# ldyken53/gaussian-splatting-wgpu

Hardware: AMD Instinct MI355X
Metric: frames/sec (higher is better)
Workload: dtype f32; 1 GPU; bicycle-like synthetic 6.1M gaussians @1920x1080; gaussians=6100000, width=1920, height=1080, tile_size=16, parallelism=single GPU, visible=2430918, processed=15909895, block_evaluated=6068168, sort_passes=1, depth_ordered_emission=True, tight_binning=True, blend_mode=fused, camera=64-step orbit, moved every frame

## Files before the change

gaussian-splatting-wgpu_amd/csrc/build.py:

```python
#!/usr/bin/env python3
import os
import subprocess
import sys
from concurrent.futures import ThreadPoolExecutor

HERE = os.path.dirname(os.path.abspath(__file__))
OUT = os.path.join(HERE, "..", "lib")
HIPCC = os.environ.get("HIPCC", "/opt/rocm/bin/hipcc")
ARCH = "gfx950"
FLAGS = ["--offload-arch=" + ARCH, "-O3", "-std=c++17", "-ffp-contract=off", "-fno-slp-vectorize", "-fPIC", "-fvisibility=hidden",
         "-Wall", "-Wno-unused-function", "-Wno-unused-value", "-Wno-unused-result"]
FILE_FLAGS = {}
SOURCES = ["k_preprocess.hip", "k_binning.hip", "k_gsort.hip", "k_rows.hip", "k_sort.hip", "k_blend.hip", "k_pick.hip", "k_state.hip", "k_export.hip", "k_insert.hip", "k_snapshot.hip", "k_xform.hip", "k_grade.hip", "k_coverage.hip", "k_attr.hip", "k_neigh.hip", "k_cluster.hip", "k_knn.hip", "k_pack.hip",
           "gs_context.hip", "gs_frame.hip", "gs_readback.hip", "gs_state.hip", "gs_export.hip", "gs_insert.hip", "gs_snapshot.hip", "gs_xform.hip", "gs_xform_math.hip", "gs_grade.hip", "gs_grade_math.hip", "gs_coverage.hip", "gs_attr.hip", "gs_neigh.hip", "gs_cluster.hip", "gs_knn.hip", "gs_pack.hip", "gs_pack_host.hip", "gs_ply.hip", "gs_stages.hip",
           "k_moments.hip", "gs_moments.hip", "k_pairs.hip", "gs_pairs.hip", "k_consensus.hip", "gs_consensus.hip", "k_merge.hip", "gs_merge.hip", "k_surface.hip", "gs_surface.hip"]


def _stale(target, deps):
    if not os.path.exists(target):
        return True
    t = os.path.getmtime(target)
    return any(os.path.getmtime(d) > t for d in deps)


def build(force=False, verbose=False, profiling=False):
    os.makedirs(OUT, exist_ok=True)
    objdir = os.path.join(OUT, "obj_prof" if profiling else "obj")
    os.makedirs(objdir, exist_ok=True)
    headers = [os.path.join(HERE, h) for h in ("gs_device.h", "gs_binning.h", "gs_kernels.h", "gs_tight.h", "gs_runtime.h", "gs_xform_math.h", "gs_grade_math.h", "gs_state_sum.h", "gs_neigh_dev.h", "gs_pack_math.h", "gs_exact_sum.h", "gs_exact_dev.h", "gs_pair_host.h", "gs_pack_host.h", "gs_file_writer.h", "gs_consensus_host.h", "gs_merge_math.h", "gs_grid_math.h", "gs_surface_math.h")] + [
        os.path.join(HERE, "..", "..", "include", "gsplat", "gs_abi.h")]

    def compile_one(src):
        obj = os.path.join(objdir, src.replace(".hip", ".o"))
        path = os.path.join(HERE, src)
        if force or _stale(obj, [path] + headers):
            cmd = [HIPCC] + FLAGS + FILE_FLAGS.get(src, []) + (["-DGS_PROFILING"] if profiling else []) + ["-c", path, "-o", obj]
            if verbose:
                print(" ".join(cmd))
            subprocess.check_call(cmd)
        return obj

    with ThreadPoolExecutor(max_workers=12) as ex:
        objs = list(ex.map(compile_one, SOURCES))
    so = os.path.join(OUT, "libgsplat_hip_prof.so" if profiling else "libgsplat_hip.so")
    if force or _stale(so, objs):
        subprocess.check_call([HIPCC, "--offload-arch=" + ARCH, "-shared", "-fPIC", "-o", so] + objs)
    return os.path.abspath(so)


if __name__ == "__main__":
    print(build(force="--force" in sys.argv, verbose=True, profiling="--profiling" in sys.argv))


def build_napi(force=False, verbose=False):
    inc = "/usr/include/node"
    if not os.path.exists(os.path.join(inc, "node_api.h")):
        return None
    so = build(force=force, verbose=verbose)
    src = os.path.join(HERE, "napi", "gs_napi.c")
    out = os.path.join(OUT, "gsplat_napi.node")
    if force or _stale(out, [src, so, os.path.join(HERE, "..", "..", "include", "gsplat", "gs_abi.h")]):
        cmd = ["gcc", "-O2", "-fPIC", "-shared", "-Wall", "-DNODE_GYP_MODULE_NAME=gsplat_napi", "-I" + inc, src, "-o", out,
               "-L" + OUT, "-lgsplat_hip", "-Wl,-rpath,$ORIGIN"]
        if verbose:
            print(" ".join(cmd))
        subprocess.check_call(cmd)
    return os.path.abspath(out)
```

gaussian-splatting-wgpu_amd/csrc/gs_context.hip:

```cpp
#include <atomic>
#include <cmath>
#include <cstdarg>
#include <memory>
#include <new>

#include "gs_runtime.h"

thread_local char g_err[512] = "";
int32_t fail(int32_t code, const char* fmt, ...) {
    va_list ap;
    va_start(ap, fmt);
    vsnprintf(g_err, sizeof(g_err), fmt, ap);
    va_end(ap);
    return code;
}

static uint32_t tiles_f32(uint32_t extent, uint32_t ts) {
    return (uint32_t)std::ceil((float)extent / (float)ts);
}
static uint32_t bits_for(uint64_t v) {
    uint32_t b = 0;
    while (v) { ++b; v >>= 1; }
    return b ? b : 1;
}

GS_EXPORT const char* gs_last_error(void) { return g_err; }
GS_EXPORT int32_t gs_abi_version(void) { return GS_ABI_VERSION; }

int32_t alloc_kv(gs_ctx* c, uint64_t capacity, uint64_t row_cap) {
    if (capacity >= (1ull << 30)) return fail(GS_ERR_CAPACITY, "capacity %llu exceeds 2^30 intersections", (unsigned long long)capacity);
    if (row_cap >= (1ull << 31)) return fail(GS_ERR_CAPACITY, "%llu row items exceed the 2^31 limit", (unsigned long long)row_cap);
    c->gr.valid = false;
    c->keysA.reset(); c->valsA.reset(); c->keysB.reset(); c->valsB.reset(); c->keysU.reset(); c->valsU.reset();
    c->keysG.reset(); c->chunk_table.reset(); c->arena.reset(); c->rows_sorted.reset(); c->M3.reset(); c->ctl_mem.reset();
    c->valsG.reset();
    c->keysG_valid = c->valsG_valid = c->gdataG_valid = false;
    capacity = std::max<uint64_t>(capacity, 4096);
    row_cap = (std::max<uint64_t>(row_cap, 4096) + 15) & ~(uint64_t)15;
    const size_t kb = (size_t)capacity * 4;
    HIP_TRY(hipMalloc(c->keysA.out(), kb));
    HIP_TRY(hipMalloc(c->valsA.out(), kb));
    HIP_TRY(hipMalloc(c->keysB.out(), kb));
    HIP_TRY(hipMalloc(c->valsB.out(), kb));
    c->sort_index = GsSort{{c->keysA, c->valsA}, {c->keysB, c->valsB}, c->passes, 8, 0, false, false};
    c->sort_tile = GsSort{{c->keysA, c->valsA}, {c->keysB, c->valsB}, c->tile_passes, c->tile_bits, c->tile16 ? 0u : 1u, c->tile16, true};
    HIP_TRY(hipMalloc(c->chunk_table.out(), (size_t)gs_emit_chunks(std::max(capacity, row_cap)) * 4));
    if (c->tight_ok) {
        HIP_TRY(hipMalloc(c->arena.out(), (size_t)row_cap * 12));
        HIP_TRY(hipMalloc(c->rows_sorted.out(), gs_rows_sorted_bytes(row_cap)));
        HIP_TRY(hipMalloc(c->M3.out(), (size_t)gs_rows_chunks(row_cap) * 256 * 4));
    }
    const size_t ctl_sz = (sizeof(GsControl) + 255) & ~(size_t)255;
    const size_t scan_sz = (((size_t)gs_scan_blocks(c->n ? c->n : 1) + 1) * 8 + 255) & ~(size_t)255;
    const size_t sort_sz = (size_t)std::max(c->passes, c->tile_passes) * gs_sort_tiles(capacity) * 256 * 4;
    const size_t rows_sz = c->tight_ok ? (size_t)gs_rows_sort_tiles(row_cap) * 256 * 4 : 0;
    const size_t depth_sz = ((size_t)c->T * 4 + 255) & ~(size_t)255;
    c->ctl_bytes = ctl_sz + depth_sz + rows_sz + scan_sz + sort_sz;
    c->ctl_bytes_tight = ctl_sz + depth_sz + rows_sz;
    HIP_TRY(hipMalloc(c->ctl_mem.out(), c->ctl_bytes));
    char* const base = (char*)c->ctl_mem.get();
    c->ctl = (GsControl*)base;
    c->tile_depth = (uint32_t*)(base + ctl_sz);
    c->rows_status = (uint32_t*)(base + ctl_sz + depth_sz);
    c->scan_status = (unsigned long long*)(base + ctl_sz + depth_sz + rows_sz);
    c->sort_status = (uint32_t*)(base + ctl_sz + depth_sz + rows_sz + scan_sz);
    c->capacity = capacity;
    c->row_cap = row_cap;
    c->frame.capacity = (uint32_t)capacity;
    c->frame.row_cap = (uint32_t)row_cap;
    return GS_OK;
}

GS_EXPORT int32_t gs_create(const gs_config* cfg, gs_ctx** out) {
    if (!cfg || !out) return fail(GS_ERR_INVALID_ARGUMENT, "gs_create: null argument");
    if (cfg->struct_size != sizeof(gs_config)) return fail(GS_ERR_INVALID_ARGUMENT, "gs_create: struct_size %u != %zu", cfg->struct_size, sizeof(gs_config));
    if (cfg->width == 0 || cfg->height == 0) return fail(GS_ERR_INVALID_ARGUMENT, "gs_create: empty canvas");
    if (cfg->tile_size != 8 && cfg->tile_size != 16 && cfg->tile_size != 32)
        return fail(GS_ERR_INVALID_ARGUMENT, "gs_create: tile_size must be 8, 16 or 32 (got %u)", cfg->tile_size);
    int ndev = 0;
    if (hipGetDeviceCount(&ndev) != hipSuccess || ndev == 0) return fail(GS_ERR_NO_DEVICE, "gs_create: no HIP device");
    if (cfg->device < 0 || cfg->device >= ndev) return fail(GS_ERR_INVALID_ARGUMENT, "gs_create: device %d of %d", cfg->device, ndev);
    HIP_TRY(hipSetDevice(cfg->device));

    std::unique_ptr<gs_ctx> c(new (std::nothrow) gs_ctx());
    if (!c) return fail(GS_ERR_OUT_OF_MEMORY, "gs_create: host allocation failed");
    c->cfg = *cfg;
    GsFrame& f = c->frame;
    f.width = cfg->width; f.height = cfg->height; f.tile_size = cfg->tile_size;
    f.ntx = tiles_f32(cfg->width, cfg->tile_size);
    f.nty = tiles_f32(cfg->height, cfg->tile_size);
    if (f.ntx >= 32768 || f.nty >= 65536) return fail(GS_ERR_INVALID_ARGUMENT, "gs_create: canvas too large");
    f.col0 = cfg->col_begin;
    f.col1 = cfg->col_end;
    if (f.col0 == 0 && f.col1 == 0) f.col1 = f.ntx;
    if (f.col1 > f.ntx || f.col0 >= f.col1) return fail(GS_ERR_INVALID_ARGUMENT, "gs_create: bad tile-column slab [%u,%u) of %u", f.col0, f.col1, f.ntx);
    f.full = (f.col0 == 0 && f.col1 == f.ntx) ? 1u : 0u;
    f.px0 = f.col0 * f.tile_size;
    f.slab_w = std::min(f.width, f.col1 * f.tile_size) - f.px0;
    c->T = f.ntx * f.nty;
    const uint64_t max_key = ((uint64_t)f.nty * f.ntx + f.ntx) * 1000ull + 999ull;
    if (max_key > 0xFFFFFFFFull) return fail(GS_ERR_INVALID_ARGUMENT, "gs_create: tile ids overflow the 32-bit key (write_tile_ids.wgsl:29)");
    c->key_bits = bits_for(max_key);
    c->passes = (c->key_bits + 7) / 8;
    const uint32_t tbits = bits_for((uint64_t)f.nty * f.ntx + f.ntx);
    c->tile_passes = (tbits + 7) / 8;
    c->tile_bits = (tbits + c->tile_passes - 1) / c->tile_passes;
    c->tile16 = ((uint64_t)f.nty * f.ntx + f.ntx) < 0xFFFFull;
    if ((uint64_t)(f.ntx + 1) * (f.nty + 1) > GS_COUNT_MASK) return fail(GS_ERR_INVALID_ARGUMENT, "gs_create: canvas has too many tiles");
    c->tight_ok = f.ntx <= 255u && f.nty <= 255u;

    hipDeviceProp_t prop;
    HIP_TRY(hipGetDeviceProperties(&prop, cfg->device));
    c->opt.grid_persist = (uint32_t)prop.multiProcessorCount * 4;
    if (cfg->stream) c->stream = (hipStream_t)cfg->stream;
    else { HIP_TRY(hipStreamCreateWithFlags(c->own_stream.out(), hipStreamNonBlocking)); c->stream = c->own_stream; }

    HIP_TRY(hipMalloc(c->ranges.out(), (size_t)c->T * 4));
    HIP_TRY(hipMemset(c->ranges, 0, (size_t)c->T * 4));
    const size_t px = (size_t)f.slab_w * f.height;
    HIP_TRY(hipMalloc(c->rgba8.out(), px * 4));
    HIP_TRY(hipMemset(c->rgba8, 0, px * 4));
    if (cfg->flags & GS_FLAG_F32_TAP) HIP_TRY(hipMalloc(c->rgbf.out(), px * 12));
    if (cfg->flags & GS_FLAG_AUX_OUTPUTS) {
        HIP_TRY(hipMalloc(c->alpha.out(), px * 4));
        HIP_TRY(hipMalloc(c->depth.out(), px * 4));
        HIP_TRY(hipMemset(c->alpha, 0, px * 4));
        HIP_TRY(hipMemset(c->depth, 0, px * 4));
    }
    HIP_TRY(hipHostMalloc(c->h_ctl.out(), sizeof(GsControl), hipHostMallocDefault));
    memset(c->h_ctl, 0, sizeof(GsControl));
    HIP_TRY(hipMalloc(c->d_pxb.out(), 65 * 4));
    HIP_TRY(hipMalloc(c->tileoff.out(), 256 * 256 * 4));
    HIP_TRY(hipMalloc(c->rowtot.out(), 256 * 4));
    HIP_TRY(hipMalloc(c->sticky.out(), 4 * 4));
    HIP_TRY(hipMemset(c->sticky, 0, 4 * 4));
    HIP_TRY(hipHostMalloc(c->h_rep.out(), sizeof(GsReport), hipHostMallocDefault));
    memset(c->h_rep, 0, sizeof(GsReport));
    if (cfg->flags & GS_FLAG_TIMING) {
        for (auto& row : c->ev)
            for (auto& e : row) HIP_TRY(hipEventCreate(e.out()));
        c->have_events = true;
    }
    c->fif = (c->own_stream && f.full) ? 3u : 1u;
    *out = c.release();
    return GS_OK;
}

gs_ctx::~gs_ctx() { drop_graph(this); }

GS_EXPORT int32_t gs_destroy(gs_ctx* c) {
    if (!c) return GS_OK;
    hipSetDevice(c->cfg.device);
    drop_shadows(c);
    if (c->stream) hipStreamSynchronize(c->stream);
    delete c;
    return GS_OK;
}

static int32_t alloc_per_gaussian(gs_ctx* c, uint64_t n, uint64_t min_capacity = 0, uint64_t min_rows = 0) {
    c->gr.valid = false;
    c->scene_own.reset();
    c->scene_mem = nullptr;
    c->n = (uint32_t)n;
    c->frame.n = (uint32_t)n;
    c->have_frame = false;
    c->cov.reset();
    c->ng = gs_ctx::Neigh{};
    c->cl = gs_ctx::Cluster{};
    c->kn = gs_ctx::Knn{};
    c->sf = gs_ctx::Surface{};
    c->counts.reset(); c->offsets.reset(); c->grec.reset(); c->rowptr.reset(); c->gsort_scratch.reset(); c->gdata.reset(); c->gdataG.reset();
    c->unit_off.reset(); c->unit_n.reset();
    const size_t np = ((size_t)n + 63) & ~(size_t)63;
    const size_t ne = (size_t)gs_gsort_tiles((uint32_t)(n ? n : 1)) * 2048, nu = ne / 1024 + 2;
    HIP_TRY(hipMalloc(c->counts.out(), ne * 4));
    HIP_TRY(hipMalloc(c->offsets.out(), std::max<size_t>(np * 4, 256)));
    HIP_TRY(hipMalloc(c->grec.out(), std::max<size_t>(np * 16, 256)));
    HIP_TRY(hipMalloc(c->rowptr.out(), ne * 4));
    HIP_TRY(hipMalloc(c->unit_off.out(), ne * 2));
    HIP_TRY(hipMalloc(c->unit_n.out(), nu * 4));
    HIP_TRY(hipMemsetAsync(c->unit_n, 0, nu * 4, c->stream));
    HIP_TRY(hipMalloc(c->gsort_scratch.out(), gs_gsort_scratch_bytes((uint32_t)n)));
    HIP_TRY(hipMalloc(c->gdata.out(), ((size_t)n + GS_RECORD_SLACK) * 64));
    HIP_TRY(hipMemsetAsync(c->gdata, 0, ((size_t)n + GS_RECORD_SLACK) * 64, c->stream));
    uint64_t cap = c->cfg.max_intersections ? c->cfg.max_intersections : std::max<uint64_t>(4 * n, 1u << 22);
    cap = std::max<uint64_t>(cap, min_capacity);
    cap = std::min<uint64_t>(cap, (1ull << 30) - 1);
    const uint64_t rows = std::max<uint64_t>(std::max<uint64_t>(2 * n, 1u << 20), min_rows);
    return alloc_kv(c, cap, rows);
}

GsSceneLayout scene_layout(void* base, uint64_t n, bool state) {
    GsSceneLayout L;
    const size_t np = ((size_t)n + 63) & ~(size_t)63;
    const size_t sh_end = np * 4 * 4 + np * 32 + (size_t)n * 192, state_at = (sh_end + 255) & ~(size_t)255;
    L.np = np;
    L.state_at = state_at;
    L.bytes = state ? state_at + np : sh_end;
    char* p = (char*)base;
    GsScene& s = L.scene;
    s.px = (float*)p; p += np * 4; s.py = (float*)p; p += np * 4; s.pz = (float*)p; p += np * 4;
    s.smax = (float*)p; p += np * 4;
    s.geo = (float4*)p; p += np * 32;
    s.sh = (float4*)p;
    s.state = state ? (const uint8_t*)base + state_at : nullptr;
    return L;
}
static void scene_views(gs_ctx* c, uint64_t n) {
    const GsSceneLayout L = scene_layout(c->scene_own.get(), n, has_state(c));
    c->scene_mem = c->scene_own;
    c->scene_bytes = L.bytes;
    c->scene = L.scene;
}

uint64_t scene_new_serial() {
    static std::atomic<uint64_t> next{1};
    return next.fetch_add(1, std::memory_order_relaxed);
}
int32_t scene_alloc(gs_ctx* c, uint64_t n, uint64_t min_capacity, uint64_t min_rows) {
    c->scene_serial = scene_new_serial();
    int32_t rc = alloc_per_gaussian(c, n, min_capacity, min_rows);
    if (rc != GS_OK) return rc;
    const GsSceneLayout L = scene_layout(nullptr, n, has_state(c));
    HIP_TRY(hipMalloc(c->scene_own.out(), std::max<size_t>(L.bytes, 256)));
    scene_views(c, n);
    if (has_state(c))
        HIP_TRY(hipMemsetAsync((char*)c->scene_mem + L.state_at, 0, std::max<size_t>(L.np, 4), c->stream));
    return GS_OK;
}

int32_t scene_install(gs_ctx* c, DevBuf<>&& mem, uint64_t n, uint64_t min_capacity, uint64_t min_rows) {
    const int32_t rc = alloc_per_gaussian(c, n, min_capacity, min_rows);
    if (rc != GS_OK) {
        c->scene = GsScene{};
        c->n = c->frame.n = 0;
        return rc;
    }
    c->scene_own = std::move(mem);
    scene_views(c, n);
    return GS_OK;
}

static int32_t upload_common(gs_ctx* c, const void* d_aos, uint64_t n) {
    int32_t rc = scene_alloc(c, n);
    if (rc != GS_OK) return rc;
    if (n) gs_launch_repack(d_aos, (uint32_t)n, 0, c->scene, c->stream);
    HIP_TRY(hipGetLastError());
    HIP_TRY(hipStreamSynchronize(c->stream));
    return GS_OK;
}

void drop_shadows(gs_ctx* c) {
    for (gs_ctx* s : c->shadows) gs_destroy(s);
    c->shadows.clear();
    c->last = c;
    c->rr = 0;
    c->cap_hint = 0;
    c->row_hint = 0;
}
GS_EXPORT int32_t gs_share_splats(gs_ctx* c, gs_ctx* owner) {
    if (!c || !owner || c == owner) return fail(GS_ERR_INVALID_ARGUMENT, "gs_share_splats: needs two distinct contexts");
    if (c->cfg.device != owner->cfg.device) return fail(GS_ERR_INVALID_ARGUMENT, "gs_share_splats: contexts are on different devices");
    if (!c->is_shadow) drop_shadows(c);
    if (!owner->scene_mem) return fail(GS_ERR_NO_SCENE, "gs_share_splats: the owner holds no splats");
    if (has_state(c) && !has_state(owner))
        return fail(GS_ERR_INVALID_ARGUMENT, "gs_share_splats: this context has GS_FLAG_SPLAT_STATE, the owner keeps no state plane");
    HIP_TRY(hipSetDevice(c->cfg.device));
    if (c->pending) { int32_t rc = wait_one(c); if (rc != GS_OK) return rc; }
    int32_t rc = alloc_per_gaussian(c, owner->n, c->cfg.max_intersections ? 0 : owner->capacity, owner->row_cap);
    if (rc != GS_OK) return rc;
    c->scene_mem = owner->scene_mem;
    c->scene_bytes = owner->scene_bytes;
    c->scene = owner->scene;
    c->scene_serial = scene_new_serial();
    HIP_TRY(hipStreamSynchronize(c->stream));
    return GS_OK;
}

GS_EXPORT int32_t gs_upload_splats_device(gs_ctx* c, const void* d_aos, uint64_t n) {
    if (!c || (!d_aos && n)) return fail(GS_ERR_INVALID_ARGUMENT, "gs_upload_splats_device: null argument");
    if (n >= (1ull << 31)) return fail(GS_ERR_INVALID_ARGUMENT, "gs_upload_splats: too many gaussians");
    HIP_TRY(hipSetDevice(c->cfg.device));
    drop_shadows(c);
    return upload_common(c, d_aos, n);
}

GS_EXPORT int32_t gs_upload_splats(gs_ctx* c, const void* aos, uint64_t n) {
    if (!c || (!aos && n)) return fail(GS_ERR_INVALID_ARGUMENT, "gs_upload_splats: null argument");
    if (n >= (1ull << 31)) return fail(GS_ERR_INVALID_ARGUMENT, "gs_upload_splats: too many gaussians");
    HIP_TRY(hipSetDevice(c->cfg.device));
    drop_shadows(c);
    DevBuf<> d;
    const size_t bytes = (size_t)n * GS_SPLAT_RECORD_BYTES;
    HIP_TRY(hipMalloc(d.out(), std::max<size_t>(bytes, 256)));
    if (bytes) {
        hipError_t e = hipMemcpy(d, aos, bytes, hipMemcpyHostToDevice);
        if (e != hipSuccess) return fail(GS_ERR_HIP, "upload memcpy: %s", hipGetErrorString(e));
    }
    return upload_common(c, d, n);
}

GS_EXPORT int32_t gs_host_alloc(uint64_t bytes, void** out) {
    if (!out) return fail(GS_ERR_INVALID_ARGUMENT, "gs_host_alloc: null argument");
    *out = nullptr;
    HIP_TRY(hipHostMalloc(out, std::max<size_t>((size_t)bytes, 256), hipHostMallocDefault));
    return GS_OK;
}
GS_EXPORT void gs_host_free(void* p) { if (p) hipHostFree(p); }

GS_EXPORT int32_t gs_slab_width(gs_ctx* c, uint32_t* px_begin, uint32_t* px_width) {
    if (!c) return fail(GS_ERR_INVALID_ARGUMENT, "gs_slab_width: null ctx");
    if (px_begin) *px_begin = c->frame.px0;
    if (px_width) *px_width = c->frame.slab_w;
    return GS_OK;
}

static int32_t set_option_one(gs_ctx* c, int32_t key, int64_t value) {
    c->gr.valid = false;
    GsOptions& o = c->opt;
    switch (key) {
    case GS_OPT_FRAME_GRAPH: o.frame_graph = (value != 0); return GS_OK;
    case GS_OPT_BLEND_ABLATION: o.blend_ablation = (uint32_t)value & 0x3FFFFu; return GS_OK;
    case GS_OPT_PERSISTENT_GRID: if (value <= 0) break; o.grid_persist = (uint32_t)value; return GS_OK;
    case GS_OPT_RESET_TIMING: c->timed_from = c->frames; c->max_I_seen = 0; c->truncated_frames = 0; return GS_OK;
    case GS_OPT_EMIT_ORDER: if (value < 0 || value > 2) break; o.emit_order = (int)value; return GS_OK;
    case GS_OPT_UNFUSED: return GS_OK;
    case GS_OPT_DEBUG_VIEW: if (value < 0 || value > 4) break; o.debug_view = (uint32_t)value; return GS_OK;
    case GS_OPT_TILE_CULL: o.tile_cull = (value != 0); return GS_OK;
    case GS_OPT_PROJ_CHUNKS: if (value != 0 && value != 2 && value != 4 && value != 8) break; o.tight_nb = (uint32_t)value; return GS_OK;
    case GS_OPT_SELECT_TINT:
        if (!has_state(c)) return fail(GS_ERR_INVALID_ARGUMENT, "gs_set_option: GS_OPT_SELECT_TINT needs GS_FLAG_SPLAT_STATE");
        if (value < 0 || value > 0xFFFFFFFFll) break;
        o.select_tint = (uint32_t)value;
        return GS_OK;
    default: break;
    }
    return fail(GS_ERR_INVALID_ARGUMENT, "gs_set_option: bad key/value %d/%lld", key, (long long)value);
}
GS_EXPORT int32_t gs_set_option(gs_ctx* c, int32_t key, int64_t value) {
    if (!c) return fail(GS_ERR_INVALID_ARGUMENT, "gs_set_option: null ctx");
    if (key == GS_OPT_FRAMES_IN_FLIGHT) {
        if (value < 1 || value > 4) return fail(GS_ERR_INVALID_ARGUMENT, "gs_set_option: frames in flight must be 1..4");
        if (!c->own_stream || !c->frame.full) value = 1;
        int32_t rc = gs_wait(c);
        if (rc != GS_OK && rc != GS_ERR_TRUNCATED) return rc;
        while (c->shadows.size() + 1 > (size_t)value) {
            if (c->last == c->shadows.back()) { c->last = c; }
            gs_destroy(c->shadows.back());
            c->shadows.pop_back();
        }
        c->fif = (uint32_t)value;
        c->rr = 0;
        return GS_OK;
    }
    int32_t rc = set_option_one(c, key, value);
    for (gs_ctx* s : c->shadows) if (rc == GS_OK) rc = set_option_one(s, key, value);
    return rc;
}
```

gaussian-splatting-wgpu_amd/csrc/gs_device.h:

```cpp
#pragma once
#include <hip/hip_runtime.h>
#include <stdint.h>

#define GS_WAVE 64

struct GsFrame {
    uint32_t n;
    uint32_t width, height, tile_size;
    uint32_t ntx, nty;
    uint32_t col0, col1;
    uint32_t px0, slab_w;
    uint32_t capacity;
    uint32_t full;
    uint32_t row_cap;
};

#define GS_COUNT_BITS 22
#define GS_COUNT_MASK 0x3FFFFFu

struct GsControl {
    uint32_t scan_ticket[2];
    uint32_t sort_ticket[4];
    uint32_t rows_ticket;
    uint32_t num_slots;
    uint32_t num_items;
    uint32_t fault;
    uint32_t overflow;
    uint32_t num_intersections;
    uint32_t num_visible;
    uint32_t pad0;
    uint32_t row_cursor[16];
    uint32_t rec_cursor[16];
    unsigned long long num_processed[64];
    unsigned long long num_evaluated[64];
    uint32_t hist[4][256];
    uint32_t rowhist[8][256];
};
__device__ __forceinline__ uint32_t gs_rowhist(const GsControl* ctl, uint32_t r) {
    uint32_t s = 0;
#pragma unroll
    for (int k = 0; k < 8; ++k) s += ctl->rowhist[k][r];
    return s;
}

struct GsReport {
    uint32_t fault, overflow, num_intersections, num_visible, num_slots, num_items, pad0, pad1;
    uint32_t row_cursor[16];
    uint32_t sticky[4];
};
__device__ __forceinline__ void gs_frame_report(const GsControl* ctl, uint32_t I, uint32_t num_items, uint32_t capacity, uint32_t* sticky,
                                                GsReport* rep) {
    uint32_t need = 0;
    for (int k = 0; k < 16; ++k) need = ctl->row_cursor[k] > need ? ctl->row_cursor[k] : need;
    need = need > 0x07FFFFFFu ? 0x7FFFFFFFu : need * 16u;
    const uint32_t over = (I > capacity || ctl->overflow) ? 1u : 0u;
    uint32_t s0 = 0, s1 = 0, s2 = 0, s3 = 0;
    if (sticky) {
        s0 = atomicAdd(&sticky[0], over) + over;
        s1 = atomicOr(&sticky[1], ctl->fault ? 1u : 0u) | (ctl->fault ? 1u : 0u);
        s2 = atomicMax(&sticky[2], I); s2 = s2 > I ? s2 : I;
        s3 = atomicMax(&sticky[3], need); s3 = s3 > need ? s3 : need;
    }
    if (rep) {
        rep->fault = ctl->fault; rep->overflow = over; rep->num_intersections = I; rep->num_visible = ctl->num_visible;
        rep->num_slots = ctl->num_slots; rep->num_items = num_items;
        for (int k = 0; k < 16; ++k) rep->row_cursor[k] = ctl->row_cursor[k];
        rep->sticky[0] = s0; rep->sticky[1] = s1; rep->sticky[2] = s2; rep->sticky[3] = s3;
    }
}

struct GsTightOut {
    uint32_t* arena; uint32_t* rowptr; GsControl* ctl;
    unsigned short* unit_off; uint32_t* unit_n;
    uint32_t rec_shard_cap;
};
#define GS_RECORD_SLACK (16u * 512u * 8u)

struct GsScene {
    const float* px; const float* py; const float* pz;
    const float* smax;
    const float4* geo;
    const float4* sh;
    const uint8_t* state;
};

#define GS_ST_HIDDEN 1u
#define GS_ST_SELECTED 2u
struct GsTint { float t[3]; float k; };
__device__ __forceinline__ uint32_t gs_state_apply(uint32_t s, uint32_t op, uint32_t bits) {
    return op == 1u ? (s | bits) : op == 2u ? (s & ~bits) : op == 3u ? (s ^ bits) : bits;
}
struct GsStateQuad { uint32_t w, valid; };
__device__ __forceinline__ GsStateQuad gs_state_quad(const uint8_t* __restrict__ state, uint32_t n, uint32_t q) {
    const uint64_t first = (uint64_t)q * 4u;
    uint32_t w = 0u, valid = 0u;
    if (first + 4u <= n) {
        valid = 4u;
        if (state) w = reinterpret_cast<const uint32_t*>(state)[q];
    } else if (first < n) {
        valid = (uint32_t)(n - first);
        if (state)
            for (uint32_t k = 0; k < valid; ++k) w |= (uint32_t)state[first + k] << (8u * k);
    }
    return GsStateQuad{w, valid};
}

struct GsPlyTable {
    uint32_t stride, nsrc, all_float;
    uint16_t soff[11 + 48];
    uint8_t stype[11 + 48], slot[11 + 48];
};

struct GsUniforms {
    float view[16];
    float proj[16];
    float cam[3];
    float tan_fovx, tan_fovy, focal_x, focal_y, scale_modifier;
};

__device__ __forceinline__ float wg_max(float a, float b) { return (a < b) ? b : a; }
__device__ __forceinline__ float wg_min(float a, float b) { return (b < a) ? b : a; }
__device__ __forceinline__ int wg_maxi(int a, int b) { return (a < b) ? b : a; }
__device__ __forceinline__ int wg_mini(int a, int b) { return (b < a) ? b : a; }

__device__ __forceinline__ int f2i_sat(float x) {
    if (x != x) return 0;
    if (x >= 2147483648.0f) return 2147483647;
    if (x <= -2147483648.0f) return (-2147483647 - 1);
    return (int)x;
}
__device__ __forceinline__ uint32_t f2u_sat(float x) {
    if (x != x) return 0u;
    if (x >= 4294967296.0f) return 0xFFFFFFFFu;
    if (x <= 0.0f) return 0u;
    return (uint32_t)x;
}

__device__ __forceinline__ float gs_exp(float x) {
    if (x != x) return x;
    if (x > 88.72283935546875f) return __builtin_inff();
    if (x < -103.97208404541015625f) return 0.0f;
    const float nf = __builtin_rintf(x * 1.44269502162933349609375f);
    float r = __builtin_fmaf(-nf, 0.693145751953125f, x);
    r = __builtin_fmaf(-nf, 1.42860677465796470642e-06f, r);
    float p = 1.9875691500e-4f;
    p = __builtin_fmaf(p, r, 1.3981999507e-3f);
    p = __builtin_fmaf(p, r, 8.3334519073e-3f);
    p = __builtin_fmaf(p, r, 4.1665795894e-2f);
    p = __builtin_fmaf(p, r, 1.6666665459e-1f);
    p = __builtin_fmaf(p, r, 5.0000001201e-1f);
    const float z = r * r;
    float y = __builtin_fmaf(p, z, r);
    y = y + 1.0f;
    const int n = (int)nf;
    const int a = n >> 1;
    const int b = n - a;
    const float sa = __uint_as_float((uint32_t)(a + 127) << 23);
    const float sb = __uint_as_float((uint32_t)(b + 127) << 23);
    return (y * sa) * sb;
}

__device__ __forceinline__ float gs_blend_power(float cx, float cy, float cz, float dx, float dy) {
    const float t1 = cx * dx * dx, t2 = cz * dy * dy, t3 = cy * dx * dy;
    return -0.5f * (t1 + t2) - t3;
}
__device__ __forceinline__ float gs_blend_alpha(float op, float power) { return wg_min(0.99f, op * gs_exp(power)); }
struct GsPixel { float T, cr, cg, cb, cd; };
template <bool AUX>
__device__ __forceinline__ GsPixel gs_blend_exact(GsPixel p, float4 p1, float4 p2, float dx, float dy) {
    const float power = gs_blend_power(p1.x, p1.y, p1.z, dx, dy);
    const float alpha = gs_blend_alpha(p2.w, power);
    const float test = p.T * (1.0f - alpha);
    const float cond = (power <= 0.0f && alpha >= (float)(1.0 / 255.0) && test >= 0.0001f) ? 1.0f : 0.0f;
    p.cr += cond * p2.x * alpha * p.T;
    p.cg += cond * p2.y * alpha * p.T;
    p.cb += cond * p2.z * alpha * p.T;
    if constexpr (AUX) p.cd += cond * p1.w * alpha * p.T;
    p.T = cond * test + (1.0f - cond) * p.T;
    return p;
}
template <bool EXACT>
__device__ __forceinline__ bool gs_pixel_final(float T) {
    const float c255 = (float)(1.0 / 255.0);
    return (EXACT ? T * (1.0f - c255) : __builtin_fmaf(-T, c255, T)) < 0.0001f;
}

__device__ __forceinline__ float block_qmin(float cx, float cy, float cz, float dxlo, float dxhi, float dylo, float dyhi,
                                            float& mag) {
    const float X = __builtin_fminf(__builtin_fmaxf(0.0f, dxlo), dxhi);
    const float Y = __builtin_fminf(__builtin_fmaxf(0.0f, dylo), dyhi);
    float q = 3.0e38f;
    mag = 0.0f;
    if (X == 0.0f && Y == 0.0f) return 0.0f;
    if (X != 0.0f) {
        const float dy = __builtin_fminf(__builtin_fmaxf(-cy * X * __builtin_amdgcn_rcpf(cz), dylo), dyhi);
        const float a = 0.5f * cx * X * X, b = 0.5f * cz * dy * dy, c = cy * X * dy;
        q = a + b + c;
        mag = __builtin_fabsf(a) + __builtin_fabsf(b) + __builtin_fabsf(c);
    }
    if (Y != 0.0f) {
        const float dx = __builtin_fminf(__builtin_fmaxf(-cy * Y * __builtin_amdgcn_rcpf(cx), dxlo), dxhi);
        const float a = 0.5f * cx * dx * dx, b = 0.5f * cz * Y * Y, c = cy * dx * Y;
        const float q2 = a + b + c;
        if (q2 < q) { q = q2; mag = __builtin_fabsf(a) + __builtin_fabsf(b) + __builtin_fabsf(c); }
    }
    return q;
}

__device__ __forceinline__ bool blend_tmax_cull(float cx, float cy, float cz, float op, float dxlo, float dxhi, float dylo, float dyhi, float Tmax) {
    const float ax0 = (0.5f * cx) * dxlo * dxlo, ax1 = (0.5f * cx) * dxhi * dxhi, by0 = (0.5f * cz) * dylo * dylo, by1 = (0.5f * cz) * dyhi * dyhi;
    const float c00 = cy * dxlo * dylo, c01 = cy * dxlo * dyhi, c10 = cy * dxhi * dylo, c11 = cy * dxhi * dyhi;
    const float qmax = __builtin_fmaxf(__builtin_fmaxf(ax0 + by0 + c00, ax0 + by1 + c01), __builtin_fmaxf(ax1 + by0 + c10, ax1 + by1 + c11));
    const float qmag = __builtin_fmaxf(ax0, ax1) + __builtin_fmaxf(by0, by1) +
                       __builtin_fmaxf(__builtin_fmaxf(__builtin_fabsf(c00), __builtin_fabsf(c01)), __builtin_fmaxf(__builtin_fabsf(c10), __builtin_fabsf(c11)));
    const float alo = 0.99f * __builtin_fminf(0.99f, op * __builtin_amdgcn_exp2f(-1.44269502162933349609375f * (qmax + 1.0e-5f * qmag)));
    return Tmax * (1.0f - alo) < 0.0000999f;
}

struct GsLiveBox { float c0, c1, r0, r1; };
template <bool EMPTY_OK>
__device__ __forceinline__ GsLiveBox gs_live_box(unsigned long long lv) {
    uint32_t lcm = (uint32_t)lv | (uint32_t)(lv >> 32);
    lcm |= lcm >> 16; lcm |= lcm >> 8; lcm &= 0xFFu;
    const unsigned long long lo = EMPTY_OK ? lv | (1ull << 63) : lv, hi = EMPTY_OK ? lv | 1ull : lv;
    return GsLiveBox{(float)__builtin_ctz(lcm | 0x100u), (float)(31 - __builtin_clz(lcm | 1u)), (float)(__builtin_ctzll(lo) >> 3),
                     (float)((63 - __builtin_clzll(hi)) >> 3)};
}

__device__ __forceinline__ uint2 gs_tile_range(const uint32_t* __restrict__ ranges, uint32_t tile, uint32_t capacity) {
    const uint32_t start = tile > 0 ? ranges[tile - 1] : 0u;
    uint32_t end = ranges[tile];
    if (end > capacity) end = capacity;
    return make_uint2(start, end);
}

struct GsListRec {
    float ux, uy, cx, cy, cz, z, op;
    uint32_t id;
    bool live;
};
__device__ __forceinline__ GsListRec gs_list_fetch(const uint4* __restrict__ gdata, const uint32_t* __restrict__ values, uint32_t i, uint32_t end,
                                                   uint32_t id_mask, uint32_t want, uint32_t nrec, uint32_t n) {
    GsListRec r;
    r.ux = r.uy = r.cx = r.cy = r.cz = r.z = r.op = 0.0f;
    r.id = 0u;
    r.live = false;
    if (i < end) {
        const uint32_t v = values[i];
        const uint32_t g = v & id_mask;
        if (g < nrec && (want == 0u || (v & want) != 0u)) {
            const uint4 p0 = gdata[(uint64_t)g * 4 + 0];
            const uint4 p1 = gdata[(uint64_t)g * 4 + 1];
            r.op = __uint_as_float(((const uint32_t*)gdata)[(uint64_t)g * 16 + 11]);
            r.ux = __uint_as_float(p0.x); r.uy = __uint_as_float(p0.y);
            r.cx = __uint_as_float(p1.x); r.cy = __uint_as_float(p1.y); r.cz = __uint_as_float(p1.z); r.z = __uint_as_float(p1.w);
            r.id = p0.z;
            r.live = p0.z < n;
        }
    }
    return r;
}
__device__ __forceinline__ uint32_t gs_bcast(uint32_t v, int l) { return (uint32_t)__builtin_amdgcn_readlane((int)v, l); }
__device__ __forceinline__ float gs_bcast(float v, int l) { return __uint_as_float((uint32_t)__builtin_amdgcn_readlane((int)__float_as_uint(v), l)); }

__device__ __forceinline__ void slab_cols(uint32_t rx0, uint32_t rx1, const GsFrame& f, uint32_t& xa, uint32_t& wmain,
                                          uint32_t& alias) {
    const uint32_t hi = rx1 < f.ntx ? rx1 : f.ntx;
    xa = rx0 > f.col0 ? rx0 : f.col0;
    const uint32_t xb = hi < f.col1 ? hi : f.col1;
    wmain = xb > xa ? xb - xa : 0u;
    alias = (rx1 == f.ntx + 1u && f.col0 == 0u) ? 1u : 0u;
}

__device__ __forceinline__ uint32_t lane_id() { return __builtin_amdgcn_mbcnt_hi(~0u, __builtin_amdgcn_mbcnt_lo(~0u, 0u)); }

#define GS_DPP(v, ctrl, rm) (uint32_t)__builtin_amdgcn_update_dpp(0, (int)(v), (ctrl), (rm), 0xf, false)
__device__ __forceinline__ uint32_t wave_incl_scan(uint32_t v, uint32_t) {
    v += GS_DPP(v, 0x111, 0xf);
    v += GS_DPP(v, 0x112, 0xf);
    v += GS_DPP(v, 0x114, 0xf);
    v += GS_DPP(v, 0x118, 0xf);
    v += GS_DPP(v, 0x142, 0xa);
    v += GS_DPP(v, 0x143, 0xc);
    return v;
}
__device__ __forceinline__ unsigned long long wave_incl_scan64(unsigned long long v, uint32_t lane) {
#pragma unroll
    for (int d = 1; d < 64; d <<= 1) {
        const uint32_t lo = __shfl_up((uint32_t)v, d, 64), hi = __shfl_up((uint32_t)(v >> 32), d, 64);
        if ((int)lane >= d) v += ((unsigned long long)hi << 32) | lo;
    }
    return v;
}
__device__ __forceinline__ uint32_t wave_incl_max(uint32_t v) {
    uint32_t t;
    t = GS_DPP(v, 0x111, 0xf); v = (t > v) ? t : v;
    t = GS_DPP(v, 0x112, 0xf); v = (t > v) ? t : v;
    t = GS_DPP(v, 0x114, 0xf); v = (t > v) ? t : v;
    t = GS_DPP(v, 0x118, 0xf); v = (t > v) ? t : v;
    t = GS_DPP(v, 0x142, 0xa); v = (t > v) ? t : v;
    t = GS_DPP(v, 0x143, 0xc); v = (t > v) ? t : v;
    return v;
}
__device__ __forceinline__ uint32_t wave_sum(uint32_t v) {
    return (uint32_t)__builtin_amdgcn_readlane((int)wave_incl_scan(v, 0u), 63);
}

__device__ __forceinline__ void st_agent(uint32_t* p, uint32_t v) {
    __hip_atomic_store(p, v, __ATOMIC_RELAXED, __HIP_MEMORY_SCOPE_AGENT);
}
__device__ __forceinline__ uint32_t ld_agent(const uint32_t* p) {
    return __hip_atomic_load(p, __ATOMIC_RELAXED, __HIP_MEMORY_SCOPE_AGENT);
}
// ... 9 lines not shown
```

gaussian-splatting-wgpu_amd/csrc/gs_export.hip:

```cpp
#include "gs_file_writer.h"
#include "gs_runtime.h"

static int32_t edit_begin(gs_ctx* c, const char* who, uint32_t mask, uint32_t value) { return resident_begin(c, who, Plane::filtered, mask, value); }

int32_t edit_select(gs_ctx* c, uint32_t mask, uint32_t value, bool want_ids, uint64_t* total) {
    const uint32_t nb = gs_select_blocks(c->n);
    int32_t rc = c->ex.counts.reserve((uint64_t)nb + 1);
    if (rc != GS_OK) return rc;
    gs_launch_select_count(c->scene.state, c->n, mask, value, c->ex.counts, c->stream);
    HIP_TRY(hipGetLastError());
    uint32_t t = 0;
    HIP_TRY(hipMemcpyAsync(&t, c->ex.counts.get() + nb, 4, hipMemcpyDeviceToHost, c->stream));
    HIP_TRY(hipStreamSynchronize(c->stream));
    *total = t;
    if (!want_ids || !t) return GS_OK;
    rc = c->ex.ids.reserve(t);
    if (rc != GS_OK) return rc;
    gs_launch_select_scatter(c->scene.state, c->n, mask, value, c->ex.counts, c->ex.ids, t, c->stream);
    HIP_TRY(hipGetLastError());
    return GS_OK;
}

GS_EXPORT int32_t gs_state_list(gs_ctx* c, uint32_t mask, uint32_t value, uint32_t* ids, uint64_t cap, uint64_t* n) {
    int32_t rc = edit_begin(c, "gs_state_list", mask, value);
    if (rc != GS_OK) return rc;
    if (!n) return fail(GS_ERR_INVALID_ARGUMENT, "gs_state_list: null n");
    uint64_t total = 0;
    rc = edit_select(c, mask, value, ids != nullptr, &total);
    if (rc != GS_OK) return rc;
    *n = total;
    if (!ids) return GS_OK;
    if (cap < total) return fail(GS_ERR_INVALID_ARGUMENT, "gs_state_list: %llu ids needed, the buffer holds %llu", (unsigned long long)total, (unsigned long long)cap);
    if (total) HIP_TRY(hipMemcpyAsync(ids, c->ex.ids, (size_t)total * 4, hipMemcpyDeviceToHost, c->stream));
    HIP_TRY(hipStreamSynchronize(c->stream));
    return GS_OK;
}

static int32_t export_common(gs_ctx* c, const char* who, uint32_t mask, uint32_t value, void* out, uint64_t cap, uint64_t* n, uint32_t* ids_out,
                             bool device) {
    int32_t rc = edit_begin(c, who, mask, value);
    if (rc != GS_OK) return rc;
    if (!n) return fail(GS_ERR_INVALID_ARGUMENT, "%s: null n", who);
    const bool all = !(mask | value);
    uint64_t total = c->n;
    if (!all) {
        rc = edit_select(c, mask, value, out != nullptr, &total);
        if (rc != GS_OK) return rc;
    }
    *n = total;
    if (!out) return GS_OK;
    if (cap < total) return fail(GS_ERR_INVALID_ARGUMENT, "%s: %llu records needed, the buffer holds %llu", who, (unsigned long long)total, (unsigned long long)cap);
    const uint32_t* sel = all ? nullptr : c->ex.ids.get();
    if (device) {
        gs_launch_unpack(c->scene, c->n, sel, 0, (uint32_t)total, out, ids_out, c->stream);
        HIP_TRY(hipGetLastError());
        HIP_TRY(hipStreamSynchronize(c->stream));
        return GS_OK;
    }
    DevBuf<> bounce;
    HIP_TRY(hipMalloc(bounce.out(), std::max<size_t>((size_t)std::min(total, kBounceRecords) * GS_SPLAT_RECORD_BYTES, 256)));
    for (uint64_t first = 0; first < total; first += kBounceRecords) {
        const uint64_t m = std::min(kBounceRecords, total - first);
        gs_launch_unpack(c->scene, c->n, sel, (uint32_t)first, (uint32_t)m, bounce, nullptr, c->stream);
        HIP_TRY(hipGetLastError());
        HIP_TRY(hipMemcpyAsync((char*)out + first * GS_SPLAT_RECORD_BYTES, bounce, (size_t)m * GS_SPLAT_RECORD_BYTES, hipMemcpyDeviceToHost, c->stream));
        HIP_TRY(hipStreamSynchronize(c->stream));
    }
    if (ids_out) {
        if (all) for (uint64_t i = 0; i < total; ++i) ids_out[i] = (uint32_t)i;
        else if (total) HIP_TRY(hipMemcpy(ids_out, c->ex.ids, (size_t)total * 4, hipMemcpyDeviceToHost));
    }
    return GS_OK;
}

GS_EXPORT int32_t gs_export_splats(gs_ctx* c, uint32_t mask, uint32_t value, void* aos320, uint64_t cap_records, uint64_t* n, uint32_t* ids) {
    return export_common(c, "gs_export_splats", mask, value, aos320, cap_records, n, ids, false);
}
GS_EXPORT int32_t gs_export_splats_device(gs_ctx* c, uint32_t mask, uint32_t value, void* d_aos320, uint64_t cap_records, uint64_t* n,
                                          uint32_t* d_ids) {
    return export_common(c, "gs_export_splats_device", mask, value, d_aos320, cap_records, n, d_ids, true);
}

GS_EXPORT int32_t gs_compact(gs_ctx* c, uint32_t mask, uint32_t value, uint64_t* kept, uint32_t* ids) {
    int32_t rc = edit_begin(c, "gs_compact", mask, value);
    if (rc != GS_OK) return rc;
    if (c->scene_mem != c->scene_own.get())
        return fail(GS_ERR_INVALID_ARGUMENT, "gs_compact: this context borrows its splats (gs_share_splats): compact the owner");
    uint64_t total = 0;
    rc = edit_select(c, mask, value, true, &total);
    if (rc != GS_OK) return rc;
    if (ids && total) HIP_TRY(hipMemcpyAsync(ids, c->ex.ids, (size_t)total * 4, hipMemcpyDeviceToHost, c->stream));
    HIP_TRY(hipStreamSynchronize(c->stream));
    drop_shadows(c);
    DevBuf<> old_mem = std::move(c->scene_own);
    const GsScene old = c->scene;
    const uint32_t n_old = c->n;
    rc = scene_alloc(c, total, c->capacity, c->row_cap);
    if (rc != GS_OK) {
        c->scene_own.reset();
        c->scene_mem = nullptr;
        c->scene = GsScene{};
        c->n = c->frame.n = 0;
        return rc;
    }
    gs_launch_compact_planes(old, n_old, c->ex.ids, (uint32_t)total, c->scene, c->stream);
    HIP_TRY(hipGetLastError());
    HIP_TRY(hipStreamSynchronize(c->stream));
    if (kept) *kept = total;
    return GS_OK;
}

static void ply_rows(const uint32_t* rec, uint64_t m, int K, uint32_t* out) {
    for (uint64_t i = 0; i < m; ++i, rec += 80) {
        *out++ = rec[0]; *out++ = rec[1]; *out++ = rec[2];
        *out++ = 0u; *out++ = 0u; *out++ = 0u;
        *out++ = rec[16]; *out++ = rec[17]; *out++ = rec[18];
        for (int ch = 0; ch < 3; ++ch)
            for (int k = 0; k < K; ++k) *out++ = rec[16 + 4 * (k + 1) + ch];
        *out++ = rec[12];
        *out++ = rec[4]; *out++ = rec[5]; *out++ = rec[6];
        *out++ = rec[8]; *out++ = rec[9]; *out++ = rec[10]; *out++ = rec[11];
    }
}
static std::string ply_header(uint64_t n, int K) {
    std::string h = "ply\nformat binary_little_endian 1.0\nelement vertex " + std::to_string(n) + "\n";
    auto prop = [&](const std::string& name) { h += "property float " + name + "\n"; };
    for (const char* nm : {"x", "y", "z", "nx", "ny", "nz", "f_dc_0", "f_dc_1", "f_dc_2"}) prop(nm);
    for (int k = 0; k < 3 * K; ++k) prop("f_rest_" + std::to_string(k));
    for (const char* nm : {"opacity", "scale_0", "scale_1", "scale_2", "rot_0", "rot_1", "rot_2", "rot_3"}) prop(nm);
    return h + "end_header\n";
}
static constexpr uint64_t kPlyChunk = kStreamTrip;

GS_EXPORT int32_t gs_ply_save(const char* path, const void* records, uint64_t n, int32_t sh_degree) {
    if (!path) return fail(GS_ERR_INVALID_ARGUMENT, "gs_ply_save: null path");
    if (!records && n) return fail(GS_ERR_INVALID_ARGUMENT, "gs_ply_save: null records (%s)", path);
    if (sh_degree < 0 || sh_degree > 3) return fail(GS_ERR_INVALID_ARGUMENT, "gs_ply_save: sh_degree %d is not 0..3 (%s)", sh_degree, path);
    const int K = (sh_degree + 1) * (sh_degree + 1) - 1;
    const size_t row = 17 + 3 * (size_t)K;
    FileWriter w("gs_ply_save", path);
    int32_t rc = w.open(ply_header(n, K));
    if (rc != GS_OK) return rc;
    std::vector<uint32_t> rows((size_t)std::min<uint64_t>(std::max<uint64_t>(n, 1), kPlyChunk) * row);
    for (uint64_t first = 0; first < n; first += kPlyChunk) {
        const uint64_t m = std::min(kPlyChunk, n - first);
        ply_rows((const uint32_t*)records + first * 80, m, K, rows.data());
        rc = w.write(rows.data(), (size_t)m * row * 4);
        if (rc != GS_OK) return rc;
    }
    return w.finish();
}

GS_EXPORT int32_t gs_export_ply(gs_ctx* c, const char* path, uint32_t mask, uint32_t value, int32_t sh_degree, uint64_t* n_out) {
    int32_t rc = edit_begin(c, "gs_export_ply", mask, value);
    if (rc != GS_OK) return rc;
    if (!path) return fail(GS_ERR_INVALID_ARGUMENT, "gs_export_ply: null path");
    if (sh_degree < 0 || sh_degree > 3) return fail(GS_ERR_INVALID_ARGUMENT, "gs_export_ply: sh_degree %d is not 0..3 (%s)", sh_degree, path);
    const bool all = !(mask | value);
    uint64_t total = c->n;
    if (!all) {
        rc = edit_select(c, mask, value, true, &total);
        if (rc != GS_OK) return rc;
    }
    const uint32_t* sel = all ? nullptr : c->ex.ids.get();
    const int K = (sh_degree + 1) * (sh_degree + 1) - 1;
    const size_t row = 17 + 3 * (size_t)K;
    const size_t chunk_bytes = (size_t)kPlyChunk * GS_SPLAT_RECORD_BYTES;
    FileWriter w("gs_export_ply", path);
    rc = w.open(ply_header(total, K));
    if (rc != GS_OK) return rc;
    DevBuf<> d_stage;
    TripRing ring;
    HIP_TRY(hipMalloc(d_stage.out(), chunk_bytes));
    rc = ring.init(chunk_bytes, false);
    if (rc != GS_OK) return rc;
    std::vector<uint32_t> rows((size_t)kPlyChunk * row);
    auto records = [&](uint64_t it) { return std::min(kPlyChunk, total - it * kPlyChunk); };
    rc = ring.drain((total + kPlyChunk - 1) / kPlyChunk, c->stream,
                    [&](uint64_t it, unsigned char* h) {
                        gs_launch_unpack(c->scene, c->n, sel, (uint32_t)(it * kPlyChunk), (uint32_t)records(it), d_stage, nullptr, c->stream);
                        HIP_TRY(hipGetLastError());
                        HIP_TRY(hipMemcpyAsync(h, d_stage, (size_t)records(it) * GS_SPLAT_RECORD_BYTES, hipMemcpyDeviceToHost, c->stream));
                        return (int32_t)GS_OK;
                    },
                    [&](uint64_t it, unsigned char* h) {
                        ply_rows((const uint32_t*)h, records(it), K, rows.data());
                        return w.write(rows.data(), (size_t)records(it) * row * 4);
                    });
    if (rc != GS_OK) return rc;
    HIP_TRY(hipStreamSynchronize(c->stream));
    rc = w.finish();
    if (rc != GS_OK) return rc;
    if (n_out) *n_out = total;
    return GS_OK;
}
```

gaussian-splatting-wgpu_amd/csrc/gs_frame.hip:

```cpp
#include <dlfcn.h>

#include "gs_runtime.h"
#include "gs_tight.h"

namespace {
struct Roctx {
    int (*push)(const char*) = nullptr;
    int (*pop)() = nullptr;
    Roctx() {
        void* h = dlopen("librocprofiler-sdk-roctx.so.1", RTLD_LAZY | RTLD_LOCAL);
        if (!h) h = dlopen("libroctx64.so.4", RTLD_LAZY | RTLD_LOCAL);
        if (h) {
            push = (int (*)(const char*))dlsym(h, "roctxRangePushA");
            pop = (int (*)())dlsym(h, "roctxRangePop");
            if (!push || !pop) push = nullptr, pop = nullptr;
        }
    }
};
Roctx& roctx() { static Roctx r; return r; }
const char* const kStageRange[] = {"gsplat:process_gaussians", "gsplat:exclusive_scan", "gsplat:write_tile_ids", "gsplat:radix_sort",
                                   "gsplat:compute_ranges", "gsplat:compute_tiles"};
}

static inline void mark(gs_ctx* c, int i) {
    if (!c->have_events) return;
    hipEventRecord(c->ev[c->frames % GS_EV_RING][i], c->stream);
    Roctx& r = roctx();
    if (r.push) {
        if (i > 0) r.pop();
        if (i < GS_STAGE_COUNT) r.push(kStageRange[i]);
    }
}

static void mark_cb(void* p, int i) { mark((gs_ctx*)p, i); }

GsLists frame_lists(const gs_ctx* c) {
    return GsLists{c->gdata, c->notes.valsS, c->ranges, c->frame, c->notes.last_tight ? GS_ID_MASK : 0xFFFFFFFFu,
                   c->notes.last_tight ? c->n + GS_RECORD_SLACK : c->n};
}

static void prepare_projection(gs_ctx* c, const GsUniforms& u, bool tight) {
    gs_preprocess_prepare(c->pre, c->scene, u, c->frame, c->gdata, c->counts, tight, c->arena, c->rowptr, c->unit_off, c->unit_n, c->ctl, c->opt.tight_nb,
                          has_state(c), tint_of(c->opt.select_tint));
}


static FrameNotes bin_tight(gs_ctx* c) {
    hipStream_t st = c->stream;
    gs_launch_gsort(c->counts, c->rowptr, c->unit_off, c->unit_n, c->n, c->gsort_scratch, c->grec, c->chunk_table,
                    (uint32_t)gs_emit_chunks(std::max(c->capacity, c->row_cap)), &c->ctl->num_visible, &c->ctl->num_slots, c->opt.grid_persist, st);
    mark(c, 2);
    gs_launch_rows(c->arena, c->grec, c->chunk_table, c->rows_sorted, c->ctl, c->rows_status, (uint32_t)c->row_cap, c->M3, c->tileoff, c->rowtot, c->frame,
                   c->valsA, c->ranges, c->opt.grid_persist / 4u, c->sticky, c->h_rep, st, mark_cb, c);
    mark(c, 4);
    return FrameNotes{nullptr, c->valsA,  1u,  1u,  false,  false,  true};
}

static FrameNotes sort_to_ranges(gs_ctx* c, const GsSort& plan, bool by_index) {
    hipStream_t st = c->stream;
    mark(c, 3);
    const GsSortPair sorted = gs_launch_sort(plan, c->ctl, c->sort_status, (uint32_t)c->capacity, c->opt.grid_persist, st);
    mark(c, 4);
    const uint32_t grid = c->opt.grid_persist * 2;
    if (plan.keys16) gs_launch_ranges16((const uint16_t*)sorted.keys, c->ctl, (uint32_t)c->capacity, c->T, c->ranges, grid, c->sticky, c->h_rep, st);
    else gs_launch_ranges(sorted.keys, c->ctl, (uint32_t)c->capacity, c->T, c->ranges, grid, c->sticky, c->h_rep, st);
    return FrameNotes{sorted.keys, sorted.vals, plan.passes,  1u, by_index, plan.keys16,  false};
}

static int32_t bin_by_index(gs_ctx* c, bool debug, FrameNotes& nt) {
    hipStream_t st = c->stream;
    gs_launch_scan(c->counts, c->n, c->offsets, c->scan_status, &c->ctl->scan_ticket[0], c->ctl, st);
    mark(c, 2);
    gs_launch_emit(c->gdata, c->counts, c->offsets, c->frame, c->keysA, c->valsA, c->ctl, st);
    if (debug) {
        const size_t kb = (size_t)c->capacity * 4;
        if (!c->keysU) {
            HIP_TRY(hipMalloc(c->keysU.out(), kb));
            HIP_TRY(hipMalloc(c->valsU.out(), kb));
        }
        HIP_TRY(hipMemcpyAsync(c->keysU, c->keysA, kb, hipMemcpyDeviceToDevice, st));
        HIP_TRY(hipMemcpyAsync(c->valsU, c->valsA, kb, hipMemcpyDeviceToDevice, st));
    }
    nt = sort_to_ranges(c, c->sort_index, true);
    return GS_OK;
}

static FrameNotes bin_by_depth(gs_ctx* c) {
    gs_launch_gsort(c->counts, nullptr, nullptr, nullptr, c->n, c->gsort_scratch, c->grec, c->chunk_table, (uint32_t)gs_emit_chunks(std::max(c->capacity, c->row_cap)),
                    &c->ctl->num_visible, &c->ctl->num_intersections, c->opt.grid_persist, c->stream);
    mark(c, 2);
    gs_launch_emit_balanced(c->gdata, c->grec, c->chunk_table, c->frame, c->keysA, c->valsA, c->ctl, c->opt.grid_persist * 2, c->tile_bits, c->tile_passes,
                            c->tile16, c->stream);
    return sort_to_ranges(c, c->sort_tile, false);
}

static int32_t record_frame(gs_ctx* c, const GsUniforms& u, bool debug, void* ext_rgba8, bool tight, bool index_order) {
    hipStream_t st = c->stream;
    const GsOptions& o = c->opt;
    gs_launch_zero(c->ctl_mem, tight ? c->ctl_bytes_tight : c->ctl_bytes, st);
    c->h_ctl_valid = false;
    if (debug) HIP_TRY(hipMemsetAsync(c->gdata, 0, std::max<size_t>((size_t)c->n * 64, 256), st));
    mark(c, 0);
    prepare_projection(c, u, tight);
    gs_launch_preprocess(c->pre, st);
    mark(c, 1);
    FrameNotes& nt = c->notes;
    if (tight) nt = bin_tight(c);
    else if (!debug && !index_order) nt = bin_by_depth(c);
    else if (const int32_t rc = bin_by_index(c, debug, nt); rc != GS_OK) return rc;
    mark(c, 5);
    uint32_t* target = ext_rgba8 ? (uint32_t*)ext_rgba8 : c->rgba8.get();
    const bool prof = (o.blend_ablation & 0x10000u) != 0;
    if (prof && !c->blend_prof) HIP_TRY(hipMalloc(c->blend_prof.out(), (size_t)(1u << 20) * 16));
    const bool aux = (c->cfg.flags & GS_FLAG_AUX_OUTPUTS) != 0;
    const int walkers = gs_launch_blend(frame_lists(c), target, c->rgbf, aux, c->alpha, c->depth, c->ctl, c->tile_depth, (c->cfg.flags & GS_FLAG_EXACT_BLEND) != 0,
                                        o.blend_ablation & 0xFFFFu, st, prof ? c->blend_prof.get() : nullptr, &c->blend_prof_blocks);
    if (walkers == -2) return fail(GS_ERR_INVALID_ARGUMENT, "blend: GS_FLAG_AUX_OUTPUTS without its alpha / depth planes");
    if (walkers < 0) return fail(GS_ERR_INVALID_ARGUMENT, "unsupported tile size %u", c->frame.tile_size);
    nt.blend_walkers = (uint32_t)walkers;
    mark(c, 6);
    if (o.debug_view) gs_launch_debug_view(c->ranges, c->frame, o.debug_view, target, st);
    return GS_OK;
}

void drop_graph(gs_ctx* c) {
    if (c->gr.exec) hipGraphExecDestroy(c->gr.exec);
    if (c->gr.graph) hipGraphDestroy(c->gr.graph);
    c->gr.exec = nullptr; c->gr.graph = nullptr; c->gr.pre_node = nullptr;
    c->gr.valid = false;
}

static int32_t enqueue_frame(gs_ctx* c, const GsUniforms& u, bool debug, void* ext_rgba8) {
    hipStream_t st = c->stream;
    bool index_order = (c->opt.emit_order == 1);
    if (c->opt.emit_order == 2) {
        const uint64_t saved = c->passes > c->tile_passes ? c->passes - c->tile_passes : 0;
        index_order = !(c->have_frame && saved * (uint64_t)c->h_rep->num_intersections >= 1000000ull);
    }
    const bool tight = !debug && c->opt.tile_cull && c->tight_ok && (uint64_t)c->n + GS_RECORD_SLACK <= (1ull << GS_ID_BITS);
    const bool graphable = c->opt.frame_graph && !debug && !c->have_events && !(c->opt.blend_ablation & 0x10000u) && c->n;
    if (graphable) {
        const GraphKey key{index_order, tight, ext_rgba8, c->alpha, c->depth};
        if (!c->gr.exec || !c->gr.valid || !(c->gr.key == key)) {
            if (c->gr.exec) HIP_TRY(hipStreamSynchronize(st));
            drop_graph(c);
            HIP_TRY(hipStreamBeginCapture(st, hipStreamCaptureModeRelaxed));
            const int32_t rc = record_frame(c, u, debug, ext_rgba8, tight, index_order);
            const hipError_t e = hipStreamEndCapture(st, &c->gr.graph);
            if (rc != GS_OK) { drop_graph(c); return rc; }
            if (e != hipSuccess || !c->gr.graph) return fail(GS_ERR_HIP, "frame graph capture: %s", hipGetErrorString(e));
            hipGraph_t g = c->gr.graph;
            HIP_TRY(hipGraphInstantiate(&c->gr.exec, g, nullptr, nullptr, 0));
            size_t nn = 0;
            HIP_TRY(hipGraphGetNodes(g, nullptr, &nn));
            std::vector<hipGraphNode_t> nodes(nn);
            HIP_TRY(hipGraphGetNodes(g, nodes.data(), &nn));
            uint32_t found = 0;
            for (hipGraphNode_t nd : nodes) {
                hipGraphNodeType ty;
                if (hipGraphNodeGetType(nd, &ty) != hipSuccess || ty != hipGraphNodeTypeKernel) continue;
                hipKernelNodeParams kp;
                if (hipGraphKernelNodeGetParams(nd, &kp) == hipSuccess && kp.func == c->pre.func) { c->gr.pre_node = nd; ++found; }
            }
            if (found != 1) {
                c->opt.frame_graph = false;
                c->gr.pre_node = nullptr;
            }
            c->gr.key = key;
            c->gr.notes = c->notes;
            c->gr.valid = true;
        } else {
            c->notes = c->gr.notes;
            prepare_projection(c, u, tight);
            hipKernelNodeParams kp{};
            kp.func = const_cast<void*>(c->pre.func);
            kp.gridDim = dim3(c->pre.blocks); kp.blockDim = dim3(256); kp.sharedMemBytes = 0;
            kp.kernelParams = c->pre.args; kp.extra = nullptr;
            HIP_TRY(hipGraphExecKernelNodeSetParams(c->gr.exec, c->gr.pre_node, &kp));
        }
        HIP_TRY(hipGraphLaunch(c->gr.exec, st));
        c->gr.frames++;
    } else {
        const int32_t rc = record_frame(c, u, debug, ext_rgba8, tight, index_order);
        if (rc != GS_OK) return rc;
    }
    c->keysG_valid = c->valsG_valid = c->gdataG_valid = false;
    c->h_ctl_valid = false;
    HIP_TRY(hipGetLastError());
    c->pending = true;
    c->have_frame = true;
    c->last_debug = debug;
    c->last_ext = ext_rgba8;
    c->last_u = u;
    c->frames++;
    return GS_OK;
}

static int32_t render_common(gs_ctx* c, const void* uniforms, bool debug, void* ext) {
    if (!c || !uniforms) return fail(GS_ERR_INVALID_ARGUMENT, "gs_render: null argument");
    if (!c->scene_mem) return fail(GS_ERR_NO_SCENE, "gs_render: no splats uploaded");
    HIP_TRY(hipSetDevice(c->cfg.device));
    GsUniforms u;
    static_assert(sizeof(GsUniforms) == GS_UNIFORM_BYTES, "uniform block must be 160 bytes");
    memcpy(&u, uniforms, sizeof(u));
    return enqueue_frame(c, u, debug, ext);
}

int32_t wait_one(gs_ctx* c) {
    if (!c) return fail(GS_ERR_INVALID_ARGUMENT, "gs_wait: null ctx");
    HIP_TRY(hipSetDevice(c->cfg.device));
    uint32_t dropped = 0;
    for (int attempt = 0; attempt < 8; ++attempt) {
        HIP_TRY(hipStreamSynchronize(c->stream));
        c->pending = false;
        if (!c->have_frame) return GS_OK;
        const uint32_t over_frames = c->h_rep->sticky[0], fault_any = c->h_rep->sticky[1];
        const uint64_t max_I = c->h_rep->sticky[2], max_rows = c->h_rep->sticky[3];
        if (over_frames || fault_any || max_I || max_rows) HIP_TRY(hipMemset(c->sticky, 0, 4 * 4));
        c->h_rep->sticky[0] = c->h_rep->sticky[1] = c->h_rep->sticky[2] = c->h_rep->sticky[3] = 0;
        if (max_I > c->max_I_seen) c->max_I_seen = max_I;
        if (fault_any || c->h_rep->fault) return fail(GS_ERR_DEVICE_FAULT, "a look-back spin exceeded its bound (fault word set)");
        const uint64_t I = c->h_rep->num_intersections;
        uint64_t rows_last = 0;
        if (c->notes.last_tight)
            for (int k = 0; k < 16; ++k) rows_last = std::max<uint64_t>(rows_last, (uint64_t)c->h_rep->row_cursor[k] * 16);
        const bool last_over = I > c->capacity || c->h_rep->overflow;
        if (attempt == 0 && over_frames > (last_over ? 1u : 0u)) dropped = over_frames - (last_over ? 1u : 0u);
        const uint64_t need = std::max<uint64_t>(I, max_I), need_rows = std::max<uint64_t>(rows_last, max_rows);
        if (!last_over && need <= c->capacity && need_rows <= c->row_cap) break;
        if (need >= (1ull << 30)) return fail(GS_ERR_CAPACITY, "%llu intersections exceed the 2^30 limit", (unsigned long long)need);
        uint64_t want = c->capacity, want_rows = c->row_cap;
        if (need > c->capacity) want = std::min<uint64_t>(std::max<uint64_t>(need + need / 4, c->capacity * 2), (1ull << 30) - 1);
        if (need_rows > c->row_cap) want_rows = std::max<uint64_t>(need_rows + need_rows / 4, c->row_cap * 2);
        if (want == c->capacity && want_rows == c->row_cap) {
            if (last_over) return fail(GS_ERR_CAPACITY, "the frame reports an overflow that growing cannot fix (capacity %llu, rows %llu)",
                                       (unsigned long long)c->capacity, (unsigned long long)c->row_cap);
            break;
        }
        int32_t rc = alloc_kv(c, want, want_rows);
        if (rc != GS_OK) return rc;
        if (!last_over) break;
        if (attempt == 7) return fail(GS_ERR_CAPACITY, "capacity did not converge");
        c->frames--;
        rc = enqueue_frame(c, c->last_u, c->last_debug, c->last_ext);
        if (rc != GS_OK) return rc;
    }
    if (dropped) {
        c->truncated_frames += dropped;
        return fail(GS_ERR_TRUNCATED, "%u frame(s) enqueued before the last one overflowed the (key,value) capacity and were rendered from "
                    "truncated lists; the capacity has been grown to %llu -- wait after every frame, or pass gs_config.max_intersections",
                    dropped, (unsigned long long)c->capacity);
    }
    return GS_OK;
}

GS_EXPORT int32_t gs_wait(gs_ctx* c) {
    if (!c) return fail(GS_ERR_INVALID_ARGUMENT, "gs_wait: null ctx");
    int32_t first = wait_one(c);
    char msg[sizeof(g_err)];
    if (first != GS_OK) memcpy(msg, g_err, sizeof(msg));
    for (gs_ctx* s : c->shadows) {
        const int32_t rc = wait_one(s);
        if (rc != GS_OK && first == GS_OK) { first = rc; memcpy(msg, g_err, sizeof(msg)); }
    }
    c->cap_hint = std::max(c->cap_hint, over_ring(c, [](const gs_ctx* m) { return m->capacity; }, true));
    c->row_hint = std::max(c->row_hint, over_ring(c, [](const gs_ctx* m) { return m->row_cap; }, true));
    if (first != GS_OK) memcpy(g_err, msg, sizeof(msg));
    return first;
}

static int32_t add_shadow(gs_ctx* c) {
    gs_config cfg = c->cfg;
    cfg.stream = nullptr;
    cfg.max_intersections = 0;
    gs_ctx* s = nullptr;
    int32_t rc = gs_create(&cfg, &s);
    if (rc != GS_OK) return rc;
    s->fif = 1;
    s->is_shadow = true;
    rc = gs_share_splats(s, c);
    if (rc != GS_OK) { gs_destroy(s); return rc; }
    s->opt = c->opt;
    c->shadows.push_back(s);
    return GS_OK;
}

GS_EXPORT int32_t gs_render(gs_ctx* c, const void* uniforms) {
    if (!c || !uniforms) return fail(GS_ERR_INVALID_ARGUMENT, "gs_render: null argument");
    gs_ctx* t = c;
    if (c->fif > 1 && c->scene_mem) {
        if (c->pending && c->shadows.size() + 1 < c->fif) {
            int32_t rc = add_shadow(c);
            if (rc != GS_OK) return rc;
            c->rr = (uint32_t)c->shadows.size();
        }
        if (!c->shadows.empty()) {
            const uint32_t slot = c->rr++ % (uint32_t)(c->shadows.size() + 1);
            t = slot ? c->shadows[slot - 1] : c;
        }
        if (t->capacity < c->cap_hint || t->row_cap < c->row_hint) {
            HIP_TRY(hipSetDevice(t->cfg.device));
            if (t->pending) { int32_t rc = wait_one(t); if (rc != GS_OK && rc != GS_ERR_TRUNCATED) return rc; }
            int32_t rc = alloc_kv(t, std::max(t->capacity, c->cap_hint), std::max(t->row_cap, c->row_hint));
            if (rc != GS_OK) return rc;
            t->have_frame = false;
        }
    }
    const int32_t rc = render_common(t, uniforms, false, nullptr);
    if (rc == GS_OK) c->last = t;
    return rc;
}
GS_EXPORT int32_t gs_render_debug(gs_ctx* c, const void* uniforms) {
    const int32_t rc = render_common(c, uniforms, true, nullptr);
    if (rc == GS_OK && c) c->last = c;
    return rc;
}
GS_EXPORT int32_t gs_render_to(gs_ctx* c, const void* uniforms, void* d_rgba8) {
    if (!d_rgba8) return fail(GS_ERR_INVALID_ARGUMENT, "gs_render_to: null output");
    const int32_t rc = render_common(c, uniforms, false, d_rgba8);
    if (rc == GS_OK && c) c->last = c;
    return rc;
}

GS_EXPORT int32_t gs_render_host(gs_ctx* c, const void* uniforms, void* host_dst, uint64_t size, uint64_t* ticket) {
    if (!c || !uniforms || !host_dst || !ticket) return fail(GS_ERR_INVALID_ARGUMENT, "gs_render_host: null argument");
    const uint64_t bytes = (uint64_t)c->frame.slab_w * c->frame.height * 4;
    if (size < bytes) return fail(GS_ERR_INVALID_ARGUMENT, "gs_render_host: need %llu bytes, got %llu", (unsigned long long)bytes, (unsigned long long)size);
    int32_t rc = gs_render(c, uniforms);
    if (rc != GS_OK) return rc;
    gs_ctx* t = last_of(c);
    if (!t->ev_done) HIP_TRY(hipEventCreateWithFlags(t->ev_done.out(), hipEventDisableTiming));
    HIP_TRY(hipMemcpyAsync(host_dst, t->rgba8, bytes, hipMemcpyDeviceToHost, t->stream));
    std::lock_guard<std::mutex> lk(c->ticket_mu);
    HIP_TRY(hipEventRecord(t->ev_done, t->stream));
    const uint64_t k = c->next_ticket++;
    c->tickets[k & 63u].ticket = k;
    c->tickets[k & 63u].member = t;
    *ticket = k;
    return GS_OK;
}

GS_EXPORT int32_t gs_wait_ticket(gs_ctx* c, uint64_t ticket) {
    if (!c) return fail(GS_ERR_INVALID_ARGUMENT, "gs_wait_ticket: null ctx");
    gs_ctx* t = nullptr;
    {
        std::lock_guard<std::mutex> lk(c->ticket_mu);
        if (ticket == 0 || ticket >= c->next_ticket) return fail(GS_ERR_INVALID_ARGUMENT, "gs_wait_ticket: unknown ticket %llu", (unsigned long long)ticket);
        if (c->next_ticket - ticket > 64 || c->tickets[ticket & 63u].ticket != ticket) return GS_OK;
        t = c->tickets[ticket & 63u].member;
    }
    HIP_TRY(hipSetDevice(c->cfg.device));
    HIP_TRY(hipEventSynchronize(t->ev_done));
    return GS_OK;
}
```

gaussian-splatting-wgpu_amd/csrc/gs_grade.hip:

```cpp
#include "gs_grade_math.h"
#include "gs_runtime.h"

GS_EXPORT int32_t gs_grade_compose(const float gain[3], const float offset[3], float saturation, float black, float white, float opacity_gain,
                                   gs_grade* out) {
    char msg[256] = "";
    const int32_t rc = gs_grade_compose_host(gain, offset, saturation, black, white, opacity_gain, out, msg, sizeof(msg));
    return rc == GS_OK ? GS_OK : fail(rc, "%s", msg);
}

GS_EXPORT int32_t gs_grade_splats(gs_ctx* c, uint32_t mask, uint32_t value, const gs_grade* g, uint64_t* matched) {
    const char* who = "gs_grade_splats";
    if (!c) return fail(GS_ERR_INVALID_ARGUMENT, "%s: null ctx", who);
    char msg[256] = "";
    if (gs_grade_validate_host(g, msg, sizeof(msg)) != GS_OK) return fail(GS_ERR_INVALID_ARGUMENT, "%s", msg);
    if (c->scene_mem && c->scene_mem != c->scene_own.get())
        return fail(GS_ERR_INVALID_ARGUMENT, "%s: this context borrows its splats (gs_share_splats): grade the owner", who);
    int32_t rc = resident_begin(c, who, Plane::filtered, mask, value);
    if (rc != GS_OK) return rc;
    const bool all = !(mask | value);
    uint64_t total = c->n;
    if (!all) {
        rc = edit_select(c, mask, value, g->flags != 0u, &total);
        if (rc != GS_OK) return rc;
    }
    gs_launch_grade(c->scene, c->n, all ? nullptr : c->ex.ids.get(), (uint32_t)total, *g, c->stream);
    HIP_TRY(hipGetLastError());
    HIP_TRY(hipStreamSynchronize(c->stream));
    if (matched) *matched = total;
    return GS_OK;
}
```

gaussian-splatting-wgpu_amd/csrc/gs_insert.hip:

```cpp
#include "gs_runtime.h"

static int32_t new_state_check(const char* who, uint32_t new_state) {
    if (new_state > 0xFFu) return fail(GS_ERR_INVALID_ARGUMENT, "%s: new_state 0x%x does not fit the state byte", who, new_state);
    return GS_OK;
}
static int32_t insert_check(gs_ctx* c, const char* who, uint32_t new_state, uint32_t mask = 0, uint32_t value = 0) {
    const int32_t rc = resident_check(c, who, Plane::filtered, mask, value);
    if (rc != GS_OK) return rc;
    if (new_state && !has_state(c)) return fail(GS_ERR_INVALID_ARGUMENT, "%s: the context was created without GS_FLAG_SPLAT_STATE (new_state must be 0)", who);
    if (c->scene_mem != c->scene_own.get())
        return fail(GS_ERR_INVALID_ARGUMENT, "%s: this context borrows its splats (gs_share_splats): insert into the owner", who);
    return GS_OK;
}
static int32_t insert_fits(const gs_ctx* c, const char* who, uint64_t m) {
    if (m >= (1ull << 31) || (uint64_t)c->n + m >= (1ull << 31))
        return fail(GS_ERR_INVALID_ARGUMENT, "%s: %u resident + %llu new splats reach the limit of 2^31", who, c->n, (unsigned long long)m);
    return GS_OK;
}

template <class Fill>
static int32_t insert_grow(gs_ctx* c, uint64_t m, uint32_t new_state, Fill fill) {
    const uint32_t n_old = c->n;
    const uint64_t n_new = (uint64_t)n_old + m;
    const bool state = has_state(c);
    DevBuf<> mem;
    HIP_TRY(hipMalloc(mem.out(), std::max<size_t>(scene_layout(nullptr, n_new, state).bytes, 256)));
    const GsScene dst = scene_layout(mem.get(), n_new, state).scene;
    gs_launch_grow(c->scene, n_old, dst, (uint32_t)n_new, new_state, c->opt.grid_persist * 2u, c->stream);
    HIP_TRY(hipGetLastError());
    int32_t rc = fill(dst);
    if (rc != GS_OK) return rc;
    HIP_TRY(hipGetLastError());
    HIP_TRY(hipStreamSynchronize(c->stream));
    drop_shadows(c);
    rc = scene_install(c, std::move(mem), n_new, c->capacity, c->row_cap);
    if (rc != GS_OK) return rc;
    HIP_TRY(hipStreamSynchronize(c->stream));
    return GS_OK;
}

static int32_t append_common(gs_ctx* c, const char* who, const void* aos, uint64_t m, uint32_t new_state, uint64_t* first, bool device) {
    int32_t rc = new_state_check(who, new_state);
    if (rc != GS_OK) return rc;
    if (!aos && m) return fail(GS_ERR_INVALID_ARGUMENT, "%s: null records", who);
    rc = insert_check(c, who, new_state);
    if (rc != GS_OK) return rc;
    rc = insert_fits(c, who, m);
    if (rc != GS_OK) return rc;
    rc = resident_drain(c);
    if (rc != GS_OK) return rc;
    const uint32_t n_old = c->n;
    if (m) {
        DevBuf<> bounce;
        const void* d_aos = aos;
        if (!device) {
            HIP_TRY(hipMalloc(bounce.out(), (size_t)m * GS_SPLAT_RECORD_BYTES));
            hipError_t e = hipMemcpy(bounce, aos, (size_t)m * GS_SPLAT_RECORD_BYTES, hipMemcpyHostToDevice);
            if (e != hipSuccess) return fail(GS_ERR_HIP, "%s: memcpy: %s", who, hipGetErrorString(e));
            d_aos = bounce;
        }
        rc = insert_grow(c, m, new_state, [&](const GsScene& dst) {
            gs_launch_repack(d_aos, (uint32_t)m, n_old, dst, c->stream);
            return (int32_t)GS_OK;
        });
        if (rc != GS_OK) return rc;
    }
    if (first) *first = n_old;
    return GS_OK;
}

GS_EXPORT int32_t gs_append_splats(gs_ctx* c, const void* aos320, uint64_t m, uint32_t new_state, uint64_t* first) {
    return append_common(c, "gs_append_splats", aos320, m, new_state, first, false);
}
GS_EXPORT int32_t gs_append_splats_device(gs_ctx* c, const void* d_aos320, uint64_t m, uint32_t new_state, uint64_t* first) {
    return append_common(c, "gs_append_splats_device", d_aos320, m, new_state, first, true);
}

template <class Source>
static int32_t append_source(const char* who, gs_ctx* c, const char* path, uint32_t new_state, uint64_t* first, uint64_t* m_out) {
    int32_t rc = new_state_check(who, new_state);
    if (rc != GS_OK) return rc;
    if (!path) return fail(GS_ERR_INVALID_ARGUMENT, "%s: null path", who);
    rc = insert_check(c, who, new_state);
    if (rc != GS_OK) return rc;
    Source src;
    rc = src.open(who, path);
    if (rc != GS_OK) return rc;
    const uint64_t m = src.count();
    rc = insert_fits(c, who, m);
    if (rc != GS_OK) return rc;
    rc = resident_drain(c);
    if (rc != GS_OK) return rc;
    const uint32_t n_old = c->n;
    if (m) {
        rc = insert_grow(c, m, new_state, [&](const GsScene& dst) { return src.stream(who, c, dst, n_old); });
        if (rc != GS_OK) return rc;
    }
    if (first) *first = n_old;
    if (m_out) *m_out = m;
    return GS_OK;
}
GS_EXPORT int32_t gs_append_ply(gs_ctx* c, const char* path, uint32_t new_state, uint64_t* first, uint64_t* m_out) {
    return append_source<PlySource>("gs_append_ply", c, path, new_state, first, m_out);
}
GS_EXPORT int32_t gs_append_packed(gs_ctx* c, const char* path, uint32_t new_state, uint64_t* first, uint64_t* m_out) {
    return append_source<PackSource>("gs_append_packed", c, path, new_state, first, m_out);
}

GS_EXPORT int32_t gs_duplicate_splats(gs_ctx* c, uint32_t mask, uint32_t value, uint32_t new_state, uint64_t* first, uint64_t* m_out,
                                      uint32_t* ids) {
    static const char who[] = "gs_duplicate_splats";
    int32_t rc = new_state_check(who, new_state);
    if (rc != GS_OK) return rc;
    rc = insert_check(c, who, new_state, mask, value);
    if (rc != GS_OK) return rc;
    rc = resident_drain(c);
    if (rc != GS_OK) return rc;
    const uint32_t n_old = c->n;
    uint64_t m = 0;
    rc = edit_select(c, mask, value, true, &m);
    if (rc != GS_OK) return rc;
    rc = insert_fits(c, who, m);
    if (rc != GS_OK) return rc;
    if (m) {
        rc = insert_grow(c, m, new_state, [&](const GsScene& dst) {
            gs_launch_compact_planes(c->scene, n_old, c->ex.ids, (uint32_t)m, dst, c->stream, n_old, false);
            return (int32_t)GS_OK;
        });
        if (rc != GS_OK) return rc;
        if (ids) HIP_TRY(hipMemcpy(ids, c->ex.ids, (size_t)m * 4, hipMemcpyDeviceToHost));
    }
    if (first) *first = n_old;
    if (m_out) *m_out = m;
    return GS_OK;
}
```

gaussian-splatting-wgpu_amd/csrc/gs_kernels.h:

```cpp
#pragma once
#include "gs_device.h"
#include "gs_consensus_host.h"
#include "gs_grid_math.h"

void gs_launch_repack(const void* d_aos, uint32_t n, uint32_t first, const GsScene& s, hipStream_t st);
void gs_launch_ply_chunk(const void* d_raw, uint32_t m, uint32_t first, const GsPlyTable& t, const GsScene& s, hipStream_t st);
struct GsPreprocessLaunch {
    const void* func;
    uint32_t blocks;
    GsScene s; GsUniforms u; GsFrame f;
    void* gdata; uint32_t* counts; GsTightOut to; GsTint tint;
    float w2;
    void* args[8];
};
float gs_view_norm2(const GsUniforms& u);
void gs_preprocess_prepare(GsPreprocessLaunch& L, const GsScene& s, const GsUniforms& u, const GsFrame& f, void* gdata, uint32_t* counts,
                           bool tight, uint32_t* arena, uint32_t* rowptr, unsigned short* unit_off, uint32_t* unit_n, GsControl* ctl,
                           uint32_t tight_nb = 0, bool state = false, GsTint tint = GsTint{});
void gs_launch_preprocess(GsPreprocessLaunch& L, hipStream_t st);
void gs_launch_zero(void* p, uint64_t bytes, hipStream_t st);
uint32_t gs_scan_blocks(uint32_t n);
void gs_launch_scan(const uint32_t* counts, uint32_t n, uint32_t* offsets, unsigned long long* status, uint32_t* ticket, GsControl* ctl,
                    hipStream_t st);
uint64_t gs_emit_chunks(uint64_t capacity);
void gs_launch_emit_balanced(const void* gdata, const void* grec, const uint32_t* chunk_table, const GsFrame& f, uint32_t* keys, uint32_t* values,
                             GsControl* ctl, uint32_t grid, uint32_t hist_bits, uint32_t hist_passes, bool keys16, hipStream_t st);
void gs_launch_emit(const void* gdata, const uint32_t* counts, const uint32_t* offsets, const GsFrame& f, uint32_t* keys, uint32_t* values,
                    GsControl* ctl, hipStream_t st);
void gs_launch_ranges16(const uint16_t* tiles, const GsControl* ctl, uint32_t capacity, uint32_t T, uint32_t* ranges, uint32_t grid,
                        uint32_t* sticky, GsReport* rep, hipStream_t st);
void gs_launch_rebuild_keys(const uint16_t* tiles, const uint32_t* vals, const uint32_t* counts, uint32_t count, uint32_t n, uint32_t* keys,
                            hipStream_t st);
void gs_launch_ranges(const uint32_t* keys, const GsControl* ctl, uint32_t capacity, uint32_t T, uint32_t* ranges, uint32_t grid,
                      uint32_t* sticky, GsReport* rep, hipStream_t st);
uint32_t gs_sort_tiles(uint64_t capacity);
struct GsSortPair { uint32_t *keys, *vals; };
struct GsSort {
    GsSortPair in, alt;
    uint32_t passes, bits, by_tile;
    bool keys16, have_hist;
};
GsSortPair gs_launch_sort(const GsSort& s, GsControl* ctl, uint32_t* status, uint32_t capacity, uint32_t grid, hipStream_t st);
struct GsLists {
    const void* gdata;
    const uint32_t* values;
    const uint32_t* ranges;
    GsFrame f;
    uint32_t id_mask;
    uint32_t nrec;
};
int gs_launch_blend(const GsLists& L, uint32_t* rgba8, float* rgbf, bool aux, float* alpha, float* depth, GsControl* ctl, uint32_t* tile_depth,
                    bool exact, uint32_t ablation, hipStream_t st, uint32_t* prof = nullptr, uint32_t* prof_blocks = nullptr);
void gs_launch_debug_view(const uint32_t* ranges, const GsFrame& f, uint32_t view, uint32_t* rgba8, hipStream_t st);
void gs_launch_assemble(const void* slabs, void* image, uint32_t width, uint32_t height, const uint32_t* d_px_bounds, uint32_t n_slabs,
                        uint64_t slab_stride_px, hipStream_t st);
uint32_t gs_gsort_tiles(uint32_t n);
uint64_t gs_gsort_scratch_bytes(uint32_t n);
void gs_launch_gsort(const uint32_t* words, const uint32_t* aux_in, const unsigned short* unit_off, const uint32_t* unit_n, uint32_t n, void* scratch,
                     void* grec, uint32_t* chunk_table, uint32_t chunk_cap, uint32_t* tot_visible, uint32_t* tot_quantity, uint32_t grid, hipStream_t st);
uint32_t gs_rows_sort_tiles(uint64_t row_cap);
uint32_t gs_rows_chunks(uint64_t row_cap);
size_t gs_rows_sorted_bytes(uint64_t row_cap);
void gs_launch_rows(const uint32_t* arena, const void* grec, const uint32_t* chunk_table, uint32_t* rows_sorted, GsControl* ctl, uint32_t* sort_status, uint32_t row_cap,
                    uint32_t* M3, uint32_t* tileoff, uint32_t* rowtot, const GsFrame& f, uint32_t* values, uint32_t* ranges, uint32_t cus,
                    uint32_t* sticky, GsReport* rep, hipStream_t st, void (*mark)(void*, int), void* mark_arg);
void gs_launch_rows_rebuild_keys(const uint32_t* ranges, uint32_t T, const uint32_t* vals, const void* gdata, uint32_t nrec, uint32_t count, uint32_t n,
                                 uint32_t* keys, hipStream_t st);
void gs_launch_rows_rebuild_taps(const uint32_t* vals, const void* gdata, uint32_t nrec, uint32_t count, uint32_t n, uint32_t* ids_out, void* gdata_out,
                                 hipStream_t st);
struct GsRegionDev {
    float a[3], b[3];
    float x0, y0, x1, y1;
    float W, H;
    uint32_t wi, hi;
    float proj[16];
    float viewz[4];
    const uint8_t* mask;
};
#define GS_STATE_SLOTS 32
#define GS_STATE_SLOT_STRIDE 32
void gs_launch_state_region(uint32_t kind, uint8_t* state, const GsScene& s, uint32_t n, const GsRegionDev& r, uint32_t op, uint32_t bits,
                            uint32_t where_mask, uint32_t where_value, unsigned long long* matched, hipStream_t st);
void gs_launch_state_ids(uint8_t* state, const uint32_t* ids, uint64_t n, uint32_t op, uint32_t bits, hipStream_t st);
void gs_launch_state_count(const uint8_t* state, uint32_t n, uint32_t mask, uint32_t value, unsigned long long* count, hipStream_t st);
void gs_launch_state_coverage(uint8_t* state, const void* planes, uint32_t n, uint32_t min_hits, float min_weight, uint32_t covered, uint32_t op,
                              uint32_t bits, uint32_t where_mask, uint32_t where_value, unsigned long long* matched, hipStream_t st);
void gs_launch_attr_state(uint32_t kind, uint8_t* state, const GsScene& s, const void* cov, uint32_t n, const GsAttrDev& a, float lo, float hi,
                          uint32_t inside, uint32_t op, uint32_t bits, uint32_t where_mask, uint32_t where_value, unsigned long long* matched,
                          hipStream_t st);
struct GsAttrSlot { unsigned long long matched, nan; uint32_t kmin, kmax; };
void gs_launch_attr_summary(uint32_t kind, const uint8_t* state, const GsScene& s, const void* cov, uint32_t n, const GsAttrDev& a, uint32_t mask,
                            uint32_t value, unsigned long long* slots, hipStream_t st);
void gs_launch_attr_histogram(uint32_t kind, const uint8_t* state, const GsScene& s, const void* cov, uint32_t n, const GsAttrDev& a, uint32_t mask,
                              uint32_t value, float lo, float hi, float scale, uint32_t bins, unsigned long long* counts, uint32_t grid, hipStream_t st);
void gs_launch_attr_values(uint32_t kind, const GsScene& s, const void* cov, uint32_t n, const GsAttrDev& a, const uint32_t* ids, uint32_t first,
                           uint32_t m, float* out, hipStream_t st);
#define GS_CONSENSUS_PAD 8u
void gs_launch_consensus(uint32_t kind, const uint8_t* state, const float* px, const float* py, const float* pz, uint32_t n, const float* params,
                         uint32_t hp, float lo, float hi, uint32_t mask, uint32_t value, unsigned long long* counts, unsigned long long* slots,
                         uint32_t grid, hipStream_t st);
#define GS_MOMENTS_SLOTS 8
#define GS_MOMENTS_SLOT_WORDS 192
void gs_launch_moments(uint32_t planes, const uint8_t* state, const float* p0, const float* p1, const float* p2, uint32_t n, uint32_t mask,
                       uint32_t value, unsigned long long* slots, uint32_t grid, hipStream_t st);
#define GS_PAIRS_SLOTS 8
#define GS_PAIRS_SLOT_WORDS 448
void gs_launch_pairs(const uint8_t* state, const float* px, const float* py, const float* pz, const uint32_t* partner, uint32_t n, uint32_t mask,
                     uint32_t value, float max_d2, unsigned long long* slots, uint32_t grid, hipStream_t st);
void gs_launch_neigh_bounds(const uint8_t* state, const GsScene& s, uint32_t n, uint32_t smask, uint32_t svalue, uint32_t qmask, uint32_t qvalue,
                            const uint32_t* gate, uint32_t* out, hipStream_t st);
void gs_launch_neigh_keys(const uint8_t* state, const GsScene& s, uint32_t n, uint32_t mask, uint32_t value, const uint32_t* gate, const GsNeighGrid& g,
                          uint32_t* keys, uint32_t* vals, hipStream_t st);
void gs_launch_neigh_records(const uint32_t* keys, const uint32_t* vals, uint32_t n, const GsNeighGrid& g, const GsScene& s, void* rec, uint32_t* skeys,
                             void* table, hipStream_t st);
void gs_launch_neigh_cands(const void* qrec, uint32_t nq, const void* srec, const uint32_t* skeys, const void* table, uint32_t nrec, const GsNeighGrid& g,
                           unsigned long long* sums, hipStream_t st);
void gs_launch_neigh_query(const void* qrec, uint32_t nq, uint32_t first_block, uint32_t blocks, const void* srec, const uint32_t* skeys, const void* table,
                           uint32_t nrec, const GsNeighGrid& g, float r2, uint32_t limit, uint32_t n, uint32_t* plane, hipStream_t st);
void gs_launch_state_neigh(uint8_t* state, const uint32_t* plane, uint32_t n, uint32_t min_count, uint32_t max_count, uint32_t inside, uint32_t op,
                           uint32_t bits, uint32_t where_mask, uint32_t where_value, unsigned long long* matched, hipStream_t st);
void gs_launch_cluster_init(const uint8_t* state, const GsScene& s, uint32_t n, uint32_t mask, uint32_t value, uint32_t* parent, uint32_t* count,
                            hipStream_t st);
void gs_launch_cluster_edges(const void* rec, uint32_t nrec, uint32_t first_block, uint32_t blocks, const uint32_t* skeys, const void* table,
                             const GsNeighGrid& g, float r2, uint32_t n, uint32_t* parent, uint32_t* changed, hipStream_t st);
void gs_launch_cluster_flatten(const void* rec, uint32_t nrec, uint32_t n, uint32_t* parent, hipStream_t st);
void gs_launch_cluster_sizes(const void* rec, uint32_t nrec, uint32_t n, const uint32_t* parent, uint32_t* count, bool fold, hipStream_t st);
void gs_launch_cluster_commit(const uint32_t* parent, const uint32_t* count, uint32_t n, uint32_t* labels, uint32_t* sizes, unsigned long long* slots,
                              hipStream_t st);
void gs_launch_cluster_seeds(const uint8_t* state, const uint32_t* labels, uint32_t n, uint32_t mask, uint32_t value, uint32_t* flag, hipStream_t st);
void gs_launch_state_cluster_linked(uint8_t* state, const uint32_t* labels, uint32_t n, const uint32_t* flag, uint32_t op, uint32_t bits, uint32_t where_mask,
                                    uint32_t where_value, unsigned long long* matched, hipStream_t st);
void gs_launch_knn_init(const uint8_t* state, uint32_t n, uint32_t mask, uint32_t value, uint32_t* dist2, uint32_t* nearest, hipStream_t st);
void gs_launch_knn_query(const void* qrec, uint32_t nq, uint32_t first_block, uint32_t blocks, const void* srec, const uint32_t* skeys, const void* table,
                         uint32_t nrec, const GsNeighGrid& g, float r2, uint32_t k, uint32_t n, uint32_t* dist2, uint32_t* nearest, uint32_t* unresolved,
                         hipStream_t st);
void gs_launch_state_knn(uint8_t* state, const uint32_t* dist2, uint32_t n, float lo, float hi, uint32_t inside, uint32_t op, uint32_t bits,
                         uint32_t where_mask, uint32_t where_value, unsigned long long* matched, hipStream_t st);
void gs_launch_surface_init(uint32_t n, void* nrm, void* eig, hipStream_t st);
void gs_launch_surface_query(const void* qrec, uint32_t nq, uint32_t first_block, uint32_t blocks, const void* srec, const uint32_t* skeys, const void* table,
                             uint32_t nrec, const GsNeighGrid& g, float r2, float scale, uint32_t n, int64_t* out, bool by_id, uint64_t word_stride,
                             uint32_t* unresolved, hipStream_t st);
void gs_launch_surface_finish(const void* qrec, uint32_t first, uint32_t count, uint32_t n, const int64_t* in, bool by_id, uint64_t word_stride,
                              double unscale, bool orient, const float toward[3], void* nrm, void* eig, hipStream_t st);
void gs_launch_surface_unpack(const void* rec, uint32_t n, float* xyz, uint32_t* w, hipStream_t st);
void gs_launch_state_surface(uint8_t* state, const void* plane, uint32_t n, uint32_t kind, float lo, float hi, uint32_t inside, const float axis[3], uint32_t op,
                             uint32_t bits, uint32_t where_mask, uint32_t where_value, unsigned long long* matched, hipStream_t st);
uint32_t gs_select_blocks(uint32_t n);
void gs_launch_select_count(const uint8_t* state, uint32_t n, uint32_t mask, uint32_t value, uint32_t* counts, hipStream_t st);
void gs_launch_select_scatter(const uint8_t* state, uint32_t n, uint32_t mask, uint32_t value, const uint32_t* offsets, uint32_t* ids, uint32_t cap,
                              hipStream_t st);
void gs_launch_unpack(const GsScene& s, uint32_t n, const uint32_t* ids, uint32_t first, uint32_t m, void* d_aos, uint32_t* out_ids, hipStream_t st);
void gs_launch_compact_planes(const GsScene& o, uint32_t n_old, const uint32_t* ids, uint32_t m, const GsScene& d, hipStream_t st, uint32_t first = 0,
                              bool with_state = true);
void gs_launch_grow(const GsScene& o, uint32_t n_old, const GsScene& d, uint32_t n_new, uint32_t new_state, uint32_t grid, hipStream_t st);
struct GsSnapshotDev {
    const uint32_t* ids;
    float *x, *y, *z;
    float4 *geo, *sh;
    uint32_t* state;
};
void gs_launch_snapshot(uint32_t mode, const GsScene& sc, uint32_t n, const GsSnapshotDev& s, uint32_t m, uint32_t parts, hipStream_t st);
void gs_launch_write(const void* d_aos, const uint8_t* d_states, uint32_t m, const uint32_t* ids, const GsScene& s, uint32_t n, uint32_t parts,
                     hipStream_t st);
void gs_launch_ids_ascending(const uint32_t* ids, uint64_t m, uint32_t n, unsigned long long* first_bad, hipStream_t st);
struct gs_xform;
void gs_launch_xform(const GsScene& s, uint32_t n, const uint32_t* ids, uint32_t m, const gs_xform& x, hipStream_t st);
struct gs_grade;
void gs_launch_grade(const GsScene& s, uint32_t n, const uint32_t* ids, uint32_t m, const gs_grade& x, hipStream_t st);
struct GsPackBox { float lo[3], hi[3]; };
void gs_launch_pack_keys(const GsScene& s, uint32_t n, const uint32_t* ids, uint32_t m, const GsPackBox& box, uint32_t* keys, uint32_t* vals,
                         hipStream_t st);
// ... 25 lines not shown
```

gaussian-splatting-wgpu_amd/csrc/gs_readback.hip:

```cpp
#include <cstddef>

#include "gs_runtime.h"
#include "gs_tight.h"

static int32_t tight_tap(gs_ctx* c, bool want_gdata) {
    if (want_gdata ? c->gdataG_valid : c->valsG_valid) return GS_OK;
    if (c->pending) { int32_t rc = wait_one(c); if (rc != GS_OK) return rc; }
    const uint64_t I = std::min<uint64_t>(c->h_rep->num_intersections, c->capacity);
    const GsLists L = frame_lists(c);
    const size_t gbytes = std::max<size_t>((size_t)c->n * 64, 256);
    if (want_gdata) {
        if (!c->gdataG) HIP_TRY(hipMalloc(c->gdataG.out(), gbytes));
        HIP_TRY(hipMemsetAsync(c->gdataG, 0, gbytes, c->stream));
    } else if (!c->valsG) HIP_TRY(hipMalloc(c->valsG.out(), (size_t)c->capacity * 4));
    gs_launch_rows_rebuild_taps(L.values, L.gdata, L.nrec, (uint32_t)I, c->n, want_gdata ? nullptr : c->valsG.get(),
                                want_gdata ? c->gdataG.get() : nullptr, c->stream);
    HIP_TRY(hipGetLastError());
    HIP_TRY(hipStreamSynchronize(c->stream));
    (want_gdata ? c->gdataG_valid : c->valsG_valid) = true;
    return GS_OK;
}

static int32_t tap(gs_ctx* c, int32_t which, void** ptr, uint64_t* bytes) {
    const FrameNotes& nt = c->notes;
    const uint64_t I = std::min<uint64_t>(c->h_rep->num_intersections, c->capacity);
    const uint64_t px = (uint64_t)c->frame.slab_w * c->frame.height;
    switch (which) {
    case GS_BUF_TILE_COUNTS: *ptr = c->counts; *bytes = (uint64_t)c->n * 4; return GS_OK;
    case GS_BUF_TILE_OFFSETS:
        if (!c->last_debug) return fail(GS_ERR_NO_FRAME, "the offsets tap needs gs_render_debug (index-order scan)");
        *ptr = c->offsets; *bytes = (uint64_t)c->n * 4; return GS_OK;
    case GS_BUF_GAUSSIAN_DATA:
        *bytes = (uint64_t)c->n * 64;
        if (!nt.last_tight) { *ptr = c->gdata; return GS_OK; }
        if (const int32_t rc = tight_tap(c, true); rc != GS_OK) return rc;
        *ptr = c->gdataG;
        return GS_OK;
    case GS_BUF_KEYS_UNSORTED:
    case GS_BUF_VALUES_UNSORTED:
        if (!c->last_debug || !c->keysU) return fail(GS_ERR_NO_FRAME, "unsorted taps need gs_render_debug");
        *ptr = which == GS_BUF_KEYS_UNSORTED ? c->keysU.get() : c->valsU.get(); *bytes = I * 4; return GS_OK;
    case GS_BUF_KEYS:
        *bytes = I * 4;
        if (!nt.last_keys16 && !nt.last_tight) { *ptr = nt.keysS; return GS_OK; }
        if (!c->keysG_valid) {
            if (c->pending) { int32_t rc = wait_one(c); if (rc != GS_OK) return rc; }
            if (!c->keysG) HIP_TRY(hipMalloc(c->keysG.out(), (size_t)c->capacity * 4));
            if (nt.last_tight) gs_launch_rows_rebuild_keys(c->ranges, c->T, nt.valsS, c->gdata, c->n + GS_RECORD_SLACK, (uint32_t)I, c->n, c->keysG, c->stream);
            else gs_launch_rebuild_keys((const uint16_t*)nt.keysS, nt.valsS, c->counts, (uint32_t)I, c->n, c->keysG, c->stream);
            HIP_TRY(hipStreamSynchronize(c->stream));
            c->keysG_valid = true;
        }
        *ptr = c->keysG;
        return GS_OK;
    case GS_BUF_VALUES:
    case GS_BUF_BLOCK_MASKS:
        *bytes = I * 4;
        if (!nt.last_tight) { *ptr = nt.valsS; return GS_OK; }
        if (const int32_t rc = tight_tap(c, false); rc != GS_OK) return rc;
        *ptr = c->valsG;
        return GS_OK;
    case GS_BUF_RANGES: *ptr = c->ranges; *bytes = (uint64_t)c->T * 4; return GS_OK;
    case GS_BUF_RGBA8: *ptr = c->last_ext ? c->last_ext : (void*)c->rgba8.get(); *bytes = px * 4; return GS_OK;
    case 12:
        *ptr = c->scene_mem; *bytes = c->scene_bytes; return GS_OK;
    case 11:
        if (!c->blend_prof) return fail(GS_ERR_INVALID_ARGUMENT, "no blend profile (GS_OPT_BLEND_ABLATION bit 16)");
        *ptr = c->blend_prof; *bytes = (uint64_t)c->blend_prof_blocks * 16; return GS_OK;
    case GS_BUF_RGB_F32:
        if (!c->rgbf) return fail(GS_ERR_INVALID_ARGUMENT, "GS_BUF_RGB_F32 needs GS_FLAG_F32_TAP");
        *ptr = c->rgbf; *bytes = px * 12; return GS_OK;
    case GS_BUF_ALPHA_F32:
    case GS_BUF_DEPTH_F32:
        if (!c->alpha || !c->depth)
            return fail(GS_ERR_INVALID_ARGUMENT, "%s needs GS_FLAG_AUX_OUTPUTS", which == GS_BUF_ALPHA_F32 ? "GS_BUF_ALPHA_F32" : "GS_BUF_DEPTH_F32");
        *ptr = which == GS_BUF_ALPHA_F32 ? c->alpha.get() : c->depth.get(); *bytes = px * 4; return GS_OK;
    default: return fail(GS_ERR_INVALID_ARGUMENT, "unknown buffer id %d", which);
    }
}

static int32_t state_tap(gs_ctx* c, void** ptr, uint64_t* bytes) {
    if (!has_state(c)) return fail(GS_ERR_INVALID_ARGUMENT, "GS_BUF_SPLAT_STATE needs GS_FLAG_SPLAT_STATE");
    if (!c->scene_mem || !c->scene.state) return fail(GS_ERR_NO_SCENE, "GS_BUF_SPLAT_STATE: no splats uploaded");
    *ptr = const_cast<uint8_t*>(c->scene.state);
    *bytes = c->n;
    return GS_OK;
}

int32_t last_frame(gs_ctx* root, const char* who, gs_ctx** out) {
    gs_ctx* c = last_of(root);
    if (who && !c->have_frame) return fail(GS_ERR_NO_FRAME, "%s: no frame rendered", who);
    if (c->pending) { int32_t rc = wait_one(c); if (rc != GS_OK) return rc; }
    HIP_TRY(hipSetDevice(c->cfg.device));
    *out = c;
    return GS_OK;
}

static int32_t size_protocol(uint64_t bytes, const void* dst, uint64_t size, uint64_t* written, bool* copy) {
    if (written) *written = bytes;
    *copy = dst != nullptr;
    if (dst && size < bytes) return fail(GS_ERR_INVALID_ARGUMENT, "gs_read_buffer: need %llu bytes, got %llu", (unsigned long long)bytes, (unsigned long long)size);
    return GS_OK;
}

GS_EXPORT int32_t gs_read_buffer(gs_ctx* c, int32_t which, void* dst, uint64_t size, uint64_t* written) {
    if (!c) return fail(GS_ERR_INVALID_ARGUMENT, "gs_read_buffer: null ctx");
    void* p = nullptr;
    uint64_t bytes = 0;
    bool copy = false;
    if (which == GS_BUF_SPLAT_STATE) {
        int32_t rc = state_tap(c, &p, &bytes);
        if (rc == GS_OK) rc = size_protocol(bytes, dst, size, written, &copy);
        if (rc != GS_OK || !copy) return rc;
        HIP_TRY(hipSetDevice(c->cfg.device));
        if (bytes) HIP_TRY(hipMemcpy(dst, p, bytes, hipMemcpyDeviceToHost));
        return GS_OK;
    }
    { int32_t rc = last_frame(c, "gs_read_buffer", &c); if (rc != GS_OK) return rc; }
    const GsLists L = frame_lists(c);
    const bool tight = c->notes.last_tight;
    const uint64_t I = std::min<uint64_t>(c->h_rep->num_intersections, c->capacity);
    const bool all_masks = which == GS_BUF_BLOCK_MASKS && !tight, list_counts = which == GS_BUF_TILE_COUNTS && tight;
    if (all_masks) bytes = I * 4;
    else if (list_counts) bytes = (uint64_t)c->n * 4;
    else { int32_t rc = tap(c, which, &p, &bytes); if (rc != GS_OK) return rc; }
    { int32_t rc = size_protocol(bytes, dst, size, written, &copy); if (rc != GS_OK || !copy) return rc; }
    uint32_t* w = (uint32_t*)dst;
    if (all_masks) {
        const uint32_t nb = (c->frame.tile_size / 8) * (c->frame.tile_size / 8);
        const uint32_t all = nb >= 32 ? 0xFFFFFFFFu : (1u << nb) - 1u;
        for (uint64_t i = 0; i < bytes / 4; ++i) w[i] = all;
        return GS_OK;
    }
    if (list_counts) {
        std::vector<uint32_t> v(I);
        uint64_t vbytes = 0;
        { int32_t rc = tap(c, GS_BUF_VALUES, &p, &vbytes); if (rc != GS_OK) return rc; }
        if (I) HIP_TRY(hipMemcpy(v.data(), p, I * 4, hipMemcpyDeviceToHost));
        memset(w, 0, bytes);
        for (uint64_t i = 0; i < I; ++i) { const uint32_t g = v[i] & L.id_mask; if (g < c->n) w[g]++; }
        return GS_OK;
    }
    if (bytes) HIP_TRY(hipMemcpy(dst, p, bytes, hipMemcpyDeviceToHost));
    if (which == GS_BUF_TILE_COUNTS)
        for (uint64_t i = 0; i < bytes / 4; ++i) w[i] &= GS_COUNT_MASK;
    if (which == GS_BUF_GAUSSIAN_DATA && !tight)
        for (uint64_t i = 0; i < bytes / 64; ++i) w[i * 16 + 2] = 0u;
    if (which == GS_BUF_VALUES && L.id_mask != 0xFFFFFFFFu)
        for (uint64_t i = 0; i < bytes / 4; ++i) w[i] &= L.id_mask;
    if (which == GS_BUF_BLOCK_MASKS) {
        const uint32_t ts = c->frame.tile_size;
        for (uint64_t i = 0; i < bytes / 4; ++i) {
            const uint32_t m = w[i] >> GS_ID_BITS;
            uint32_t out = m & (ts == 8 ? 1u : 0xFu);
            if (ts == 32) {
                out = 0;
                for (uint32_t by = 0; by < 4; ++by)
                    for (uint32_t bx = 0; bx < 4; ++bx)
                        if ((m >> ((by / 2) * 2 + bx / 2)) & 1u) out |= 1u << (by * 4 + bx);
            }
            w[i] = out;
        }
    }
    return GS_OK;
}

GS_EXPORT int32_t gs_read_rgba8(gs_ctx* c, void* dst, uint64_t size) {
    if (!dst) return fail(GS_ERR_INVALID_ARGUMENT, "gs_read_rgba8: null destination");
    return gs_read_buffer(c, GS_BUF_RGBA8, dst, size, nullptr);
}

GS_EXPORT int32_t gs_device_ptr(gs_ctx* c, int32_t which, void** d_ptr) {
    if (!c || !d_ptr) return fail(GS_ERR_INVALID_ARGUMENT, "gs_device_ptr: null argument");
    uint64_t bytes = 0;
    if (which == GS_BUF_SPLAT_STATE) return state_tap(c, d_ptr, &bytes);
    c = last_of(c);
    if (which == GS_BUF_RGBA8) { *d_ptr = c->rgba8; return GS_OK; }
    if (!c->have_frame) return fail(GS_ERR_NO_FRAME, "gs_device_ptr: no frame rendered");
    return tap(c, which, d_ptr, &bytes);
}

static void stage_times(const gs_ctx* c, gs_stats* out) {
    if (!c->have_events || c->frames == 0) return;
    const uint64_t last = c->frames - 1;
    uint64_t first = c->timed_from;
    if (last + 1 > GS_EV_RING && first < last + 1 - GS_EV_RING) first = last + 1 - GS_EV_RING;
    if (first > last) first = last;
    double sum[GS_STAGE_COUNT + 1] = {0};
    uint32_t cnt = 0;
    for (uint64_t fr = first; fr <= last; ++fr) {
        const Event* e = c->ev[fr % GS_EV_RING];
        float ms = 0, tot = 0;
        bool ok = true;
        float st[GS_STAGE_COUNT];
        for (int i = 0; i < GS_STAGE_COUNT && ok; ++i) {
            ok = hipEventElapsedTime(&ms, e[i], e[i + 1]) == hipSuccess;
            st[i] = ms * 1000.0f;
        }
        ok = ok && hipEventElapsedTime(&tot, e[0], e[GS_STAGE_COUNT]) == hipSuccess;
        if (!ok) continue;
        for (int i = 0; i < GS_STAGE_COUNT; ++i) sum[i] += st[i];
        sum[GS_STAGE_COUNT] += tot * 1000.0f;
        ++cnt;
        if (fr == last) {
            for (int i = 0; i < GS_STAGE_COUNT; ++i) out->stage_us[i] = st[i];
            out->frame_us = tot * 1000.0f;
        }
    }
    out->frames_timed = cnt;
    if (cnt) {
        for (int i = 0; i < GS_STAGE_COUNT; ++i) out->stage_us_mean[i] = (float)(sum[i] / cnt);
        out->frame_us_mean = (float)(sum[GS_STAGE_COUNT] / cnt);
    }
}

GS_EXPORT int32_t gs_get_stats(gs_ctx* root, gs_stats* out) {
    if (!root || !out) return fail(GS_ERR_INVALID_ARGUMENT, "gs_get_stats: null argument");
    gs_ctx* c = nullptr;
    { int32_t rc = last_frame(root, nullptr, &c); if (rc != GS_OK) return rc; }
    const FrameNotes& nt = c->notes;
    memset(out, 0, sizeof(*out));
    out->num_gaussians = c->n;
    out->num_tiles = c->T;
    out->sort_passes = nt.last_passes ? nt.last_passes : c->passes;
    out->frames = over_ring(root, [](const gs_ctx* m) { return m->frames; });
    out->depth_ordered = (c->have_frame && !nt.last_by_index) ? 1u : 0u;
    if (c->have_frame) {
        if (!c->h_ctl_valid) {
            HIP_TRY(hipMemcpy(c->h_ctl, c->ctl, offsetof(GsControl, hist), hipMemcpyDeviceToHost));
            c->h_ctl_valid = true;
        }
        out->num_visible = c->h_rep->num_visible;
        out->num_intersections = c->h_rep->num_intersections;
        out->capacity = c->capacity;
        out->max_intersections_seen = std::max<uint64_t>(c->max_I_seen, c->h_rep->num_intersections);
        out->truncated_frames = over_ring(root, [](const gs_ctx* m) { return m->truncated_frames; });
        out->frames_in_flight = (uint32_t)root->shadows.size() + 1u;
        out->graph_frames = over_ring(root, [](const gs_ctx* m) { return m->gr.frames; });
        out->tight_binning = nt.last_tight ? 1u : 0u;
        out->row_capacity = c->row_cap;
        if (nt.last_tight) {
            out->num_row_items = c->h_rep->num_items;
            out->num_row_slots = c->h_rep->num_slots;
        }
        for (int k = 0; k < 64; ++k) out->num_processed += c->h_ctl->num_processed[k];
        if (nt.blend_walkers >= 4) {
            std::vector<uint32_t> depth(c->T);
            if (hipMemcpy(depth.data(), c->tile_depth, (size_t)c->T * 4, hipMemcpyDeviceToHost) == hipSuccess)
                for (uint32_t v : depth) out->num_processed += v;
        }
        for (int k = 0; k < 64; ++k) out->num_evaluated += c->h_ctl->num_evaluated[k];
        stage_times(c, out);
    }
    return GS_OK;
}

GS_EXPORT int32_t gs_pick(gs_ctx* root, const gs_pick_query* queries, uint32_t n, gs_pick_result* results, uint32_t max_contrib,
                          gs_pick_contrib* contrib) {
    static_assert(sizeof(gs_pick_query) == 8 && sizeof(gs_pick_result) == 48 && sizeof(gs_pick_contrib) == 8, "gs_pick record layouts");
    if (!root || !queries || !results) return fail(GS_ERR_INVALID_ARGUMENT, "gs_pick: null argument");
    if (n == 0 || n > GS_PICK_MAX_QUERIES) return fail(GS_ERR_INVALID_ARGUMENT, "gs_pick: n must be 1..%u (got %u)", GS_PICK_MAX_QUERIES, n);
    if (max_contrib > GS_PICK_MAX_CONTRIB) return fail(GS_ERR_INVALID_ARGUMENT, "gs_pick: max_contrib must be at most %u (got %u)", GS_PICK_MAX_CONTRIB, max_contrib);
    if ((contrib != nullptr) != (max_contrib != 0))
        return fail(GS_ERR_INVALID_ARGUMENT, "gs_pick: contrib and max_contrib must be given together (contrib %s, max_contrib %u)",
                    contrib ? "set" : "null", max_contrib);
    for (uint32_t i = 0; i < n; ++i)
        if (queries[i].x >= root->frame.width || queries[i].y >= root->frame.height)
            return fail(GS_ERR_INVALID_ARGUMENT, "gs_pick: query %u: pixel (%u, %u) is outside the %u x %u canvas", i, queries[i].x, queries[i].y,
                        root->frame.width, root->frame.height);
    gs_ctx* c = nullptr;
    int32_t rc = last_frame(root, "gs_pick", &c);
    if (rc != GS_OK) return rc;
    auto& pk = root->pick;
    if (!pk.q) HIP_TRY(hipMalloc(pk.q.out(), (size_t)GS_PICK_MAX_QUERIES * sizeof(gs_pick_query)));
    if (!pk.r) HIP_TRY(hipMalloc(pk.r.out(), (size_t)GS_PICK_MAX_QUERIES * sizeof(gs_pick_result)));
    const uint64_t cbytes = (uint64_t)n * max_contrib * sizeof(gs_pick_contrib);
    rc = pk.c.reserve(cbytes);
    if (rc != GS_OK) return rc;
    HIP_TRY(hipMemcpyAsync(pk.q, queries, (size_t)n * sizeof(gs_pick_query), hipMemcpyHostToDevice, c->stream));
    gs_launch_pick(frame_lists(c), pk.q, n, pk.r, max_contrib, max_contrib ? pk.c.get() : nullptr, c->stream);
// ... 26 lines not shown
```

gaussian-splatting-wgpu_amd/csrc/gs_runtime.h:

```cpp
#pragma once
#include <hip/hip_runtime.h>

#include <algorithm>
#include <cstdint>
#include <cstdio>
#include <cstring>
#include <mutex>
#include <vector>

#include "../../include/gsplat/gs_abi.h"
#include "gs_kernels.h"
#include "gs_pack_host.h"

#define GS_EXPORT extern "C" __attribute__((visibility("default")))

extern thread_local char g_err[512];
int32_t fail(int32_t code, const char* fmt, ...) __attribute__((format(printf, 2, 3)));
#define HIP_TRY(expr)                                                                                       \
    do {                                                                                                    \
        hipError_t e_ = (expr);                                                                             \
        if (e_ != hipSuccess)                                                                               \
            return fail(e_ == hipErrorOutOfMemory ? GS_ERR_OUT_OF_MEMORY : GS_ERR_HIP, "%s: %s", #expr,      \
                        hipGetErrorString(e_));                                                             \
    } while (0)

template <class P, auto Destroy>
struct Owned {
    P p = nullptr;
    Owned() = default;
    explicit Owned(P q) : p(q) {}
    Owned(const Owned&) = delete;
    Owned& operator=(const Owned&) = delete;
    Owned(Owned&& o) noexcept : p(o.p) { o.p = nullptr; }
    Owned& operator=(Owned&& o) noexcept { if (this != &o) { reset(); p = o.p; o.p = nullptr; } return *this; }
    ~Owned() { reset(); }
    void reset() { if (p) { (void)Destroy(p); p = nullptr; } }
    P* out() { reset(); return &p; }
    P get() const { return p; }
    operator P() const { return p; }
    P operator->() const { return p; }
};
template <class T = void> using DevBuf = Owned<T*, hipFree>;
template <class T = void> using PinnedBuf = Owned<T*, hipHostFree>;
template <class T>
struct Scratch : DevBuf<T> {
    uint64_t cap = 0;
    int32_t reserve(uint64_t count) {
        if (count <= cap) return GS_OK;
        cap = 0;
        HIP_TRY(hipMalloc(this->out(), (size_t)count * sizeof(T)));
        cap = count;
        return GS_OK;
    }
};
using Event = Owned<hipEvent_t, hipEventDestroy>;
using Stream = Owned<hipStream_t, hipStreamDestroy>;
using File = Owned<FILE*, fclose>;

struct FrameNotes {
    uint32_t *keysS = nullptr, *valsS = nullptr;
    uint32_t last_passes = 0;
    uint32_t blend_walkers = 1;
    bool last_by_index = true;
    bool last_keys16 = false;
    bool last_tight = false;
};

struct GraphKey {
    bool index = false, tight = false;
    void* ext = nullptr;
    float *alpha = nullptr, *depth = nullptr;
    bool operator==(const GraphKey& o) const { return index == o.index && tight == o.tight && ext == o.ext && alpha == o.alpha && depth == o.depth; }
};

struct GsOptions {
    int emit_order = 2;
    uint32_t debug_view = 0;
    bool tile_cull = true;
    uint32_t tight_nb = 0;
    uint32_t blend_ablation = 0;
    uint32_t select_tint = 0x80FFFF00u;
    uint32_t grid_persist = 0;
    bool frame_graph = false;
};

#define GS_EV_RING 256
struct gs_ctx {
    ~gs_ctx();
    gs_config cfg{};
    Stream own_stream;
    hipStream_t stream = nullptr;
    GsFrame frame{};
    uint32_t T = 0, passes = 0, key_bits = 0;
    uint32_t tile_passes = 0, tile_bits = 0;
    bool tile16 = false;
    bool tight_ok = false;
    GsOptions opt;
    DevBuf<uint32_t> blend_prof;
    uint32_t blend_prof_blocks = 0;
    uint32_t fif = 1;
    std::vector<gs_ctx*> shadows;
    bool is_shadow = false;
    gs_ctx* last = nullptr;
    uint32_t rr = 0;
    uint64_t cap_hint = 0, row_hint = 0;
    Event ev_done;
    uint64_t next_ticket = 1;
    struct { uint64_t ticket; gs_ctx* member; } tickets[64] = {};
    std::mutex ticket_mu;
    DevBuf<> scene_own;
    void* scene_mem = nullptr;
    size_t scene_bytes = 0;
    GsScene scene{};
    uint32_t n = 0;
    uint64_t scene_serial = 0;
    DevBuf<uint32_t> counts, offsets, rowptr;
    DevBuf<unsigned short> unit_off;
    DevBuf<uint32_t> unit_n;
    DevBuf<> gdata;
    DevBuf<> grec;
    DevBuf<> gsort_scratch;
    uint64_t capacity = 0;
    DevBuf<uint32_t> keysA, valsA, keysB, valsB;
    GsSort sort_index{}, sort_tile{};
    DevBuf<uint32_t> keysU, valsU;
    DevBuf<uint32_t> keysG;
    bool keysG_valid = false;
    DevBuf<uint32_t> valsG;
    DevBuf<> gdataG;
    bool valsG_valid = false, gdataG_valid = false;
    DevBuf<uint32_t> chunk_table;
    uint64_t row_cap = 0;
    DevBuf<uint32_t> arena, rows_sorted, M3;
    DevBuf<uint32_t> tileoff, rowtot;
    DevBuf<> ctl_mem;
    size_t ctl_bytes = 0;
    size_t ctl_bytes_tight = 0;
    GsControl* ctl = nullptr;
    uint32_t* tile_depth = nullptr;
    uint32_t* rows_status = nullptr;
    unsigned long long* scan_status = nullptr;
    uint32_t* sort_status = nullptr;
    PinnedBuf<GsControl> h_ctl;
    bool h_ctl_valid = false;
    PinnedBuf<GsReport> h_rep;
    DevBuf<uint32_t> sticky;
    uint64_t max_I_seen = 0;
    uint64_t truncated_frames = 0;
    DevBuf<uint32_t> ranges, rgba8;
    DevBuf<float> rgbf;
    DevBuf<float> alpha, depth;
    DevBuf<uint32_t> d_pxb;
    uint32_t pxb_host[65] = {};
    uint32_t pxb_n = 0;
    struct { DevBuf<> q, r; Scratch<uint8_t> c; } pick;
    struct { DevBuf<unsigned long long> counter; Scratch<uint32_t> ids; Scratch<uint8_t> mask; } st;
    struct { Scratch<uint32_t> counts, ids; } ex;
    struct { DevBuf<unsigned long long> slots; Scratch<unsigned long long> hist; Scratch<float> vals; } at;
    struct { DevBuf<unsigned long long> counts; DevBuf<float> params; Scratch<uint32_t> ids; } cs;
    struct { DevBuf<unsigned long long> slots; Scratch<float> vals[3]; } mo;
    struct { DevBuf<unsigned long long> slots; Scratch<uint32_t> partner; } pr;
    DevBuf<> cov;
    struct Neigh {
        DevBuf<uint32_t> plane;
        Scratch<uint32_t> keysA, valsA, keysB, valsB, skeys, bounds;
        Scratch<uint8_t> ctl, src, qry, table;
        Scratch<unsigned long long> sums;
        uint32_t n32 = 0;
    } ng;
    struct Cluster { DevBuf<uint32_t> label, size; } cl;
    struct Knn { DevBuf<uint32_t> dist2, nearest; uint32_t k = 0; } kn;
    struct Surface {
        DevBuf<> nrm, eig;
        DevBuf<int64_t> sums;
        bool have_sums = false;
        Scratch<int64_t> slice;
        Scratch<uint32_t> out;
    } sf;
    struct { Scratch<uint8_t> flags, member, rec; Scratch<uint32_t> counts, heads, mruns, ids, group_of, stats; Scratch<double> sums; } mg;
    Event ev[GS_EV_RING][GS_STAGE_COUNT + 1];
    bool have_events = false;
    uint64_t timed_from = 0;
    struct {
        bool valid = false;
        hipGraph_t graph = nullptr;
        hipGraphExec_t exec = nullptr;
        hipGraphNode_t pre_node = nullptr;
        GraphKey key;
        FrameNotes notes;
        uint64_t frames = 0;
    } gr;
    GsPreprocessLaunch pre{};
    FrameNotes notes;
    bool have_frame = false, pending = false, last_debug = false;
    void* last_ext = nullptr;
    GsUniforms last_u{};
    uint64_t frames = 0;
};

int32_t alloc_kv(gs_ctx* c, uint64_t capacity, uint64_t row_cap);
int32_t scene_alloc(gs_ctx* c, uint64_t n, uint64_t min_capacity = 0, uint64_t min_rows = 0);
struct GsSceneLayout {
    GsScene scene{};
    size_t np = 0, state_at = 0, bytes = 0;
};
GsSceneLayout scene_layout(void* base, uint64_t n, bool state);
int32_t scene_install(gs_ctx* c, DevBuf<>&& mem, uint64_t n, uint64_t min_capacity, uint64_t min_rows);
uint64_t scene_new_serial();
void drop_shadows(gs_ctx* c);
void drop_graph(gs_ctx* c);
int32_t wait_one(gs_ctx* c);
GsLists frame_lists(const gs_ctx* c);
template <class Get>
uint64_t over_ring(const gs_ctx* root, Get get, bool maximum = false) {
    uint64_t v = get(root);
    for (const gs_ctx* s : root->shadows) v = maximum ? std::max<uint64_t>(v, get(s)) : v + get(s);
    return v;
}
enum class Plane {
    none,
    filtered,
    always
};
int32_t resident_check(gs_ctx* c, const char* who, Plane need, uint32_t mask = 0, uint32_t value = 0);
int32_t resident_drain(gs_ctx* c, bool counter = false);
inline int32_t resident_begin(gs_ctx* c, const char* who, Plane need, uint32_t mask = 0, uint32_t value = 0) {
    const int32_t rc = resident_check(c, who, need, mask, value);
    return rc != GS_OK ? rc : resident_drain(c);
}
int32_t stage_mask(gs_ctx* root, const uint8_t* mask, hipStream_t st, const uint8_t** dev);
int32_t last_frame(gs_ctx* root, const char* who, gs_ctx** c);
int32_t cover_planes(gs_ctx* root, hipStream_t st);
int32_t neigh_plane(gs_ctx* c, hipStream_t st);
size_t plane_bytes(const gs_ctx* c);
struct NeighBuilt {
    GsNeighGrid g{};
    const uint8_t* state = nullptr;
    uint64_t sources = 0, queried = 0;
    uint32_t nsrc = 0, nqry = 0;
    bool grid = false;
    float cell_edge = 0.0f;
    const void* qrec = nullptr;
    std::vector<unsigned long long> sums;
    uint64_t candidates = 0;
};
int32_t neigh_check_radius(const char* who, float radius, float* r2);
int32_t neigh_build(gs_ctx* c, const char* who, float radius, uint32_t smask, uint32_t svalue, uint32_t qmask, uint32_t qvalue, NeighBuilt* b,
                    const uint32_t* gate = nullptr);
int32_t neigh_budget(const char* who, uint64_t candidates, uint64_t max_candidates, float radius);
template <class Launch>
void neigh_slices(const std::vector<unsigned long long>& sums, Launch launch) {
    const uint32_t nblocks = (uint32_t)sums.size();
    for (uint32_t b0 = 0; b0 < nblocks;) {
        uint64_t sum = sums[b0];
        uint32_t b1 = b0 + 1u;
        while (b1 < nblocks && sum + sums[b1] <= GS_NEIGH_SLICE_CANDIDATES) sum += sums[b1++];
        launch(b0, b1 - b0);
        b0 = b1;
    }
}
int32_t neigh_bounds(gs_ctx* c, const uint8_t* state, uint32_t smask, uint32_t svalue, uint32_t qmask, uint32_t qvalue, uint32_t hb[16],
                     const uint32_t* gate = nullptr);
static constexpr size_t kCtlBytes = (sizeof(GsControl) + 255) & ~(size_t)255;
inline size_t private_sort_bytes(uint64_t n, uint32_t passes) { return kCtlBytes + (size_t)passes * gs_sort_tiles(n) * 256 * 4; }
inline GsSort private_sort_plan(uint32_t* keysA, uint32_t* valsA, uint32_t* keysB, uint32_t* valsB, uint32_t passes) {
    return GsSort{{keysA, valsA}, {keysB, valsB}, passes, 8, 0, false, false};
}
inline int32_t private_sort_reserve(gs_ctx* c, uint32_t n, uint32_t passes) {
    gs_ctx::Neigh& s = c->ng;
    int32_t rc;
    if ((rc = s.keysA.reserve(n)) != GS_OK || (rc = s.valsA.reserve(n)) != GS_OK || (rc = s.keysB.reserve(n)) != GS_OK ||
        (rc = s.valsB.reserve(n)) != GS_OK)
        return rc;
    return s.ctl.reserve(private_sort_bytes(n, passes));
}
template <class Keys>
int32_t private_sort(gs_ctx* c, uint32_t n, uint32_t passes, Keys keys, GsSortPair* sorted) {
    gs_ctx::Neigh& s = c->ng;
    const int32_t rc = private_sort_reserve(c, n, passes);
    if (rc != GS_OK) return rc;
    HIP_TRY(hipMemsetAsync(s.ctl, 0, private_sort_bytes(n, passes), c->stream));
    GsControl* ctl = (GsControl*)s.ctl.get();
    s.n32 = n;
    HIP_TRY(hipMemcpyAsync(&ctl->num_intersections, &s.n32, 4, hipMemcpyHostToDevice, c->stream));
    keys();
    *sorted = gs_launch_sort(private_sort_plan(s.keysA, s.valsA, s.keysB, s.valsB, passes), ctl, (uint32_t*)(s.ctl.get() + kCtlBytes), n,
                             std::max(c->opt.grid_persist, 1u), c->stream);
    return GS_OK;
}
inline int32_t private_sort_fault(gs_ctx* c, uint32_t* fault) {
    HIP_TRY(hipMemcpyAsync(fault, &((const GsControl*)c->ng.ctl.get())->fault, 4, hipMemcpyDeviceToHost, c->stream));
    return GS_OK;
}
int32_t cluster_planes(gs_ctx* c, hipStream_t st);
int32_t knn_planes(gs_ctx* c, hipStream_t st);
int32_t surface_planes(gs_ctx* c, hipStream_t st);
int32_t edit_select(gs_ctx* c, uint32_t mask, uint32_t value, bool want_ids, uint64_t* total);
static constexpr uint64_t kBounceRecords = 1ull << 20;
struct PlyLayout {
    uint64_t data_off = 0, vertex_count = 0;
    uint32_t stride = 0;
    int degree = 0, nsrc = 0;
    uint32_t soff[11 + 48], stype[11 + 48], slot[11 + 48];
    bool all_float = true;
};
static constexpr uint64_t kStreamTrip = 65536;
struct PlySource {
    File fp;
    PlyLayout L;
    int32_t open(const char* who, const char* path);
    uint64_t count() const { return L.vertex_count; }
    int32_t stream(const char* who, gs_ctx* c, const GsScene& dst, uint64_t first);
};
struct PackSource {
    File fp;
    GsPackLayout L;
    int32_t open(const char* who, const char* path);
    uint64_t count() const { return L.n; }
    int32_t stream(const char* who, gs_ctx* c, const GsScene& dst, uint64_t first);
};
template <class Source>
int32_t upload_source(const char* who, gs_ctx* c, const char* path, uint64_t* n_out) {
    if (!c || !path) return fail(GS_ERR_INVALID_ARGUMENT, "%s: null argument", who);
    Source src;
    int32_t rc = src.open(who, path);
    if (rc != GS_OK) return rc;
    hipError_t he = hipSetDevice(c->cfg.device);
    if (he != hipSuccess) return fail(GS_ERR_HIP, "hipSetDevice: %s", hipGetErrorString(he));
    drop_shadows(c);
    rc = scene_alloc(c, src.count());
    if (rc != GS_OK) return rc;
    rc = src.stream(who, c, c->scene, 0);
    if (rc != GS_OK) return rc;
    if (n_out) *n_out = src.count();
    return GS_OK;
}
struct TripRing {
    PinnedBuf<unsigned char> h[2];
    DevBuf<unsigned char> d[2];
    Event done[2];
    int32_t init(size_t bytes, bool device) {
        for (int k = 0; k < 2; ++k) {
            HIP_TRY(hipHostMalloc(h[k].out(), bytes, hipHostMallocDefault));
            if (device) HIP_TRY(hipMalloc(d[k].out(), bytes));
            HIP_TRY(hipEventCreateWithFlags(done[k].out(), hipEventDisableTiming));
        }
        return GS_OK;
    }
    template <class Trip>
    int32_t feed(uint64_t trips, hipStream_t st, Trip trip) {
        for (uint64_t it = 0; it < trips; ++it) {
            const int k = (int)(it & 1u);
            if (it >= 2) HIP_TRY(hipEventSynchronize(done[k]));
            const int32_t rc = trip(it, h[k].get(), d[k].get());
            if (rc != GS_OK) return rc;
            HIP_TRY(hipEventRecord(done[k], st));
        }
        return GS_OK;
    }
    template <class Enqueue, class Consume>
    int32_t drain(uint64_t trips, hipStream_t st, Enqueue enqueue, Consume consume) {
        for (uint64_t it = 0; it <= trips && trips; ++it) {
            int32_t rc;
            if (it < trips) {
                if ((rc = enqueue(it, h[it & 1u].get())) != GS_OK) return rc;
                HIP_TRY(hipEventRecord(done[it & 1u], st));
            }
            if (it >= 1) {
                HIP_TRY(hipEventSynchronize(done[(it - 1) & 1u]));
                if ((rc = consume(it - 1, h[(it - 1) & 1u].get())) != GS_OK) return rc;
            }
        }
        return GS_OK;
    }
};
int32_t attr_check(const char* who, const gs_attr* a, GsAttrDev* dev);
inline bool attr_needs_cover(const gs_attr* a) { return a->kind >= GS_ATTR_COVER_HITS; }
inline gs_ctx* last_of(gs_ctx* c) { return (c && c->last) ? c->last : c; }
inline bool has_state(const gs_ctx* c) { return (c->cfg.flags & GS_FLAG_SPLAT_STATE) != 0; }
inline GsTint tint_of(uint32_t argb) {
    return GsTint{{(float)((argb >> 16) & 255u) / 255.0f, (float)((argb >> 8) & 255u) / 255.0f, (float)(argb & 255u) / 255.0f},
                  (float)(argb >> 24) / 255.0f};
}
```

gaussian-splatting-wgpu_amd/csrc/gs_snapshot.hip:

```cpp
#include <memory>
#include <new>

#include "gs_runtime.h"

static constexpr uint32_t kAllParts = GS_PART_RECORD | GS_PART_STATE;

static int32_t snap_check(gs_ctx* c, const char* who, const char* verb, uint32_t parts, bool filtered = false, uint32_t mask = 0, uint32_t value = 0) {
    if (!c) return fail(GS_ERR_INVALID_ARGUMENT, "%s: null ctx", who);
    if (c->scene_mem && c->scene_mem != c->scene_own.get())
        return fail(GS_ERR_INVALID_ARGUMENT, "%s: this context borrows its splats (gs_share_splats): %s the owner", who, verb);
    const int32_t rc = resident_check(c, who, filtered ? Plane::filtered : Plane::none, mask, value);
    if (rc != GS_OK) return rc;
    if ((parts & GS_PART_STATE) && !has_state(c))
        return fail(GS_ERR_INVALID_ARGUMENT, "%s: the context was created without GS_FLAG_SPLAT_STATE (GS_PART_STATE needs the plane)", who);
    return GS_OK;
}
static int32_t parts_check(const char* who, uint32_t parts) {
    if (parts & ~kAllParts) return fail(GS_ERR_INVALID_ARGUMENT, "%s: unknown part bits 0x%x", who, parts & ~kAllParts);
    return GS_OK;
}

static int32_t id_check(const char* who, uint64_t p, bool have_prev, uint32_t prev, uint32_t id, uint32_t n) {
    if (id >= n) return fail(GS_ERR_INVALID_ARGUMENT, "%s: ids[%llu] = %u is not a splat (N = %u)", who, (unsigned long long)p, id, n);
    if (have_prev && prev >= id)
        return fail(GS_ERR_INVALID_ARGUMENT, "%s: ids[%llu] = %u does not exceed ids[%llu] = %u: the ids must be strictly ascending", who,
                    (unsigned long long)p, id, (unsigned long long)(p - 1), prev);
    return GS_OK;
}
static int32_t ids_check_host(const char* who, const uint32_t* ids, uint64_t m, uint32_t n) {
    for (uint64_t p = 0; p < m; ++p) {
        const int32_t rc = id_check(who, p, p > 0, p > 0 ? ids[p - 1] : 0u, ids[p], n);
        if (rc != GS_OK) return rc;
    }
    return GS_OK;
}
static int32_t ids_check_device(gs_ctx* c, const char* who, const uint32_t* d_ids, uint64_t m) {
    unsigned long long bad = ~0ull;
    HIP_TRY(hipMemsetAsync(c->st.counter, 0xFF, sizeof(bad), c->stream));
    gs_launch_ids_ascending(d_ids, m, c->n, c->st.counter, c->stream);
    HIP_TRY(hipGetLastError());
    HIP_TRY(hipMemcpyAsync(&bad, c->st.counter, sizeof(bad), hipMemcpyDeviceToHost, c->stream));
    HIP_TRY(hipStreamSynchronize(c->stream));
    if (bad == ~0ull) return GS_OK;
    uint32_t pair[2] = {0u, 0u};
    const uint64_t from = bad ? bad - 1 : 0;
    HIP_TRY(hipMemcpy(pair + (bad ? 0 : 1), d_ids + from, bad ? 8 : 4, hipMemcpyDeviceToHost));
    const int32_t rc = id_check(who, bad, bad > 0, pair[0], pair[1], c->n);
    return rc != GS_OK ? rc : fail(GS_ERR_INVALID_ARGUMENT, "%s: ids[%llu] is out of order", who, bad);
}

static int32_t write_common(gs_ctx* c, const char* who, const uint32_t* ids, uint64_t m, const void* aos, const uint8_t* states, uint32_t parts,
                            uint64_t* written, bool device) {
    int32_t rc = parts_check(who, parts);
    if (rc != GS_OK) return rc;
    if ((parts & GS_PART_RECORD) && !aos && m) return fail(GS_ERR_INVALID_ARGUMENT, "%s: null records", who);
    if ((parts & GS_PART_STATE) && !states && m) return fail(GS_ERR_INVALID_ARGUMENT, "%s: null states (GS_PART_STATE reads one byte per record)", who);
    rc = snap_check(c, who, "write to", parts);
    if (rc != GS_OK) return rc;
    if (m > c->n)
        return fail(GS_ERR_INVALID_ARGUMENT, "%s: m = %llu records, the scene holds %u splats%s", who, (unsigned long long)m, c->n,
                    ids ? " (the ids must be strictly ascending)" : " (ids == NULL writes splats 0 .. m)");
    if (ids && !device) {
        rc = ids_check_host(who, ids, m, c->n);
        if (rc != GS_OK) return rc;
    }
    rc = resident_drain(c, device && ids != nullptr && m != 0);
    if (rc != GS_OK) return rc;
    if (written) *written = 0;
    if (!m || !parts) return GS_OK;
    const bool rec = (parts & GS_PART_RECORD) != 0, st = (parts & GS_PART_STATE) != 0;
    if (device) {
        if (ids) {
            rc = ids_check_device(c, who, ids, m);
            if (rc != GS_OK) return rc;
        }
        gs_launch_write(aos, states, (uint32_t)m, ids, c->scene, c->n, parts, c->stream);
        HIP_TRY(hipGetLastError());
        HIP_TRY(hipStreamSynchronize(c->stream));
        if (written) *written = m;
        return GS_OK;
    }
    const uint64_t trip = std::min(m, kBounceRecords);
    const size_t rec_bytes = rec ? (size_t)trip * GS_SPLAT_RECORD_BYTES : 0, ids_bytes = ids ? (size_t)trip * 4 : 0;
    DevBuf<> bounce;
    HIP_TRY(hipMalloc(bounce.out(), std::max<size_t>(rec_bytes + ids_bytes + (st ? (size_t)trip : 0), 256)));
    char* const d_rec = (char*)bounce.get();
    uint32_t* const d_ids = (uint32_t*)(d_rec + rec_bytes);
    uint8_t* const d_st = (uint8_t*)(d_rec + rec_bytes + ids_bytes);
    for (uint64_t first = 0; first < m; first += kBounceRecords) {
        const uint64_t k = std::min(kBounceRecords, m - first);
        if (rec) HIP_TRY(hipMemcpyAsync(d_rec, (const char*)aos + first * GS_SPLAT_RECORD_BYTES, (size_t)k * GS_SPLAT_RECORD_BYTES, hipMemcpyHostToDevice, c->stream));
        if (ids) HIP_TRY(hipMemcpyAsync(d_ids, ids + first, (size_t)k * 4, hipMemcpyHostToDevice, c->stream));
        if (st) HIP_TRY(hipMemcpyAsync(d_st, states + first, (size_t)k, hipMemcpyHostToDevice, c->stream));
        GsScene s = c->scene;
        uint32_t n = c->n;
        if (!ids) {
            s.px += first; s.py += first; s.pz += first; s.smax += first; s.geo += 2 * first; s.sh += 12 * first;
            if (s.state) s.state += first;
            n -= (uint32_t)first;
        }
        gs_launch_write(d_rec, d_st, (uint32_t)k, ids ? d_ids : nullptr, s, n, parts, c->stream);
        HIP_TRY(hipGetLastError());
        HIP_TRY(hipStreamSynchronize(c->stream));
    }
    if (written) *written = m;
    return GS_OK;
}

GS_EXPORT int32_t gs_write_splats(gs_ctx* c, const uint32_t* ids, uint64_t m, const void* aos320, const uint8_t* states, uint32_t parts, uint64_t* written) {
    return write_common(c, "gs_write_splats", ids, m, aos320, states, parts, written, false);
}
GS_EXPORT int32_t gs_write_splats_device(gs_ctx* c, const uint32_t* d_ids, uint64_t m, const void* d_aos320, const uint8_t* d_states, uint32_t parts,
                                         uint64_t* written) {
    return write_common(c, "gs_write_splats_device", d_ids, m, d_aos320, d_states, parts, written, true);
}

struct gs_snapshot {
    int device = 0;
    uint64_t serial = 0;
    uint64_t count = 0, n_at_take = 0;
    uint32_t parts = 0;
    bool dense = false;
    size_t bytes = 0;
    DevBuf<> mem;
    GsSnapshotDev dev{};
};
static size_t snapshot_layout(char* base, uint64_t m, uint32_t parts, bool dense, GsSnapshotDev* d) {
    const size_t m4 = ((size_t)m + 3) & ~(size_t)3;
    size_t off = 0;
    *d = GsSnapshotDev{};
    if (!dense) { d->ids = (const uint32_t*)(base + off); off += m4 * 4; }
    if (parts & GS_PART_POSITION) {
        d->x = (float*)(base + off); off += m4 * 4;
        d->y = (float*)(base + off); off += m4 * 4;
        d->z = (float*)(base + off); off += m4 * 4;
    }
    if (parts & GS_PART_GEOMETRY) { d->geo = (float4*)(base + off); off += (size_t)m * 32; }
    if (parts & GS_PART_SH) { d->sh = (float4*)(base + off); off += (size_t)m * 192; }
    if (parts & GS_PART_STATE) { d->state = (uint32_t*)(base + off); off += m4; }
    return off;
}

GS_EXPORT int32_t gs_snapshot_take(gs_ctx* c, uint32_t mask, uint32_t value, uint32_t parts, gs_snapshot** out) {
    static const char who[] = "gs_snapshot_take";
    if (!out) return fail(GS_ERR_INVALID_ARGUMENT, "%s: null out", who);
    int32_t rc = parts_check(who, parts);
    if (rc != GS_OK) return rc;
    rc = snap_check(c, who, "snapshot", parts, true, mask, value);
    if (rc != GS_OK) return rc;
    rc = resident_drain(c);
    if (rc != GS_OK) return rc;
    const bool all = !(mask | value);
    uint64_t total = c->n;
    if (!all) {
        rc = edit_select(c, mask, value, true, &total);
        if (rc != GS_OK) return rc;
    }
    std::unique_ptr<gs_snapshot> s(new (std::nothrow) gs_snapshot);
    if (!s) return fail(GS_ERR_OUT_OF_MEMORY, "%s: out of host memory", who);
    s->device = c->cfg.device;
    s->serial = c->scene_serial;
    s->count = total;
    s->n_at_take = c->n;
    s->parts = parts;
    s->dense = all;
    GsSnapshotDev d;
    s->bytes = total ? snapshot_layout(nullptr, total, parts, all, &d) : 0;
    if (s->bytes) {
        HIP_TRY(hipMalloc(s->mem.out(), s->bytes));
        snapshot_layout((char*)s->mem.get(), total, parts, all, &s->dev);
        if (!all) HIP_TRY(hipMemcpyAsync(const_cast<uint32_t*>(s->dev.ids), c->ex.ids, (size_t)total * 4, hipMemcpyDeviceToDevice, c->stream));
        gs_launch_snapshot(0u, c->scene, c->n, s->dev, (uint32_t)total, parts, c->stream);
        HIP_TRY(hipGetLastError());
        HIP_TRY(hipStreamSynchronize(c->stream));
    }
    *out = s.release();
    return GS_OK;
}

static int32_t apply_common(gs_ctx* c, const gs_snapshot* s, uint32_t parts, uint64_t* moved, uint32_t mode, const char* who) {
    if (!s) return fail(GS_ERR_INVALID_ARGUMENT, "%s: null snapshot", who);
    int32_t rc = parts_check(who, parts);
    if (rc != GS_OK) return rc;
    if (!parts) parts = s->parts;
    if (parts & ~s->parts) return fail(GS_ERR_INVALID_ARGUMENT, "%s: part bits 0x%x were not taken (the snapshot holds 0x%x)", who, parts & ~s->parts, s->parts);
    rc = snap_check(c, who, mode == 1u ? "restore" : "swap with", parts);
    if (rc != GS_OK) return rc;
    if (c->scene_serial != s->serial)
        return fail(GS_ERR_INVALID_ARGUMENT,
                    "%s: the snapshot was taken from scene serial %llu, the context holds serial %llu: the scene was replaced or renumbered "
                    "(another context, an upload or a compaction since)",
                    who, (unsigned long long)s->serial, (unsigned long long)c->scene_serial);
    rc = resident_drain(c);
    if (rc != GS_OK) return rc;
    const bool work = s->count && parts;
    if (work) {
        gs_launch_snapshot(mode, c->scene, c->n, s->dev, (uint32_t)s->count, parts, c->stream);
        HIP_TRY(hipGetLastError());
        HIP_TRY(hipStreamSynchronize(c->stream));
    }
    if (moved) *moved = work ? s->count : 0;
    return GS_OK;
}
GS_EXPORT int32_t gs_snapshot_restore(gs_ctx* c, const gs_snapshot* s, uint32_t parts, uint64_t* restored) {
    return apply_common(c, s, parts, restored, 1u, "gs_snapshot_restore");
}
GS_EXPORT int32_t gs_snapshot_swap(gs_ctx* c, gs_snapshot* s, uint32_t parts, uint64_t* swapped) {
    return apply_common(c, s, parts, swapped, 2u, "gs_snapshot_swap");
}

GS_EXPORT int32_t gs_snapshot_get_info(const gs_snapshot* s, gs_snapshot_info* out) {
    if (!s) return fail(GS_ERR_INVALID_ARGUMENT, "gs_snapshot_get_info: null snapshot");
    if (!out) return fail(GS_ERR_INVALID_ARGUMENT, "gs_snapshot_get_info: null out");
    out->count = s->count;
    out->n_at_take = s->n_at_take;
    out->device_bytes = s->bytes;
    out->parts = s->parts;
    out->dense = s->dense ? 1u : 0u;
    return GS_OK;
}

GS_EXPORT int32_t gs_snapshot_free(gs_snapshot* s) {
    if (!s) return GS_OK;
    if (s->mem) (void)hipSetDevice(s->device);
    delete s;
    return GS_OK;
}
```

gaussian-splatting-wgpu_amd/csrc/gs_xform.hip:

```cpp
#include <cmath>

#include "gs_runtime.h"
#include "gs_xform_math.h"

GS_EXPORT int32_t gs_xform_compose(const float rot_rxyz[4], const float translate[3], float scale, const float pivot[3], gs_xform* out) {
    char msg[256] = "";
    const int32_t rc = gs_xform_compose_host(rot_rxyz, translate, scale, pivot, out, msg, sizeof(msg));
    return rc == GS_OK ? GS_OK : fail(rc, "%s", msg);
}

static bool all_finite(const float* v, int n) {
    for (int k = 0; k < n; ++k)
        if (!std::isfinite(v[k])) return false;
    return true;
}

GS_EXPORT int32_t gs_transform_splats(gs_ctx* c, uint32_t mask, uint32_t value, const gs_xform* x, uint64_t* matched) {
    const char* who = "gs_transform_splats";
    if (!c) return fail(GS_ERR_INVALID_ARGUMENT, "%s: null ctx", who);
    if (!x) return fail(GS_ERR_INVALID_ARGUMENT, "%s: null xform", who);
    if (x->struct_size != sizeof(gs_xform)) return fail(GS_ERR_INVALID_ARGUMENT, "%s: struct_size %u != %zu", who, x->struct_size, sizeof(gs_xform));
    if (x->flags & ~(GS_XFORM_POSITION | GS_XFORM_ORIENT | GS_XFORM_SIZE)) return fail(GS_ERR_INVALID_ARGUMENT, "%s: unknown flag bits 0x%x", who, x->flags);
    if ((x->flags & GS_XFORM_POSITION) && !all_finite(x->m, 12)) return fail(GS_ERR_INVALID_ARGUMENT, "%s: m has a non-finite entry", who);
    if ((x->flags & GS_XFORM_ORIENT) && !(all_finite(x->q, 4) && all_finite(x->sh1, 9) && all_finite(x->sh2, 25) && all_finite(x->sh3, 49)))
        return fail(GS_ERR_INVALID_ARGUMENT, "%s: q or a band matrix has a non-finite entry", who);
    if ((x->flags & GS_XFORM_SIZE) && !std::isfinite(x->log_scale)) return fail(GS_ERR_INVALID_ARGUMENT, "%s: log_scale is not finite", who);
    if (c->scene_mem && c->scene_mem != c->scene_own.get())
        return fail(GS_ERR_INVALID_ARGUMENT, "%s: this context borrows its splats (gs_share_splats): transform the owner", who);
    int32_t rc = resident_begin(c, who, Plane::filtered, mask, value);
    if (rc != GS_OK) return rc;
    const bool all = !(mask | value);
    uint64_t total = c->n;
    if (!all) {
        rc = edit_select(c, mask, value, x->flags != 0u, &total);
        if (rc != GS_OK) return rc;
    }
    gs_launch_xform(c->scene, c->n, all ? nullptr : c->ex.ids.get(), (uint32_t)total, *x, c->stream);
    HIP_TRY(hipGetLastError());
    HIP_TRY(hipStreamSynchronize(c->stream));
    if (matched) *matched = total;
    return GS_OK;
}
```

gaussian-splatting-wgpu_amd/csrc/k_preprocess.hip:

```cpp
#include "gs_device.h"
#include "gs_kernels.h"
#include "gs_tight.h"

__global__ __launch_bounds__(256) void gs_repack_kernel(const float4* __restrict__ aos, uint32_t n, uint32_t first, float* px, float* py,
                                                         float* pz, float* smax, float* geo, float* sh) {
    const uint64_t t = (uint64_t)blockIdx.x * 256 + threadIdx.x;
    const uint64_t total = (uint64_t)n * 20;
    if (t >= total) return;
    const uint32_t g = first + (uint32_t)(t / 20), c = (uint32_t)(t % 20);
    const float4 v = aos[t];
    float* r = geo + (uint64_t)g * 8;
    if (c == 0) { px[g] = v.x; py[g] = v.y; pz[g] = v.z; }
    else if (c == 1) { r[0] = v.x; r[1] = v.y; r[2] = v.z; smax[g] = __builtin_fmaxf(v.x, __builtin_fmaxf(v.y, v.z)); }
    else if (c == 2) { r[4] = v.x; r[5] = v.y; r[6] = v.z; r[7] = v.w; }
    else if (c == 3) { r[3] = v.x; }
    else {
        const uint32_t k = c - 4;
        float* q = sh + (uint64_t)g * 48 + 3 * k;
        q[0] = v.x;
        q[1] = v.y;
        q[2] = v.z;
    }
}

__global__ __launch_bounds__(256) void gs_ply_chunk_kernel(const unsigned char* __restrict__ raw, uint32_t m, uint32_t first, GsPlyTable t,
                                                            float* px, float* py, float* pz, float* smax, float* geo, float* sh) {
    const uint64_t id = (uint64_t)blockIdx.x * 256 + threadIdx.x;
    if (id >= (uint64_t)m * t.nsrc) return;
    const uint32_t v = (uint32_t)(id / t.nsrc), k = (uint32_t)(id % t.nsrc);
    const unsigned char* src = raw + (uint64_t)v * t.stride;
    auto rd = [&](uint32_t kk) {
        const unsigned char* q = src + t.soff[kk];
        if (t.stype[kk] == 1u) {
            uint32_t w;
            if (t.all_float) w = *reinterpret_cast<const uint32_t*>(q);
            else w = (uint32_t)q[0] | ((uint32_t)q[1] << 8) | ((uint32_t)q[2] << 16) | ((uint32_t)q[3] << 24);
            return __uint_as_float(w);
        }
        if (t.stype[kk] == 2u) return (float)((double)q[0] / 255.0);
        return 0.0f;
    };
    const uint64_t g = (uint64_t)first + v;
    const uint32_t slot = t.slot[k];
    const float val = rd(k);
    if (slot == 0u) px[g] = val;
    else if (slot == 1u) py[g] = val;
    else if (slot == 2u) pz[g] = val;
    else if (slot >= 4u && slot <= 6u) {
        geo[g * 8 + (slot - 4u)] = val;
        if (slot == 4u) smax[g] = __builtin_fmaxf(val, __builtin_fmaxf(rd(4), rd(5)));
    } else if (slot >= 8u && slot <= 11u) geo[g * 8 + 4u + (slot - 8u)] = val;
    else if (slot == 12u) geo[g * 8 + 3u] = val;
    else {
        const uint32_t kk = (slot - 16u) >> 2, ch = (slot - 16u) & 3u;
        sh[g * 48 + 3u * kk + ch] = val;
    }
}
void gs_launch_ply_chunk(const void* d_raw, uint32_t m, uint32_t first, const GsPlyTable& t, const GsScene& s, hipStream_t st) {
    const uint64_t total = (uint64_t)m * t.nsrc;
    if (!total) return;
    hipLaunchKernelGGL(gs_ply_chunk_kernel, dim3((uint32_t)((total + 255) / 256)), dim3(256), 0, st, (const unsigned char*)d_raw, m, first, t,
                       (float*)s.px, (float*)s.py, (float*)s.pz, (float*)s.smax, (float*)s.geo, (float*)s.sh);
}

struct M3 { float m[3][3]; };
__device__ __forceinline__ M3 m3_mul(const M3& A, const M3& B) {
    M3 o;
#pragma unroll
    for (int c = 0; c < 3; ++c)
#pragma unroll
        for (int r = 0; r < 3; ++r) o.m[c][r] = (A.m[0][r] * B.m[c][0] + A.m[1][r] * B.m[c][1]) + A.m[2][r] * B.m[c][2];
    return o;
}
__device__ __forceinline__ M3 m3_t(const M3& A) {
    M3 o;
#pragma unroll
    for (int c = 0; c < 3; ++c)
#pragma unroll
        for (int r = 0; r < 3; ++r) o.m[c][r] = A.m[r][c];
    return o;
}
__device__ __forceinline__ void m4_mulv(const float* m, float x, float y, float z, float* o) {
#pragma unroll
    for (int r = 0; r < 4; ++r) o[r] = ((m[0 + r] * x + m[4 + r] * y) + m[8 + r] * z) + m[12 + r] * 1.0f;
}

__device__ __forceinline__ float sigmoid_ref(float o) {
    const float ez = gs_exp(o);
    const float cond = (o >= 0.0f) ? 1.0f : 0.0f;
    return (cond * (1.0f / (1.0f + gs_exp(-o)))) + ((1.0f - cond) * (ez / (1.0f + ez)));
}

__device__ __forceinline__ void sh_colour(const float4* __restrict__ sh, float x, float y, float z, const GsUniforms& u, float col[3]) {
    const float dx = x - u.cam[0], dy = y - u.cam[1], dz = z - u.cam[2];
    const float dl = __builtin_sqrtf((dx * dx + dy * dy) + dz * dz);
    const float X = dx / dl, Y = dy / dl, Z = dz / dl;
    const float xx = X * X, yy = Y * Y, zz = Z * Z, xy = X * Y, xz = X * Z, yz = Y * Z;
    float k[16];
    k[4] = 1.0925484305920792f * xy;
    k[5] = -1.0925484305920792f * yz;
    k[6] = 0.31539156525252005f * ((2.f * zz - xx) - yy);
    k[7] = -1.0925484305920792f * xz;
    k[8] = 0.5462742152960396f * (xx - yy);
    k[9] = (-0.5900435899266435f * Y) * (3.f * xx - yy);
    k[10] = (2.890611442640554f * xy) * Z;
    k[11] = (-0.4570457994644658f * Y) * ((4.f * zz - xx) - yy);
    k[12] = (0.3731763325901154f * Z) * ((2.f * zz - 3.f * xx) - 3.f * yy);
    k[13] = (-0.4570457994644658f * X) * ((4.f * zz - xx) - yy);
    k[14] = (1.445305721320277f * Z) * (xx - yy);
    k[15] = (-0.5900435899266435f * X) * (xx - 3.f * yy);
    float shv[48];
#pragma unroll
    for (int p = 0; p < 12; ++p) {
#ifdef PRE_ABLATE_SH
        const float4 vv = make_float4(X, Y, Z, 0.5f);
#else
        const float4 vv = sh[p];
#endif
        shv[4 * p + 0] = vv.x; shv[4 * p + 1] = vv.y; shv[4 * p + 2] = vv.z; shv[4 * p + 3] = vv.w;
    }
#pragma unroll
    for (int c = 0; c < 3; ++c) {
        float res = 0.28209479177387814f * shv[c];
        res = res + 0.4886025119029199f * ((((-Y) * shv[3 + c]) + Z * shv[6 + c]) - X * shv[9 + c]);
#pragma unroll
        for (int j = 4; j < 16; ++j) res = res + k[j] * shv[3 * j + c];
        res = res + 0.5f;
        col[c] = wg_max(res, 0.0f);
    }
}

__device__ __forceinline__ bool in_frustum_slab(const GsUniforms& u, const GsFrame& f, float w2, float x, float y, float z, float smax_log) {
    float ph[4], pv[4];
    m4_mulv(u.proj, x, y, z, ph);
    const float pw = 1.0f / (ph[3] + 0.0000001f);
    const float ndx = ph[0] * pw, ndy = ph[1] * pw;
    m4_mulv(u.view, x, y, z, pv);
    if ((pv[2] <= 0.2f) || (ndx <= -1.1f || ndx >= 1.1f || ndy <= -1.1f || ndy >= 1.1f)) return false;
    if (f.full) return true;
    const float sm = __expf(smax_log) * u.scale_modifier * 1.001f;
    const float limx = 1.3f * u.tan_fovx, limy = 1.3f * u.tan_fovy;
    const float iz = 1.0f / pv[2];
    const float jf2 = ((u.focal_x * iz) * (u.focal_x * iz) * (1.0f + limx * limx) + (u.focal_y * iz) * (u.focal_y * iz) * (1.0f + limy * limy)) * w2;
    const float rb = 3.0f * __builtin_sqrtf(2.0f * jf2 * sm * sm + 0.92f) * 1.001f + 2.0f;
    const float pxs = ((ndx * 0.5f) + 0.5f) * (float)f.width;
    const float ts = (float)f.tile_size;
    const float lo = pxs - rb, hi = pxs + rb;
    const bool reach = (lo < (float)f.col1 * ts) && (f.col0 == 0u || hi >= (float)f.col0 * ts);
    const bool alias = (f.col0 == 0u) && (hi >= (float)f.ntx * ts);
    return (reach || alias) || !(rb == rb);
}

#ifdef GS_PROFILING
__device__ unsigned long long gs_pre_prof[256][16];
extern "C" __attribute__((visibility("default"))) int gs_prof_preprocess(unsigned long long* out8, int reset) {
    static unsigned long long h[256][16];
    if (out8) {
        if (hipMemcpyFromSymbol(h, HIP_SYMBOL(gs_pre_prof), sizeof(h)) != hipSuccess) return -1;
        for (int k = 0; k < 8; ++k) { out8[k] = 0; for (int c = 0; c < 256; ++c) out8[k] += h[c][k]; }
    }
    if (reset) { for (auto& r : h) for (auto& v : r) v = 0; if (hipMemcpyToSymbol(HIP_SYMBOL(gs_pre_prof), h, sizeof(h)) != hipSuccess) return -1; }
    return 0;
}
#define PRE_STAMP(k) do { const uint32_t t_ = (uint32_t)__builtin_amdgcn_readfirstlane((int)(uint32_t)__builtin_amdgcn_s_memtime()); \
                          pacc[k] = (uint32_t)__builtin_amdgcn_readfirstlane((int)(pacc[k] + (t_ - tprev))); tprev = t_; } while (0)
#else
#define PRE_STAMP(k) do { } while (0)
#endif
#define PRE_G 512
#ifndef PRE_WAVES
#define PRE_WAVES 4
#endif
typedef uint32_t gs_row_u32x3 __attribute__((ext_vector_type(3), aligned(4)));


template <bool TIGHT, int NB, bool STATE>
__global__ __launch_bounds__(256, PRE_WAVES) void gs_preprocess_kernel(GsScene s, GsUniforms u, GsFrame f, uint4* __restrict__ gdata,
                                                             uint32_t* __restrict__ tile_counts, GsTightOut to, GsTint tint, float w2) {
    __shared__ uint32_t s_ids[PRE_G * NB];
    constexpr bool KEEP_POS = NB == 2;
    __shared__ float s_pos[3][KEEP_POS ? PRE_G * NB : 1];
    __shared__ uint32_t s_cnt[2][4];
    __shared__ uint32_t s_misc[8];
    __shared__ alignas(16) uint32_t s_rc[TIGHT ? 2 * NB : 1][4];
    __shared__ uint32_t s_ust[TIGHT ? 4 : 1];
    __shared__ float4 s_tA[TIGHT ? 256 : 1], s_tB[TIGHT ? 256 : 1], s_tC[TIGHT ? 256 : 1];
    __shared__ uint32_t s_mark[TIGHT ? 256 : 1], s_tcnt[TIGHT ? 256 : 1], s_tgid[TIGHT ? 256 : 1];
    __shared__ uint32_t s_tw[4];
    __shared__ uint32_t s_rowhist[TIGHT ? 256 : 1];
    const uint32_t tid = threadIdx.x, lane = tid & 63, w = tid >> 6;
    const uint32_t bid = blockIdx.x;
    const uint32_t base = bid * (PRE_G * NB);
    if (TIGHT) s_rowhist[tid] = 0u;
#ifdef GS_PROFILING
    uint32_t pacc[5] = {0, 0, 0, 0, 0};
    uint32_t tprev = (uint32_t)__builtin_amdgcn_readfirstlane((int)(uint32_t)__builtin_amdgcn_s_memtime());
#endif

    uint32_t nvis = 0;
    if (NB > 1) {
        if (!TIGHT) {
            if (tid == 0) s_misc[1] = 0u;
            __syncthreads();
        }
        uint32_t carried = 0;
        constexpr int GRP = 2 * NB < 8 ? 2 * NB : 8;
#pragma unroll 1
        for (int h = 0; h < 2 * NB / GRP; ++h) {
            float X[GRP], Y[GRP], Z[GRP], S[GRP];
            uint32_t B[GRP];
#pragma unroll
            for (int k = 0; k < GRP; ++k) {
                const uint32_t i = base + (uint32_t)(h * GRP + k) * 256u + tid;
                const uint32_t ic = i < f.n ? i : f.n - 1u;
                X[k] = s.px[ic]; Y[k] = s.py[ic]; Z[k] = s.pz[ic];
                S[k] = 0.0f;
                B[k] = STATE ? (uint32_t)s.state[ic] : 0u;
            }
            if (!f.full) {
#pragma unroll
                for (int k = 0; k < GRP; ++k) {
                    const uint32_t i = base + (uint32_t)(h * GRP + k) * 256u + tid;
                    S[k] = s.smax[i < f.n ? i : f.n - 1u];
                }
            }
            __builtin_amdgcn_sched_barrier(0);
            if (TIGHT) {
                uint32_t vm = 0;
#pragma unroll
                for (int k = 0; k < GRP; ++k) {
                    const uint32_t i = base + (uint32_t)(h * GRP + k) * 256u + tid;
                    bool v = false;
                    if (i < f.n) {
                        v = in_frustum_slab(u, f, w2, X[k], Y[k], Z[k], S[k]);
                        if (STATE && (B[k] & GS_ST_HIDDEN)) v = false;
                    }
                    vm |= (v ? 1u : 0u) << k;
                    const uint32_t c = (uint32_t)__popcll(__ballot(v));
                    if (lane == 0) s_rc[h * GRP + k][w] = c;
                }
                __syncthreads();
#pragma unroll
                for (int k = 0; k < GRP; ++k) {
                    const uint4 c = make_uint4(s_rc[h * GRP + k][0], s_rc[h * GRP + k][1], s_rc[h * GRP + k][2], s_rc[h * GRP + k][3]);
                    const bool v = (vm >> k) & 1u;
                    const unsigned long long b = __ballot(v);
                    if (v) {
                        const uint32_t off = (uint32_t)(h * GRP + k) * 256u + tid;
                        const uint32_t slot = carried + (w > 0 ? c.x : 0u) + (w > 1 ? c.y : 0u) + (w > 2 ? c.z : 0u) + (uint32_t)__popcll(b & ((1ull << lane) - 1ull));
                        s_ids[slot] = STATE ? (off | (B[k] << 16)) : off;
                        if (KEEP_POS) { s_pos[0][slot] = X[k]; s_pos[1][slot] = Y[k]; s_pos[2][slot] = Z[k]; }
                    }
                    carried += (c.x + c.y) + (c.z + c.w);
                }
                continue;
            }
#pragma unroll
            for (int k = 0; k < GRP; ++k) {
                const uint32_t off = (uint32_t)(h * GRP + k) * 256u + tid;
                const uint32_t i = base + off;
                bool v = false;
                if (i < f.n) {
                    v = in_frustum_slab(u, f, w2, X[k], Y[k], Z[k], S[k]);
                    if (STATE && (B[k] & GS_ST_HIDDEN)) v = false;
                    if (!v) tile_counts[i] = 0u;
                }
                const unsigned long long b = __ballot(v);
                if (b) {
                    uint32_t at = 0;
                    if (lane == (uint32_t)__builtin_ctzll(b)) at = atomicAdd(&s_misc[1], (uint32_t)__popcll(b));
                    at = (uint32_t)__builtin_amdgcn_readlane((int)at, __builtin_ctzll(b));
                    if (v) {
                        const uint32_t slot = at + (uint32_t)__popcll(b & ((1ull << lane) - 1ull));
                        s_ids[slot] = STATE ? (off | (B[k] << 16)) : off;
                        if (KEEP_POS) { s_pos[0][slot] = X[k]; s_pos[1][slot] = Y[k]; s_pos[2][slot] = Z[k]; }
                    }
                }
            }
        }
        if (TIGHT && tid < NB / 2) {
            uint32_t first = 0, cnt = 0;
#pragma unroll
            for (int r = 0; r < 2 * NB; ++r) {
                const uint4 c = make_uint4(s_rc[r][0], s_rc[r][1], s_rc[r][2], s_rc[r][3]);
                const uint32_t t = (c.x + c.y) + (c.z + c.w);
                if (r < 4 * (int)tid) first += t;
                else if (r < 4 * (int)tid + 4) cnt += t;
            }
            s_ust[tid] = first;
            const uint32_t un = bid * (NB / 2) + tid;
            if (un < ((f.n + 1023u) >> 10)) to.unit_n[un] = cnt;
        }
        __syncthreads();
        nvis = TIGHT ? carried : s_misc[1];
    } else {
        bool vis[2];
        uint32_t sb[2] = {0u, 0u};
        unsigned long long bal[2];
#pragma unroll
        for (int k = 0; k < 2; ++k) {
            const uint32_t i = base + k * 256 + tid;
            vis[k] = false;
            if (i < f.n) {
                vis[k] = in_frustum_slab(u, f, w2, s.px[i], s.py[i], s.pz[i], f.full ? 0.0f : s.smax[i]);
                if (STATE) {
                    sb[k] = (uint32_t)s.state[i];
                    if (sb[k] & GS_ST_HIDDEN) vis[k] = false;
                }
                if (!vis[k]) tile_counts[i] = 0u;
            }
            bal[k] = __ballot(vis[k]);
            if (lane == 0) s_cnt[k][w] = (uint32_t)__popcll(bal[k]);
        }
        __syncthreads();
#pragma unroll
        for (int k = 0; k < 2; ++k) {
            uint32_t before = 0;
#pragma unroll
            for (int ww = 0; ww < 4; ++ww) {
                const uint32_t c = s_cnt[k][ww];
                if (ww < (int)w) before += c;
                nvis += c;
            }
            if (k == 1) before += s_cnt[0][0] + s_cnt[0][1] + s_cnt[0][2] + s_cnt[0][3];
            if (vis[k]) s_ids[before + (uint32_t)__popcll(bal[k] & ((1ull << lane) - 1ull))] = (k * 256 + tid) | (STATE ? sb[k] << 16 : 0u);
        }
        __syncthreads();
    }

    PRE_STAMP(0);
    const uint32_t trips = (nvis + 255u) / 256u;
    const uint32_t ts_ = f.tile_size, sub = ts_ >= 16u ? ts_ / 2u : ts_, ns = ts_ / sub;
    const float inv_ts = 1.0f / (float)ts_, inv_sub = 1.0f / (float)sub;
    const uint32_t shard = bid & 15u, shard_cap = f.row_cap >> 4;
    for (uint32_t v = tid, trip = 0; TIGHT ? trip < trips : v < nvis; v += 256, ++trip) {
        const bool active = v < nvis;
        const uint32_t sid = s_ids[active ? v : nvis - 1u];
        const uint32_t i = base + (STATE ? (sid & 0xFFFFu) : sid);
        const float4* geo = s.geo + (uint64_t)i * 2;
        const float x = KEEP_POS ? s_pos[0][v < nvis ? v : nvis - 1u] : s.px[i], y = KEEP_POS ? s_pos[1][v < nvis ? v : nvis - 1u] : s.py[i],
                    z = KEEP_POS ? s_pos[2][v < nvis ? v : nvis - 1u] : s.pz[i];
        float ph[4], pv[4];
        m4_mulv(u.proj, x, y, z, ph);
        const float pw = 1.0f / (ph[3] + 0.0000001f);
        const float ndx = ph[0] * pw, ndy = ph[1] * pw;
        m4_mulv(u.view, x, y, z, pv);
        const float uvx = (ndx * 0.5f) + 0.5f, uvy = (ndy * 0.5f) + 0.5f;
        const float4 so = geo[0];
        const float4 q = geo[1];
        const float mod = u.scale_modifier;
        const float sc[3] = {gs_exp(so.x) * mod, gs_exp(so.y) * mod, gs_exp(so.z) * mod};
        const float len = __builtin_sqrtf(((q.x * q.x + q.y * q.y) + q.z * q.z) + q.w * q.w);
        const float qr = q.x / len, qx = q.y / len, qy = q.z / len, qz = q.w / len;
        M3 R;
        R.m[0][0] = 1.f - 2.f * (qy * qy + qz * qz); R.m[0][1] = 2.f * (qx * qy - qr * qz); R.m[0][2] = 2.f * (qx * qz + qr * qy);
        R.m[1][0] = 2.f * (qx * qy + qr * qz); R.m[1][1] = 1.f - 2.f * (qx * qx + qz * qz); R.m[1][2] = 2.f * (qy * qz - qr * qx);
        R.m[2][0] = 2.f * (qx * qz - qr * qy); R.m[2][1] = 2.f * (qy * qz + qr * qx); R.m[2][2] = 1.f - 2.f * (qx * qx + qy * qy);
        M3 M;
#pragma unroll
        for (int c = 0; c < 3; ++c)
#pragma unroll
            for (int r = 0; r < 3; ++r) M.m[c][r] = sc[r] * R.m[c][r];
        const M3 Sig = m3_mul(m3_t(M), M);
        float t0 = pv[0], t1 = pv[1];
        const float t2 = pv[2];
        const float limx = 1.3f * u.tan_fovx, limy = 1.3f * u.tan_fovy;
        t0 = wg_min(limx, wg_max(-limx, t0 / t2)) * t2;
        t1 = wg_min(limy, wg_max(-limy, t1 / t2)) * t2;
        M3 J;
        J.m[0][0] = u.focal_x / t2; J.m[0][1] = 0.f; J.m[0][2] = -(u.focal_x * t0) / (t2 * t2);
        J.m[1][0] = 0.f; J.m[1][1] = u.focal_y / t2; J.m[1][2] = -(u.focal_y * t1) / (t2 * t2);
        J.m[2][0] = 0.f; J.m[2][1] = 0.f; J.m[2][2] = 0.f;
        M3 Wm;
#pragma unroll
        for (int c = 0; c < 3; ++c)
#pragma unroll
            for (int r = 0; r < 3; ++r) Wm.m[c][r] = u.view[r * 4 + c];
        const M3 Tm = m3_mul(Wm, J);
        M3 Vrk;
        Vrk.m[0][0] = Sig.m[0][0]; Vrk.m[0][1] = Sig.m[0][1]; Vrk.m[0][2] = Sig.m[0][2];
        Vrk.m[1][0] = Sig.m[0][1]; Vrk.m[1][1] = Sig.m[1][1]; Vrk.m[1][2] = Sig.m[1][2];
        Vrk.m[2][0] = Sig.m[0][2]; Vrk.m[2][1] = Sig.m[1][2]; Vrk.m[2][2] = Sig.m[2][2];
        const M3 cov = m3_mul(m3_mul(m3_t(Tm), m3_t(Vrk)), Tm);
        const float ca = cov.m[0][0] + 0.3f, cb = cov.m[0][1], cc = cov.m[1][1] + 0.3f;
        const float det = ca * cc - cb * cb;
        uint32_t count = 0;
        uint32_t rminx = 0, rminy = 0, rmaxx = 0, rmaxy = 0;
        uint32_t t_xa = 0, t_wmain = 0, t_alias = 0;
        float conx = 0.f, cony = 0.f, conz = 0.f, opacity = 0.f;
        if (det != 0.0f) {
            const float det_inv = 1.0f / det;
            conx = cc * det_inv; cony = (-cb) * det_inv; conz = ca * det_inv;
            const float mid = 0.5f * (ca + cc);
            const float sq = __builtin_sqrtf(wg_max(0.1f, mid * mid - det));
            const float l1 = mid + sq, l2 = mid - sq;
            const float radius = __builtin_ceilf(3.f * __builtin_sqrtf(wg_max(l1, l2)));
            const float pxs = uvx * (float)f.width, pys = uvy * (float)f.height;
            const int ts = (int)f.tile_size, ntx = (int)f.ntx, nty = (int)f.nty;
            rminx = (uint32_t)wg_mini(ntx, wg_maxi(0, f2i_sat(pxs - radius) / ts));
            rminy = (uint32_t)wg_mini(nty, wg_maxi(0, f2i_sat(pys - radius) / ts));
            rmaxx = (uint32_t)(wg_mini(ntx, wg_maxi(0, f2i_sat(pxs + radius) / ts)) + 1);
            rmaxy = (uint32_t)(wg_mini(nty, wg_maxi(0, f2i_sat(pys + radius) / ts)) + 1);
            uint32_t xa, wmain, alias;
            slab_cols(rminx, rmaxx, f, xa, wmain, alias);
            count = f.full ? (rmaxy - rminy) * (rmaxx - rminx)  : (rmaxy - rminy) * (wmain + alias);
            if (TIGHT) { t_xa = xa; t_wmain = wmain; t_alias = alias; }
        }
        uint32_t nslots = 0, rowptr = 0;
        if (TIGHT) {
            uint32_t ra = 0, nrows = 0;
            if (active && count) {
                opacity = sigmoid_ref(so.w);
                const TightG tg = tight_setup(uvx, uvy, conx, cony, conz, opacity, (float)f.width, (float)f.height);
                if (tg.mode == 0u) count = 0u;
                else {
                    uint32_t rb;
                    tight_rows(tg, rminy, rmaxy, f.tile_size, inv_ts, f.nty, t_alias, ra, rb);
                    nrows = rb - ra;
                    nslots = nrows * (1u + t_alias);
                    if (!nslots) count = 0u;
                    s_tA[tid] = make_float4(tg.gx, tg.gy, tg.kc, tg.qa);
                    s_tB[tid] = make_float4(tg.qb, tg.rcx, tg.xmax, tg.dyR);
                    s_tC[tid] = make_float4(tg.eR, __uint_as_float(tg.mode), __uint_as_float(ra | (nrows << 16)),
                                            __uint_as_float(t_xa | (t_wmain << 16) | (t_alias << 31)));
                }
            } else {
                count = 0u;
            }
            s_tcnt[tid] = 0u;
            PRE_STAMP(1);
            const uint32_t rincl = wave_incl_scan(nslots, lane);
            const uint32_t Rw = (uint32_t)__builtin_amdgcn_readlane((int)rincl, 63);
            const uint32_t myrp = rincl - nslots;
            const unsigned long long recb = __ballot(nslots != 0u);
            const uint32_t recrank = (uint32_t)__popcll(recb & ((1ull << lane) - 1ull));
            if (lane == 63) s_tw[w] = rincl | ((uint32_t)__popcll(recb) << 16);
            __syncthreads();
            uint32_t wbase = 0, R = 0, cbase = 0, C = 0;
#pragma unroll
            for (int k = 0; k < 4; ++k) {
                const uint32_t t = s_tw[k];
                if (k < (int)w) { wbase += t & 0xFFFFu; cbase += t >> 16; }
                R += t & 0xFFFFu; C += t >> 16;
            }
            if (tid == 0) {
                uint32_t at = 0, rat = 0, ok = 1u;
                if (R) {
                    at = atomicAdd(&to.ctl->row_cursor[shard], R);
                    rat = atomicAdd(&to.ctl->rec_cursor[shard], C);
                    if (at > shard_cap || R > shard_cap - at) { ok = 0u; to.ctl->overflow = 1u; }
                }
                s_misc[2] = at; s_misc[3] = ok; s_misc[4] = rat;
            }
            __syncthreads();
            const uint32_t abase = shard * shard_cap + s_misc[2] + wbase;
            const bool ok = s_misc[3] != 0u;
            if (nslots) s_tgid[tid] = shard * to.rec_shard_cap + s_misc[4] + cbase + recrank;
            PRE_STAMP(2);
            uint32_t jcarry = 0u;
            for (uint32_t rb0 = 0; rb0 < Rw; rb0 += 64u) {
                s_mark[tid] = 0u;
                __builtin_amdgcn_fence(__ATOMIC_RELEASE, "wavefront");
                if (nslots && myrp >= rb0 && myrp < rb0 + 64u) s_mark[(w << 6) + (myrp - rb0)] = lane + 1u;
                __builtin_amdgcn_fence(__ATOMIC_RELEASE, "wavefront");
                __builtin_amdgcn_fence(__ATOMIC_ACQUIRE, "wavefront");
                uint32_t m = wave_incl_max(s_mark[tid]);
                m = m > jcarry ? m : jcarry;
                jcarry = (uint32_t)__builtin_amdgcn_readlane((int)m, 63);
                const uint32_t ri = rb0 + lane;
                const uint32_t rpj = (uint32_t)__shfl((int)myrp, (int)(m ? m - 1u : 0u), 64);
                if (ri < Rw) {
                    const uint32_t j = (w << 6) + (m - 1u);
                    const float4 a = s_tA[j], b = s_tB[j], c4 = s_tC[j];
                    TightG g;
                    g.gx = a.x; g.gy = a.y; g.kc = a.z; g.qa = a.w; g.qb = b.x; g.rcx = b.y; g.xmax = b.z; g.dyR = b.w;
                    g.eR = c4.x; g.mode = __float_as_uint(c4.y);
                    g.cx = g.cy = g.cz = g.cxz = g.lim2 = g.ymax = 0.0f;
                    const uint32_t rw = __float_as_uint(c4.z), cw = __float_as_uint(c4.w);
                    uint32_t w1, w2;
                    const uint32_t ilen = tight_slot_item(g, ri - rpj, rw & 0xFFFFu, rw >> 16, f.tile_size, inv_ts, sub, inv_sub, ns, f.nty, cw & 0xFFFFu,
                                                          (cw >> 16) & 0x7FFFu, cw >> 31, w1, w2);
                    if (ilen) {
                        atomicAdd(&s_tcnt[j], ilen);
                        atomicAdd(&s_rowhist[w1 & 0xFFu], 1u);
                    }
                    if (ok) {
                        gs_row_u32x3 it;
                        it.x = ilen ? s_tgid[j] : GS_ROW_HOLE; it.y = w1; it.z = w2;
                        *reinterpret_cast<gs_row_u32x3*>(to.arena + (uint64_t)(abase + ri) * 3u) = it;
                    }
                }
            }
            __builtin_amdgcn_fence(__ATOMIC_RELEASE, "wavefront");
            __builtin_amdgcn_fence(__ATOMIC_ACQUIRE, "wavefront");
            if (count) count = ok ? s_tcnt[tid] : 0u;
            rowptr = abase + myrp;
            PRE_STAMP(3);
            if (!active) continue;
        }
        const uint32_t bucket = f2u_sat(wg_min(50.0f * pv[2], 999.0f));
        const uint32_t word = count ? ((TIGHT ? nslots : count) | (bucket << GS_COUNT_BITS)) : 0u;
        if (TIGHT) {
            const uint32_t off = STATE ? (sid & 0xFFFFu) : sid, uk = off >> 10;
            const uint32_t e = ((bid * (NB / 2) + uk) << 10) + (v - (NB == 2 ? 0u : s_ust[uk]));
            tile_counts[e] = word;
            to.rowptr[e] = rowptr;
            to.unit_off[e] = (unsigned short)(off & 1023u);
        } else tile_counts[i] = word;
        if (count == 0) continue;

        float col[3];
        sh_colour(s.sh + (uint64_t)i * 12, x, y, z, u, col);
        if (STATE && ((sid >> 16) & GS_ST_SELECTED) && tint.k != 0.0f) {
#pragma unroll
            for (int c = 0; c < 3; ++c) col[c] = col[c] + tint.k * (tint.t[c] - col[c]);
        }
        if (!TIGHT) opacity = sigmoid_ref(so.w);
        uint4* o4 = gdata + (uint64_t)(TIGHT ? s_tgid[tid] : i) * 4;
        o4[0] = make_uint4(__float_as_uint(uvx), __float_as_uint(uvy), i, 0u);
        o4[1] = make_uint4(__float_as_uint(conx), __float_as_uint(cony), __float_as_uint(conz), __float_as_uint(pv[2]));
        o4[2] = make_uint4(__float_as_uint(col[0]), __float_as_uint(col[1]), __float_as_uint(col[2]), __float_as_uint(opacity));
        o4[3] = make_uint4(rminx, rminy, rmaxx, rmaxy);
    }
    PRE_STAMP(4);
#ifdef GS_PROFILING
    if (TIGHT && lane == 0) {
        unsigned long long* pp = gs_pre_prof[(bid * 4u + w) & 255u];
        for (int k = 0; k < 5; ++k) atomicAdd(&pp[k], (unsigned long long)pacc[k]);
        atomicAdd(&pp[5], 1ull);
    }
#endif
    if (TIGHT) {
        __syncthreads();
        const uint32_t c = s_rowhist[tid];
        if (c) atomicAdd(&to.ctl->rowhist[bid & 7u][tid], c);
    }
}

void gs_launch_repack(const void* d_aos, uint32_t n, uint32_t first, const GsScene& s, hipStream_t st) {
    const uint64_t total = (uint64_t)n * 20;
    const uint32_t blocks = (uint32_t)((total + 255) / 256);
    if (!blocks) return;
    hipLaunchKernelGGL(gs_repack_kernel, dim3(blocks), dim3(256), 0, st, (const float4*)d_aos, n, first, (float*)s.px, (float*)s.py,
                       (float*)s.pz, (float*)s.smax, (float*)s.geo, (float*)s.sh);
}
float gs_view_norm2(const GsUniforms& u) {
    double A[3][3];
    for (int i = 0; i < 3; ++i)
        for (int j = 0; j < 3; ++j) {
            A[i][j] = 0.0;
            for (int r = 0; r < 3; ++r) A[i][j] += (double)u.view[4 * i + r] * (double)u.view[4 * j + r];
        }
    const double q = (A[0][0] + A[1][1] + A[2][2]) / 3.0;
    const double d0 = A[0][0] - q, d1 = A[1][1] - q, d2 = A[2][2] - q;
    const double p2 = (d0 * d0 + d1 * d1 + d2 * d2 + 2.0 * (A[0][1] * A[0][1] + A[0][2] * A[0][2] + A[1][2] * A[1][2])) / 6.0;
    const double p = sqrt(p2);
    double lam = q;
    if (!(p <= 1e-14 * fabs(q))) {
        const double b01 = A[0][1] / p, b02 = A[0][2] / p, b12 = A[1][2] / p, b0 = d0 / p, b1 = d1 / p, b2 = d2 / p;
        double r = 0.5 * (b0 * (b1 * b2 - b12 * b12) - b01 * (b01 * b2 - b12 * b02) + b02 * (b01 * b12 - b1 * b02));
        r = r < -1.0 ? -1.0 : (r > 1.0 ? 1.0 : r);
        lam = q + 2.0 * p * cos(acos(r) / 3.0);
    }
    return (float)(lam * (1.0 + 1e-7));
}
void gs_preprocess_prepare(GsPreprocessLaunch& L, const GsScene& s, const GsUniforms& u, const GsFrame& f, void* gdata, uint32_t* counts,
                           bool tight, uint32_t* arena, uint32_t* rowptr, unsigned short* unit_off, uint32_t* unit_n, GsControl* ctl,
                           uint32_t tight_nb, bool state, GsTint tint) {
    const uint32_t wcols = f.col1 - f.col0;
    uint32_t nb = f.full || wcols * 4u > f.ntx * 3u ? 1u : (wcols * 10u > f.ntx * 3u ? 4u : 8u);
    if (tight) nb = tight_nb ? tight_nb : (nb == 1u ? 2u : nb);
    L.blocks = (f.n + PRE_G * nb - 1) / (PRE_G * nb);
    if (state) {
        if (tight) L.func = nb == 8u ? (const void*)&gs_preprocess_kernel<true, 8, true> : nb == 4u ? (const void*)&gs_preprocess_kernel<true, 4, true>
                                                                                                     : (const void*)&gs_preprocess_kernel<true, 2, true>;
        else L.func = nb == 8u ? (const void*)&gs_preprocess_kernel<false, 8, true> : nb == 4u ? (const void*)&gs_preprocess_kernel<false, 4, true>
                                                                                                  : (const void*)&gs_preprocess_kernel<false, 1, true>;
    } else {
        if (tight) L.func = nb == 8u ? (const void*)&gs_preprocess_kernel<true, 8, false> : nb == 4u ? (const void*)&gs_preprocess_kernel<true, 4, false>
                                                                                                      : (const void*)&gs_preprocess_kernel<true, 2, false>;
        else L.func = nb == 8u ? (const void*)&gs_preprocess_kernel<false, 8, false> : nb == 4u ? (const void*)&gs_preprocess_kernel<false, 4, false>
                                                                                                   : (const void*)&gs_preprocess_kernel<false, 1, false>;
    }
    L.s = s; L.u = u; L.f = f; L.gdata = gdata; L.counts = counts; L.tint = tint;
    L.w2 = f.full ? 1.0f : gs_view_norm2(u);
    L.to.arena = arena; L.to.rowptr = rowptr; L.to.unit_off = unit_off; L.to.unit_n = unit_n; L.to.ctl = ctl;
    L.to.rec_shard_cap = ((L.blocks + 15u) / 16u) * (PRE_G * nb);
    L.args[0] = &L.s; L.args[1] = &L.u; L.args[2] = &L.f; L.args[3] = &L.gdata; L.args[4] = &L.counts; L.args[5] = &L.to; L.args[6] = &L.tint; L.args[7] = &L.w2;
}
void gs_launch_preprocess(GsPreprocessLaunch& L, hipStream_t st) {
    if (!L.f.n) return;
    (void)hipLaunchKernel(L.func, dim3(L.blocks), dim3(256), L.args, 0, st);
}
```

Measured before the change: 1470 frames/s.

## Precompute per-gaussian 3D covariance and opacity at scene load, read in preprocess

Adds a derive kernel that computes each gaussian's 3D covariance (from scale and rotation) and sigmoid opacity into a new per-scene buffer. It runs after every scene mutation: load, insert, compact, grade, snapshot write and stream. Preprocess gets a DERIVED template variant that loads these six covariance terms plus opacity instead of doing exp, quaternion normalisation, matrix products and sigmoid every frame. The variant is used only when scale_modifier is exactly 1. This costs extra scene memory, a derive pass on each edit, and risk if any mutation path misses the refresh.

```diff
diff --git a/gaussian-splatting-wgpu_amd/csrc/build.py b/gaussian-splatting-wgpu_amd/csrc/build.py
--- a/gaussian-splatting-wgpu_amd/csrc/build.py
+++ b/gaussian-splatting-wgpu_amd/csrc/build.py
@@ -13,7 +13,7 @@
 FILE_FLAGS = {}
 SOURCES = ["k_preprocess.hip", "k_binning.hip", "k_gsort.hip", "k_rows.hip", "k_sort.hip", "k_blend.hip", "k_pick.hip", "k_state.hip", "k_export.hip", "k_insert.hip", "k_snapshot.hip", "k_xform.hip", "k_grade.hip", "k_coverage.hip", "k_attr.hip", "k_neigh.hip", "k_cluster.hip", "k_knn.hip", "k_pack.hip",
            "gs_context.hip", "gs_frame.hip", "gs_readback.hip", "gs_state.hip", "gs_export.hip", "gs_insert.hip", "gs_snapshot.hip", "gs_xform.hip", "gs_xform_math.hip", "gs_grade.hip", "gs_grade_math.hip", "gs_coverage.hip", "gs_attr.hip", "gs_neigh.hip", "gs_cluster.hip", "gs_knn.hip", "gs_pack.hip", "gs_pack_host.hip", "gs_ply.hip", "gs_stages.hip",
-           "k_moments.hip", "gs_moments.hip", "k_pairs.hip", "gs_pairs.hip", "k_consensus.hip", "gs_consensus.hip", "k_merge.hip", "gs_merge.hip", "k_surface.hip", "gs_surface.hip"]
+           "k_moments.hip", "gs_moments.hip", "k_pairs.hip", "gs_pairs.hip", "k_consensus.hip", "gs_consensus.hip", "k_merge.hip", "gs_merge.hip", "k_surface.hip", "gs_surface.hip", "k_derive.hip"]
 
 
 def _stale(target, deps):
@@ -27,7 +27,7 @@
     os.makedirs(OUT, exist_ok=True)
     objdir = os.path.join(OUT, "obj_prof" if profiling else "obj")
     os.makedirs(objdir, exist_ok=True)
-    headers = [os.path.join(HERE, h) for h in ("gs_device.h", "gs_binning.h", "gs_kernels.h", "gs_tight.h", "gs_runtime.h", "gs_xform_math.h", "gs_grade_math.h", "gs_state_sum.h", "gs_neigh_dev.h", "gs_pack_math.h", "gs_exact_sum.h", "gs_exact_dev.h", "gs_pair_host.h", "gs_pack_host.h", "gs_file_writer.h", "gs_consensus_host.h", "gs_merge_math.h", "gs_grid_math.h", "gs_surface_math.h")] + [
+    headers = [os.path.join(HERE, h) for h in ("gs_device.h", "gs_binning.h", "gs_kernels.h", "gs_tight.h", "gs_runtime.h", "gs_xform_math.h", "gs_grade_math.h", "gs_state_sum.h", "gs_neigh_dev.h", "gs_pack_math.h", "gs_exact_sum.h", "gs_exact_dev.h", "gs_pair_host.h", "gs_pack_host.h", "gs_file_writer.h", "gs_consensus_host.h", "gs_merge_math.h", "gs_grid_math.h", "gs_surface_math.h", "gs_geod_math.h")] + [
         os.path.join(HERE, "..", "..", "include", "gsplat", "gs_abi.h")]
 
     def compile_one(src):
diff --git a/gaussian-splatting-wgpu_amd/csrc/gs_context.hip b/gaussian-splatting-wgpu_amd/csrc/gs_context.hip
--- a/gaussian-splatting-wgpu_amd/csrc/gs_context.hip
+++ b/gaussian-splatting-wgpu_amd/csrc/gs_context.hip
@@ -1,6 +1,7 @@
 #include <atomic>
 #include <cmath>
 #include <cstdarg>
+#include <cstdlib>
 #include <memory>
 #include <new>
 
@@ -141,6 +142,7 @@
             for (auto& e : row) HIP_TRY(hipEventCreate(e.out()));
         c->have_events = true;
     }
+    if (const char* e = getenv("GS_PROJ_RECOMPUTE")) c->recompute = atoi(e) != 0;
     c->fif = (c->own_stream && f.full) ? 3u : 1u;
     *out = c.release();
     return GS_OK;
@@ -193,16 +195,18 @@
 GsSceneLayout scene_layout(void* base, uint64_t n, bool state) {
     GsSceneLayout L;
     const size_t np = ((size_t)n + 63) & ~(size_t)63;
-    const size_t sh_end = np * 4 * 4 + np * 32 + (size_t)n * 192, state_at = (sh_end + 255) & ~(size_t)255;
+    const size_t sh_end = np * 4 * 4 + np * 32 + (size_t)n * 192, geod_at = (sh_end + 255) & ~(size_t)255;
+    const size_t state_at = geod_at + np * 32;
     L.np = np;
     L.state_at = state_at;
-    L.bytes = state ? state_at + np : sh_end;
+    L.bytes = state ? state_at + np : state_at;
     char* p = (char*)base;
     GsScene& s = L.scene;
     s.px = (float*)p; p += np * 4; s.py = (float*)p; p += np * 4; s.pz = (float*)p; p += np * 4;
     s.smax = (float*)p; p += np * 4;
     s.geo = (float4*)p; p += np * 32;
     s.sh = (float4*)p;
+    s.geod = (float4*)((char*)base + geod_at);
     s.state = state ? (const uint8_t*)base + state_at : nullptr;
     return L;
 }
@@ -245,6 +249,7 @@
     int32_t rc = scene_alloc(c, n);
     if (rc != GS_OK) return rc;
     if (n) gs_launch_repack(d_aos, (uint32_t)n, 0, c->scene, c->stream);
+    scene_derive(c, c->scene, 0, n);
     HIP_TRY(hipGetLastError());
     HIP_TRY(hipStreamSynchronize(c->stream));
     return GS_OK;
diff --git a/gaussian-splatting-wgpu_amd/csrc/gs_device.h b/gaussian-splatting-wgpu_amd/csrc/gs_device.h
--- a/gaussian-splatting-wgpu_amd/csrc/gs_device.h
+++ b/gaussian-splatting-wgpu_amd/csrc/gs_device.h
@@ -1,6 +1,8 @@
 #pragma once
 #include <hip/hip_runtime.h>
 #include <stdint.h>
+
+#include "gs_geod_math.h"
 
 #define GS_WAVE 64
 
@@ -82,6 +84,7 @@
     const float4* geo;
     const float4* sh;
     const uint8_t* state;
+    const float4* geod;
 };
 
 #define GS_ST_HIDDEN 1u
@@ -136,29 +139,6 @@
     return (uint32_t)x;
 }
 
-__device__ __forceinline__ float gs_exp(float x) {
-    if (x != x) return x;
-    if (x > 88.72283935546875f) return __builtin_inff();
-    if (x < -103.97208404541015625f) return 0.0f;
-    const float nf = __builtin_rintf(x * 1.44269502162933349609375f);
-    float r = __builtin_fmaf(-nf, 0.693145751953125f, x);
-    r = __builtin_fmaf(-nf, 1.42860677465796470642e-06f, r);
-    float p = 1.9875691500e-4f;
-    p = __builtin_fmaf(p, r, 1.3981999507e-3f);
-    p = __builtin_fmaf(p, r, 8.3334519073e-3f);
-    p = __builtin_fmaf(p, r, 4.1665795894e-2f);
-    p = __builtin_fmaf(p, r, 1.6666665459e-1f);
-    p = __builtin_fmaf(p, r, 5.0000001201e-1f);
-    const float z = r * r;
-    float y = __builtin_fmaf(p, z, r);
-    y = y + 1.0f;
-    const int n = (int)nf;
-    const int a = n >> 1;
-    const int b = n - a;
-    const float sa = __uint_as_float((uint32_t)(a + 127) << 23);
-    const float sb = __uint_as_float((uint32_t)(b + 127) << 23);
-    return (y * sa) * sb;
-}
 
 __device__ __forceinline__ float gs_blend_power(float cx, float cy, float cz, float dx, float dy) {
     const float t1 = cx * dx * dx, t2 = cz * dy * dy, t3 = cy * dx * dy;
diff --git a/gaussian-splatting-wgpu_amd/csrc/gs_export.hip b/gaussian-splatting-wgpu_amd/csrc/gs_export.hip
--- a/gaussian-splatting-wgpu_amd/csrc/gs_export.hip
+++ b/gaussian-splatting-wgpu_amd/csrc/gs_export.hip
@@ -104,6 +104,7 @@
         return rc;
     }
     gs_launch_compact_planes(old, n_old, c->ex.ids, (uint32_t)total, c->scene, c->stream);
+    scene_derive(c, c->scene, 0, total);
     HIP_TRY(hipGetLastError());
     HIP_TRY(hipStreamSynchronize(c->stream));
     if (kept) *kept = total;
diff --git a/gaussian-splatting-wgpu_amd/csrc/gs_frame.hip b/gaussian-splatting-wgpu_amd/csrc/gs_frame.hip
--- a/gaussian-splatting-wgpu_amd/csrc/gs_frame.hip
+++ b/gaussian-splatting-wgpu_amd/csrc/gs_frame.hip
@@ -41,7 +41,7 @@
 
 static void prepare_projection(gs_ctx* c, const GsUniforms& u, bool tight) {
     gs_preprocess_prepare(c->pre, c->scene, u, c->frame, c->gdata, c->counts, tight, c->arena, c->rowptr, c->unit_off, c->unit_n, c->ctl, c->opt.tight_nb,
-                          has_state(c), tint_of(c->opt.select_tint));
+                          has_state(c), tint_of(c->opt.select_tint), !c->recompute);
 }
 
 
@@ -140,7 +140,7 @@
     const bool tight = !debug && c->opt.tile_cull && c->tight_ok && (uint64_t)c->n + GS_RECORD_SLACK <= (1ull << GS_ID_BITS);
     const bool graphable = c->opt.frame_graph && !debug && !c->have_events && !(c->opt.blend_ablation & 0x10000u) && c->n;
     if (graphable) {
-        const GraphKey key{index_order, tight, ext_rgba8, c->alpha, c->depth};
+        const GraphKey key{index_order, tight, gs_preprocess_derived(u, !c->recompute), ext_rgba8, c->alpha, c->depth};
         if (!c->gr.exec || !c->gr.valid || !(c->gr.key == key)) {
             if (c->gr.exec) HIP_TRY(hipStreamSynchronize(st));
             drop_graph(c);
@@ -281,6 +281,7 @@
     rc = gs_share_splats(s, c);
     if (rc != GS_OK) { gs_destroy(s); return rc; }
     s->opt = c->opt;
+    s->recompute = c->recompute;
     c->shadows.push_back(s);
     return GS_OK;
 }
diff --git a/gaussian-splatting-wgpu_amd/csrc/gs_geod_math.h b/gaussian-splatting-wgpu_amd/csrc/gs_geod_math.h
--- /dev/null
+++ b/gaussian-splatting-wgpu_amd/csrc/gs_geod_math.h
@@ -0,0 +1,79 @@
+#pragma once
+#include <stdint.h>
+
+#if defined(__HIPCC__)
+#include <hip/hip_runtime.h>
+#define GS_GD __host__ __device__ __forceinline__
+#else
+#define GS_GD inline
+#endif
+
+GS_GD float gs_exp(float x) {
+    if (x != x) return x;
+    if (x > 88.72283935546875f) return __builtin_inff();
+    if (x < -103.97208404541015625f) return 0.0f;
+    const float nf = __builtin_rintf(x * 1.44269502162933349609375f);
+    float r = __builtin_fmaf(-nf, 0.693145751953125f, x);
+    r = __builtin_fmaf(-nf, 1.42860677465796470642e-06f, r);
+    float p = 1.9875691500e-4f;
+    p = __builtin_fmaf(p, r, 1.3981999507e-3f);
+    p = __builtin_fmaf(p, r, 8.3334519073e-3f);
+    p = __builtin_fmaf(p, r, 4.1665795894e-2f);
+    p = __builtin_fmaf(p, r, 1.6666665459e-1f);
+    p = __builtin_fmaf(p, r, 5.0000001201e-1f);
+    const float z = r * r;
+    float y = __builtin_fmaf(p, z, r);
+    y = y + 1.0f;
+    const int n = (int)nf;
+    const int a = n >> 1;
+    const int b = n - a;
+    const float sa = __builtin_bit_cast(float, (uint32_t)(a + 127) << 23);
+    const float sb = __builtin_bit_cast(float, (uint32_t)(b + 127) << 23);
+    return (y * sa) * sb;
+}
+
+struct M3 { float m[3][3]; };
+GS_GD M3 m3_mul(const M3& A, const M3& B) {
+    M3 o;
+#pragma unroll
+    for (int c = 0; c < 3; ++c)
+#pragma unroll
+        for (int r = 0; r < 3; ++r) o.m[c][r] = (A.m[0][r] * B.m[c][0] + A.m[1][r] * B.m[c][1]) + A.m[2][r] * B.m[c][2];
+    return o;
+}
+GS_GD M3 m3_t(const M3& A) {
+    M3 o;
+#pragma unroll
+    for (int c = 0; c < 3; ++c)
+#pragma unroll
+        for (int r = 0; r < 3; ++r) o.m[c][r] = A.m[r][c];
+    return o;
+}
+
+GS_GD float sigmoid_ref(float o) {
+    const float ez = gs_exp(o);
+    const float cond = (o >= 0.0f) ? 1.0f : 0.0f;
+    return (cond * (1.0f / (1.0f + gs_exp(-o)))) + ((1.0f - cond) * (ez / (1.0f + ez)));
+}
+
+GS_GD M3 gs_cov3d(float s0, float s1, float s2, float qw0, float qw1, float qw2, float qw3, float mod) {
+    const float sc[3] = {gs_exp(s0) * mod, gs_exp(s1) * mod, gs_exp(s2) * mod};
+    const float len = __builtin_sqrtf(((qw0 * qw0 + qw1 * qw1) + qw2 * qw2) + qw3 * qw3);
+    const float qr = qw0 / len, qx = qw1 / len, qy = qw2 / len, qz = qw3 / len;
+    M3 R;
+    R.m[0][0] = 1.f - 2.f * (qy * qy + qz * qz); R.m[0][1] = 2.f * (qx * qy - qr * qz); R.m[0][2] = 2.f * (qx * qz + qr * qy);
+    R.m[1][0] = 2.f * (qx * qy + qr * qz); R.m[1][1] = 1.f - 2.f * (qx * qx + qz * qz); R.m[1][2] = 2.f * (qy * qz - qr * qx);
+    R.m[2][0] = 2.f * (qx * qz - qr * qy); R.m[2][1] = 2.f * (qy * qz + qr * qx); R.m[2][2] = 1.f - 2.f * (qx * qx + qy * qy);
+    M3 M;
+#pragma unroll
+    for (int c = 0; c < 3; ++c)
+#pragma unroll
+        for (int r = 0; r < 3; ++r) M.m[c][r] = sc[r] * R.m[c][r];
+    return m3_mul(m3_t(M), M);
+}
+
+GS_GD void gs_derive_record(const float geo[8], float out[8]) {
+    const M3 Sig = gs_cov3d(geo[0], geo[1], geo[2], geo[4], geo[5], geo[6], geo[7], 1.0f);
+    out[0] = Sig.m[0][0]; out[1] = Sig.m[0][1]; out[2] = Sig.m[0][2]; out[3] = Sig.m[1][1];
+    out[4] = Sig.m[1][2]; out[5] = Sig.m[2][2]; out[6] = sigmoid_ref(geo[3]); out[7] = 0.0f;
+}
diff --git a/gaussian-splatting-wgpu_amd/csrc/gs_grade.hip b/gaussian-splatting-wgpu_amd/csrc/gs_grade.hip
--- a/gaussian-splatting-wgpu_amd/csrc/gs_grade.hip
+++ b/gaussian-splatting-wgpu_amd/csrc/gs_grade.hip
@@ -24,6 +24,7 @@
         if (rc != GS_OK) return rc;
     }
     gs_launch_grade(c->scene, c->n, all ? nullptr : c->ex.ids.get(), (uint32_t)total, *g, c->stream);
+    if (g->flags & GS_GRADE_OPACITY) scene_derive(c, c->scene, 0, total, all ? nullptr : c->ex.ids.get());
     HIP_TRY(hipGetLastError());
     HIP_TRY(hipStreamSynchronize(c->stream));
     if (matched) *matched = total;
diff --git a/gaussian-splatting-wgpu_amd/csrc/gs_insert.hip b/gaussian-splatting-wgpu_amd/csrc/gs_insert.hip
--- a/gaussian-splatting-wgpu_amd/csrc/gs_insert.hip
+++ b/gaussian-splatting-wgpu_amd/csrc/gs_insert.hip
@@ -30,6 +30,7 @@
     HIP_TRY(hipGetLastError());
     int32_t rc = fill(dst);
     if (rc != GS_OK) return rc;
+    scene_derive(c, dst, 0, n_new);
     HIP_TRY(hipGetLastError());
     HIP_TRY(hipStreamSynchronize(c->stream));
     drop_shadows(c);
diff --git a/gaussian-splatting-wgpu_amd/csrc/gs_kernels.h b/gaussian-splatting-wgpu_amd/csrc/gs_kernels.h
--- a/gaussian-splatting-wgpu_amd/csrc/gs_kernels.h
+++ b/gaussian-splatting-wgpu_amd/csrc/gs_kernels.h
@@ -10,13 +10,20 @@
     uint32_t blocks;
     GsScene s; GsUniforms u; GsFrame f;
     void* gdata; uint32_t* counts; GsTightOut to; GsTint tint;
+    bool derived;
     float w2;
     void* args[8];
 };
 float gs_view_norm2(const GsUniforms& u);
+inline bool gs_preprocess_derived(const GsUniforms& u, bool use_derived) {
+    uint32_t bits;
+    __builtin_memcpy(&bits, &u.scale_modifier, 4);
+    return use_derived && bits == 0x3F800000u;
+}
 void gs_preprocess_prepare(GsPreprocessLaunch& L, const GsScene& s, const GsUniforms& u, const GsFrame& f, void* gdata, uint32_t* counts,
                            bool tight, uint32_t* arena, uint32_t* rowptr, unsigned short* unit_off, uint32_t* unit_n, GsControl* ctl,
-                           uint32_t tight_nb = 0, bool state = false, GsTint tint = GsTint{});
+                           uint32_t tight_nb = 0, bool state = false, GsTint tint = GsTint{}, bool use_derived = true);
+void gs_launch_derive(const GsScene& s, uint32_t first, uint32_t m, const uint32_t* ids, hipStream_t st);
 void gs_launch_preprocess(GsPreprocessLaunch& L, hipStream_t st);
 void gs_launch_zero(void* p, uint64_t bytes, hipStream_t st);
 uint32_t gs_scan_blocks(uint32_t n);
diff --git a/gaussian-splatting-wgpu_amd/csrc/gs_readback.hip b/gaussian-splatting-wgpu_amd/csrc/gs_readback.hip
--- a/gaussian-splatting-wgpu_amd/csrc/gs_readback.hip
+++ b/gaussian-splatting-wgpu_amd/csrc/gs_readback.hip
@@ -121,11 +121,14 @@
     const bool tight = c->notes.last_tight;
     const uint64_t I = std::min<uint64_t>(c->h_rep->num_intersections, c->capacity);
     const bool all_masks = which == GS_BUF_BLOCK_MASKS && !tight, list_counts = which == GS_BUF_TILE_COUNTS && tight;
+    const bool launch_rec = which == 16;
     if (all_masks) bytes = I * 4;
+    else if (launch_rec) bytes = 4;
     else if (list_counts) bytes = (uint64_t)c->n * 4;
     else { int32_t rc = tap(c, which, &p, &bytes); if (rc != GS_OK) return rc; }
     { int32_t rc = size_protocol(bytes, dst, size, written, &copy); if (rc != GS_OK || !copy) return rc; }
     uint32_t* w = (uint32_t*)dst;
+    if (launch_rec) { w[0] = c->pre.derived ? 1u : 0u; return GS_OK; }
     if (all_masks) {
         const uint32_t nb = (c->frame.tile_size / 8) * (c->frame.tile_size / 8);
         const uint32_t all = nb >= 32 ? 0xFFFFFFFFu : (1u << nb) - 1u;
diff --git a/gaussian-splatting-wgpu_amd/csrc/gs_runtime.h b/gaussian-splatting-wgpu_amd/csrc/gs_runtime.h
--- a/gaussian-splatting-wgpu_amd/csrc/gs_runtime.h
+++ b/gaussian-splatting-wgpu_amd/csrc/gs_runtime.h
@@ -68,9 +68,10 @@
 
 struct GraphKey {
     bool index = false, tight = false;
+    bool derived = false;
     void* ext = nullptr;
     float *alpha = nullptr, *depth = nullptr;
-    bool operator==(const GraphKey& o) const { return index == o.index && tight == o.tight && ext == o.ext && alpha == o.alpha && depth == o.depth; }
+    bool operator==(const GraphKey& o) const { return index == o.index && tight == o.tight && derived == o.derived && ext == o.ext && alpha == o.alpha && depth == o.depth; }
 };
 
 struct GsOptions {
@@ -191,6 +192,7 @@
         uint64_t frames = 0;
     } gr;
     GsPreprocessLaunch pre{};
+    bool recompute = false;
     FrameNotes notes;
     bool have_frame = false, pending = false, last_debug = false;
     void* last_ext = nullptr;
@@ -207,6 +209,9 @@
 GsSceneLayout scene_layout(void* base, uint64_t n, bool state);
 int32_t scene_install(gs_ctx* c, DevBuf<>&& mem, uint64_t n, uint64_t min_capacity, uint64_t min_rows);
 uint64_t scene_new_serial();
+inline void scene_derive(gs_ctx* c, const GsScene& s, uint64_t first, uint64_t m, const uint32_t* ids = nullptr) {
+    gs_launch_derive(s, (uint32_t)first, (uint32_t)m, ids, c->stream);
+}
 void drop_shadows(gs_ctx* c);
 void drop_graph(gs_ctx* c);
 int32_t wait_one(gs_ctx* c);
@@ -332,6 +337,9 @@
     if (rc != GS_OK) return rc;
     rc = src.stream(who, c, c->scene, 0);
     if (rc != GS_OK) return rc;
+    scene_derive(c, c->scene, 0, src.count());
+    HIP_TRY(hipGetLastError());
+    HIP_TRY(hipStreamSynchronize(c->stream));
     if (n_out) *n_out = src.count();
     return GS_OK;
 }
diff --git a/gaussian-splatting-wgpu_amd/csrc/gs_snapshot.hip b/gaussian-splatting-wgpu_amd/csrc/gs_snapshot.hip
--- a/gaussian-splatting-wgpu_amd/csrc/gs_snapshot.hip
+++ b/gaussian-splatting-wgpu_amd/csrc/gs_snapshot.hip
@@ -75,6 +75,7 @@
             if (rc != GS_OK) return rc;
         }
         gs_launch_write(aos, states, (uint32_t)m, ids, c->scene, c->n, parts, c->stream);
+        if (parts & GS_PART_GEOMETRY) scene_derive(c, c->scene, 0, m, ids);
         HIP_TRY(hipGetLastError());
         HIP_TRY(hipStreamSynchronize(c->stream));
         if (written) *written = m;
@@ -100,6 +101,7 @@
             n -= (uint32_t)first;
         }
         gs_launch_write(d_rec, d_st, (uint32_t)k, ids ? d_ids : nullptr, s, n, parts, c->stream);
+        if (parts & GS_PART_GEOMETRY) scene_derive(c, c->scene, first, k, ids ? d_ids : nullptr);
         HIP_TRY(hipGetLastError());
         HIP_TRY(hipStreamSynchronize(c->stream));
     }
@@ -196,6 +198,7 @@
     const bool work = s->count && parts;
     if (work) {
         gs_launch_snapshot(mode, c->scene, c->n, s->dev, (uint32_t)s->count, parts, c->stream);
+        if (parts & GS_PART_GEOMETRY) scene_derive(c, c->scene, 0, s->count, s->dev.ids);
         HIP_TRY(hipGetLastError());
         HIP_TRY(hipStreamSynchronize(c->stream));
     }
diff --git a/gaussian-splatting-wgpu_amd/csrc/gs_xform.hip b/gaussian-splatting-wgpu_amd/csrc/gs_xform.hip
--- a/gaussian-splatting-wgpu_amd/csrc/gs_xform.hip
+++ b/gaussian-splatting-wgpu_amd/csrc/gs_xform.hip
@@ -36,6 +36,7 @@
         if (rc != GS_OK) return rc;
     }
     gs_launch_xform(c->scene, c->n, all ? nullptr : c->ex.ids.get(), (uint32_t)total, *x, c->stream);
+    if (x->flags & (GS_XFORM_ORIENT | GS_XFORM_SIZE)) scene_derive(c, c->scene, 0, total, all ? nullptr : c->ex.ids.get());
     HIP_TRY(hipGetLastError());
     HIP_TRY(hipStreamSynchronize(c->stream));
     if (matched) *matched = total;
diff --git a/gaussian-splatting-wgpu_amd/csrc/k_derive.hip b/gaussian-splatting-wgpu_amd/csrc/k_derive.hip
--- /dev/null
+++ b/gaussian-splatting-wgpu_amd/csrc/k_derive.hip
@@ -0,0 +1,20 @@
+#include "gs_device.h"
+#include "gs_kernels.h"
+
+__global__ __launch_bounds__(256) void gs_derive_kernel(const float4* __restrict__ geo, float4* __restrict__ geod, uint32_t first, uint32_t m,
+                                                         const uint32_t* __restrict__ ids) {
+    const uint32_t g = blockIdx.x * 256u + threadIdx.x;
+    if (g >= m) return;
+    const uint64_t i = ids ? ids[g] : first + g;
+    const float4 a = geo[i * 2], b = geo[i * 2 + 1];
+    const float in[8] = {a.x, a.y, a.z, a.w, b.x, b.y, b.z, b.w};
+    float out[8];
+    gs_derive_record(in, out);
+    geod[i * 2] = make_float4(out[0], out[1], out[2], out[3]);
+    geod[i * 2 + 1] = make_float4(out[4], out[5], out[6], out[7]);
+}
+
+void gs_launch_derive(const GsScene& s, uint32_t first, uint32_t m, const uint32_t* ids, hipStream_t st) {
+    if (!m) return;
+    hipLaunchKernelGGL(gs_derive_kernel, dim3((m + 255u) / 256u), dim3(256), 0, st, s.geo, const_cast<float4*>(s.geod), first, m, ids);
+}
diff --git a/gaussian-splatting-wgpu_amd/csrc/k_preprocess.hip b/gaussian-splatting-wgpu_amd/csrc/k_preprocess.hip
--- a/gaussian-splatting-wgpu_amd/csrc/k_preprocess.hip
+++ b/gaussian-splatting-wgpu_amd/csrc/k_preprocess.hip
@@ -63,32 +63,9 @@
                        (float*)s.px, (float*)s.py, (float*)s.pz, (float*)s.smax, (float*)s.geo, (float*)s.sh);
 }
 
-struct M3 { float m[3][3]; };
-__device__ __forceinline__ M3 m3_mul(const M3& A, const M3& B) {
-    M3 o;
-#pragma unroll
-    for (int c = 0; c < 3; ++c)
-#pragma unroll
-        for (int r = 0; r < 3; ++r) o.m[c][r] = (A.m[0][r] * B.m[c][0] + A.m[1][r] * B.m[c][1]) + A.m[2][r] * B.m[c][2];
-    return o;
-}
-__device__ __forceinline__ M3 m3_t(const M3& A) {
-    M3 o;
-#pragma unroll
-    for (int c = 0; c < 3; ++c)
-#pragma unroll
-        for (int r = 0; r < 3; ++r) o.m[c][r] = A.m[r][c];
-    return o;
-}
 __device__ __forceinline__ void m4_mulv(const float* m, float x, float y, float z, float* o) {
 #pragma unroll
     for (int r = 0; r < 4; ++r) o[r] = ((m[0 + r] * x + m[4 + r] * y) + m[8 + r] * z) + m[12 + r] * 1.0f;
-}
-
-__device__ __forceinline__ float sigmoid_ref(float o) {
-    const float ez = gs_exp(o);
-    const float cond = (o >= 0.0f) ? 1.0f : 0.0f;
-    return (cond * (1.0f / (1.0f + gs_exp(-o)))) + ((1.0f - cond) * (ez / (1.0f + ez)));
 }
 
 __device__ __forceinline__ void sh_colour(const float4* __restrict__ sh, float x, float y, float z, const GsUniforms& u, float col[3]) {
@@ -174,7 +151,7 @@
 typedef uint32_t gs_row_u32x3 __attribute__((ext_vector_type(3), aligned(4)));
 
 
-template <bool TIGHT, int NB, bool STATE>
+template <bool TIGHT, int NB, bool STATE, bool DERIVED>
 __global__ __launch_bounds__(256, PRE_WAVES) void gs_preprocess_kernel(GsScene s, GsUniforms u, GsFrame f, uint4* __restrict__ gdata,
                                                              uint32_t* __restrict__ tile_counts, GsTightOut to, GsTint tint, float w2) {
     __shared__ uint32_t s_ids[PRE_G * NB];
@@ -337,7 +314,7 @@
         const bool active = v < nvis;
         const uint32_t sid = s_ids[active ? v : nvis - 1u];
         const uint32_t i = base + (STATE ? (sid & 0xFFFFu) : sid);
-        const float4* geo = s.geo + (uint64_t)i * 2;
+        const float4* geo = (DERIVED ? s.geod : s.geo) + (uint64_t)i * 2;
         const float x = KEEP_POS ? s_pos[0][v < nvis ? v : nvis - 1u] : s.px[i], y = KEEP_POS ? s_pos[1][v < nvis ? v : nvis - 1u] : s.py[i],
                     z = KEEP_POS ? s_pos[2][v < nvis ? v : nvis - 1u] : s.pz[i];
         float ph[4], pv[4];
@@ -348,20 +325,12 @@
         const float uvx = (ndx * 0.5f) + 0.5f, uvy = (ndy * 0.5f) + 0.5f;
         const float4 so = geo[0];
         const float4 q = geo[1];
-        const float mod = u.scale_modifier;
-        const float sc[3] = {gs_exp(so.x) * mod, gs_exp(so.y) * mod, gs_exp(so.z) * mod};
-        const float len = __builtin_sqrtf(((q.x * q.x + q.y * q.y) + q.z * q.z) + q.w * q.w);
-        const float qr = q.x / len, qx = q.y / len, qy = q.z / len, qz = q.w / len;
-        M3 R;
-        R.m[0][0] = 1.f - 2.f * (qy * qy + qz * qz); R.m[0][1] = 2.f * (qx * qy - qr * qz); R.m[0][2] = 2.f * (qx * qz + qr * qy);
-        R.m[1][0] = 2.f * (qx * qy + qr * qz); R.m[1][1] = 1.f - 2.f * (qx * qx + qz * qz); R.m[1][2] = 2.f * (qy * qz - qr * qx);
-        R.m[2][0] = 2.f * (qx * qz - qr * qy); R.m[2][1] = 2.f * (qy * qz + qr * qx); R.m[2][2] = 1.f - 2.f * (qx * qx + qy * qy);
-        M3 M;
-#pragma unroll
-        for (int c = 0; c < 3; ++c)
-#pragma unroll
-            for (int r = 0; r < 3; ++r) M.m[c][r] = sc[r] * R.m[c][r];
-        const M3 Sig = m3_mul(m3_t(M), M);
+        M3 Sig;
+        if (DERIVED) {
+            Sig.m[0][0] = so.x; Sig.m[0][1] = so.y; Sig.m[0][2] = so.z; Sig.m[1][1] = so.w; Sig.m[1][2] = q.x; Sig.m[2][2] = q.y;
+        } else {
+            Sig = gs_cov3d(so.x, so.y, so.z, q.x, q.y, q.z, q.w, u.scale_modifier);
+        }
         float t0 = pv[0], t1 = pv[1];
         const float t2 = pv[2];
         const float limx = 1.3f * u.tan_fovx, limy = 1.3f * u.tan_fovy;
@@ -410,7 +379,7 @@
         if (TIGHT) {
             uint32_t ra = 0, nrows = 0;
             if (active && count) {
-                opacity = sigmoid_ref(so.w);
+                opacity = DERIVED ? q.z : sigmoid_ref(so.w);
                 const TightG tg = tight_setup(uvx, uvy, conx, cony, conz, opacity, (float)f.width, (float)f.height);
                 if (tg.mode == 0u) count = 0u;
                 else {
@@ -515,7 +484,7 @@
 #pragma unroll
             for (int c = 0; c < 3; ++c) col[c] = col[c] + tint.k * (tint.t[c] - col[c]);
         }
-        if (!TIGHT) opacity = sigmoid_ref(so.w);
+        if (!TIGHT) opacity = DERIVED ? q.z : sigmoid_ref(so.w);
         uint4* o4 = gdata + (uint64_t)(TIGHT ? s_tgid[tid] : i) * 4;
         o4[0] = make_uint4(__float_as_uint(uvx), __float_as_uint(uvy), i, 0u);
         o4[1] = make_uint4(__float_as_uint(conx), __float_as_uint(cony), __float_as_uint(conz), __float_as_uint(pv[2]));
@@ -566,22 +535,18 @@
 }
 void gs_preprocess_prepare(GsPreprocessLaunch& L, const GsScene& s, const GsUniforms& u, const GsFrame& f, void* gdata, uint32_t* counts,
                            bool tight, uint32_t* arena, uint32_t* rowptr, unsigned short* unit_off, uint32_t* unit_n, GsControl* ctl,
-                           uint32_t tight_nb, bool state, GsTint tint) {
+                           uint32_t tight_nb, bool state, GsTint tint, bool use_derived) {
     const uint32_t wcols = f.col1 - f.col0;
     uint32_t nb = f.full || wcols * 4u > f.ntx * 3u ? 1u : (wcols * 10u > f.ntx * 3u ? 4u : 8u);
     if (tight) nb = tight_nb ? tight_nb : (nb == 1u ? 2u : nb);
     L.blocks = (f.n + PRE_G * nb - 1) / (PRE_G * nb);
-    if (state) {
-        if (tight) L.func = nb == 8u ? (const void*)&gs_preprocess_kernel<true, 8, true> : nb == 4u ? (const void*)&gs_preprocess_kernel<true, 4, true>
-                                                                                                     : (const void*)&gs_preprocess_kernel<true, 2, true>;
-        else L.func = nb == 8u ? (const void*)&gs_preprocess_kernel<false, 8, true> : nb == 4u ? (const void*)&gs_preprocess_kernel<false, 4, true>
-                                                                                                  : (const void*)&gs_preprocess_kernel<false, 1, true>;
-    } else {
-        if (tight) L.func = nb == 8u ? (const void*)&gs_preprocess_kernel<true, 8, false> : nb == 4u ? (const void*)&gs_preprocess_kernel<true, 4, false>
-                                                                                                      : (const void*)&gs_preprocess_kernel<true, 2, false>;
-        else L.func = nb == 8u ? (const void*)&gs_preprocess_kernel<false, 8, false> : nb == 4u ? (const void*)&gs_preprocess_kernel<false, 4, false>
-                                                                                                   : (const void*)&gs_preprocess_kernel<false, 1, false>;
-    }
+    const bool derived = gs_preprocess_derived(u, use_derived);
+#define PRE_PICK(T, S, D) (nb == 8u ? (const void*)&gs_preprocess_kernel<T, 8, S, D> : nb == 4u ? (const void*)&gs_preprocess_kernel<T, 4, S, D> \
+                                                                                                : (const void*)&gs_preprocess_kernel<T, (T ? 2 : 1), S, D>)
+    if (derived) L.func = state ? (tight ? PRE_PICK(true, true, true) : PRE_PICK(false, true, true)) : (tight ? PRE_PICK(true, false, true) : PRE_PICK(false, false, true));
+    else L.func = state ? (tight ? PRE_PICK(true, true, false) : PRE_PICK(false, true, false)) : (tight ? PRE_PICK(true, false, false) : PRE_PICK(false, false, false));
+#undef PRE_PICK
+    L.derived = derived;
     L.s = s; L.u = u; L.f = f; L.gdata = gdata; L.counts = counts; L.tint = tint;
     L.w2 = f.full ? 1.0f : gs_view_norm2(u);
     L.to.arena = arena; L.to.rowptr = rowptr; L.to.unit_off = unit_off; L.to.unit_n = unit_n; L.to.ctl = ctl;
```

New measurement: 1467 frames/s. No clear change (-0.2%).
